# KogarashiNetwork/dusk-plonk

Hardware: AMD Instinct MI355X
Metric: PLONK prover constraints/sec (BLS12-381) at n=2^16 and 2^20, 1/2/4/8 GPUs (higher is better)
Workload: dtype u32-limb Montgomery Fr/Fp (integer)

## Files before the change

### dusk-plonk_amd/csrc/debug.hip

```cpp
#include <hip/hip_runtime.h>

#include "g1r.hpp"
#include "internal.hpp"

namespace plk {
namespace {

template <class C>
__global__ void k_field_op(int op, const Fe<C>* __restrict__ a, const Fe<C>* __restrict__ b,
                           Fe<C>* __restrict__ out, uint64_t n) {
  const uint64_t i = (uint64_t)blockIdx.x * blockDim.x + threadIdx.x;
  if (i >= n) return;
  const Fe<C> x = a[i], y = b[i];
  Fe<C> r;
  switch (op) {
    case 0: r = fe_mul(x, y); break;
    case 1: r = fe_add(x, y); break;
    case 2: r = fe_sub(x, y); break;
    case 3: r = fe_sqr(x); break;
    default: r = fe_inv(x); break;
  }
  out[i] = r;
}

template <class C>
int run(plk_ctx* ctx, int op, const uint64_t* a, const uint64_t* b, uint64_t* out, size_t n) {
  const size_t bytes = n * sizeof(Fe<C>);
  DevBuf da, db, dout;
  int st;
  if ((st = da.alloc(bytes)) || (st = db.alloc(bytes)) || (st = dout.alloc(bytes))) return st;
  hipStream_t s = ctx->stream;
  PLK_HIP_TRY(hipMemcpyAsync(da.ptr, a, bytes, hipMemcpyHostToDevice, s));
  PLK_HIP_TRY(hipMemcpyAsync(db.ptr, b ? b : a, bytes, hipMemcpyHostToDevice, s));
  hipLaunchKernelGGL(k_field_op<C>, dim3((unsigned)((n + 255) / 256)), dim3(256), 0, s, op,
                     da.as<Fe<C>>(), db.as<Fe<C>>(), dout.as<Fe<C>>(), (uint64_t)n);
  PLK_HIP_TRY(hipGetLastError());
  PLK_HIP_TRY(hipMemcpyAsync(out, dout.ptr, bytes, hipMemcpyDeviceToHost, s));
  PLK_HIP_TRY(stream_wait(s));
  return PLK_OK;
}

enum : int {
  kOpMul = 0, kOpSqr, kOpMulAdd, kOpMul2, kOpMul2Asm, kOpSqr2, kOpSqr2Asm, kOpMulAddMul2,
  kOpMulAddMul2Asm, kOpMul3, kOpAdd, kOpSub, kOpSubLazy, kOpSub2N6, kOpSmall2, kOpSmall3,
  kOpCanon, kOpIsZero, kOpIsZeroU, kOpUnpackPack, kOpSubU = 100, kOpSubN = 200
};

constexpr int rx_op_nin(int op) {
  if (op >= kOpSubU) return 2;
  switch (op) {
    case kOpSqr: case kOpSmall2: case kOpSmall3: case kOpCanon: case kOpIsZero: case kOpIsZeroU:
    case kOpUnpackPack: return 1;
    case kOpMul: case kOpSqr2: case kOpSqr2Asm: case kOpAdd: case kOpSub: case kOpSubLazy: return 2;
    case kOpSub2N6: return 3;
    default: return 4;
  }
}
constexpr int rx_op_nout(int op) {
  switch (op) {
    case kOpMul2: case kOpMul2Asm: case kOpSqr2: case kOpSqr2Asm: case kOpUnpackPack: return 2;
    case kOpMulAddMul2: case kOpMulAddMul2Asm: case kOpMul3: return 3;
    default: return 1;
  }
}

template <class C>
__device__ __forceinline__ Rx<C> ld_row(const uint32_t* __restrict__ p, uint64_t i) {
  Rx<C> r;
#pragma unroll
  for (int k = 0; k < RxShape<C>::L; ++k) r.v[k] = p[i * RxShape<C>::L + k];
  return r;
}
template <class C>
__device__ __forceinline__ void st_row(uint32_t* __restrict__ p, uint64_t i, const Rx<C>& r) {
#pragma unroll
  for (int k = 0; k < RxShape<C>::L; ++k) p[i * RxShape<C>::L + k] = r.v[k];
}
template <class C>
__device__ __forceinline__ Rx<C> rx_flag(bool f) {
  Rx<C> r = rx_zero<C>();
  r.v[0] = f ? 1u : 0u;
  return r;
}

template <class C, int OP>
__global__ void __launch_bounds__(256)
    k_rx_op(const uint32_t* __restrict__ a, const uint32_t* __restrict__ b,
            const uint32_t* __restrict__ c, const uint32_t* __restrict__ d,
            uint32_t* __restrict__ out, uint64_t n) {
  constexpr int NIN = rx_op_nin(OP), NOUT = rx_op_nout(OP);
  const uint64_t i = (uint64_t)blockIdx.x * blockDim.x + threadIdx.x;
  if (i >= n) return;
  const Rx<C> x0 = ld_row<C>(a, i);
  const Rx<C> x1 = NIN > 1 ? ld_row<C>(b, i) : rx_zero<C>();
  const Rx<C> x2 = NIN > 2 ? ld_row<C>(c, i) : rx_zero<C>();
  const Rx<C> x3 = NIN > 3 ? ld_row<C>(d, i) : rx_zero<C>();
  Rx<C> o0 = rx_zero<C>(), o1 = rx_zero<C>(), o2 = rx_zero<C>();
  if constexpr (OP == kOpMul) o0 = rx_mul(x0, x1);
  else if constexpr (OP == kOpSqr) o0 = rx_sqr(x0);
  else if constexpr (OP == kOpMulAdd) o0 = rx_mul_add(x0, x1, x2, x3);
  else if constexpr (OP == kOpMul2) rx_mul2<C, false>(x0, x1, x2, x3, o0, o1);
  else if constexpr (OP == kOpMul2Asm) rx_mul2<C, true>(x0, x1, x2, x3, o0, o1);
  else if constexpr (OP == kOpSqr2) rx_sqr2<C, false>(x0, x1, o0, o1);
  else if constexpr (OP == kOpSqr2Asm) rx_sqr2<C, true>(x0, x1, o0, o1);
  else if constexpr (OP == kOpMulAddMul2) rx_mul_add_mul2<C, false>(x0, x1, x2, x3, x0, x3, x2, x1, o0, o1, o2);
  else if constexpr (OP == kOpMulAddMul2Asm) rx_mul_add_mul2<C, true>(x0, x1, x2, x3, x0, x3, x2, x1, o0, o1, o2);
  else if constexpr (OP == kOpMul3) rx_mul3<C>(x0, x1, x2, x3, x3, x0, o0, o1, o2);
  else if constexpr (OP == kOpAdd) o0 = rx_add(x0, x1);
  else if constexpr (OP == kOpSub) o0 = rx_sub(x0, x1);
  else if constexpr (OP == kOpSubLazy) o0 = rx_sub_lazy(x0, x1);
  else if constexpr (OP == kOpSub2N6) o0 = rx_sub2_n<C, 6>(x0, x1, x2);
  else if constexpr (OP == kOpSmall2) o0 = rx_small_mul_n<C, 2>(x0);
  else if constexpr (OP == kOpSmall3) o0 = rx_small_mul_n<C, 3>(x0);
  else if constexpr (OP == kOpCanon) o0 = rx_canon(x0);
  else if constexpr (OP == kOpIsZero) o0 = rx_flag<C>(rx_is_zero(x0));
  else if constexpr (OP == kOpIsZeroU) o0 = rx_flag<C>(rx_is_zero_u(x0));
  else if constexpr (OP == kOpUnpackPack) {
    Fe<C> w;
#pragma unroll
    for (int k = 0; k < C::N; ++k) w.v[k] = x0.v[k];
    o0 = rx_unpack(w);
    w = rx_pack(o0);
#pragma unroll
    for (int k = 0; k < C::N; ++k) o1.v[k] = w.v[k];
  } else if constexpr (OP >= kOpSubN) o0 = rx_sub_n<C, OP - kOpSubN>(x0, x1);
  else o0 = rx_sub_u<C, OP - kOpSubU>(x0, x1);
  st_row<C>(out, i * NOUT, o0);
  if constexpr (NOUT > 1) st_row<C>(out, i * NOUT + 1, o1);
  if constexpr (NOUT > 2) st_row<C>(out, i * NOUT + 2, o2);
}

using RxKernel = void (*)(const uint32_t*, const uint32_t*, const uint32_t*, const uint32_t*,
                          uint32_t*, uint64_t);
#define PLK_RX_CASE(C, OP) \
  case OP: return k_rx_op<C, OP>;
#define PLK_RX_COMMON(C)                                                                       \
  PLK_RX_CASE(C, kOpMul) PLK_RX_CASE(C, kOpSqr) PLK_RX_CASE(C, kOpMulAdd) PLK_RX_CASE(C, kOpMul2) \
  PLK_RX_CASE(C, kOpMul2Asm) PLK_RX_CASE(C, kOpSqr2) PLK_RX_CASE(C, kOpMulAddMul2)             \
  PLK_RX_CASE(C, kOpMul3) PLK_RX_CASE(C, kOpAdd) PLK_RX_CASE(C, kOpSub) PLK_RX_CASE(C, kOpSubLazy) \
  PLK_RX_CASE(C, kOpSub2N6) PLK_RX_CASE(C, kOpSmall2) PLK_RX_CASE(C, kOpSmall3)                \
  PLK_RX_CASE(C, kOpCanon) PLK_RX_CASE(C, kOpIsZero) PLK_RX_CASE(C, kOpIsZeroU)                \
  PLK_RX_CASE(C, kOpUnpackPack) PLK_RX_CASE(C, kOpSubU + 3) PLK_RX_CASE(C, kOpSubU + 5)        \
  PLK_RX_CASE(C, kOpSubU + 6) PLK_RX_CASE(C, kOpSubN + 3) PLK_RX_CASE(C, kOpSubN + 5)          \
  PLK_RX_CASE(C, kOpSubN + 6)
RxKernel rx_kernel(int field, int op) {
  if (field == 0) {
    switch (op) {
      PLK_RX_COMMON(FrCfg)
      default: return nullptr;
    }
  }
  switch (op) {
    PLK_RX_COMMON(FpCfg)
    PLK_RX_CASE(FpCfg, kOpSqr2Asm) PLK_RX_CASE(FpCfg, kOpMulAddMul2Asm)
    PLK_RX_CASE(FpCfg, kOpSubU + 4) PLK_RX_CASE(FpCfg, kOpSubU + 10)
    PLK_RX_CASE(FpCfg, kOpSubN + 4) PLK_RX_CASE(FpCfg, kOpSubN + 10)
// ... 17 lines not shown
  r.X = ld_row<FpCfg>(p, 4 * i);
  r.Y = ld_row<FpCfg>(p, 4 * i + 1);
  r.ZZ = ld_row<FpCfg>(p, 4 * i + 2);
  r.ZZZ = ld_row<FpCfg>(p, 4 * i + 3);
  return r;
}

template <bool GROUPED, bool ASM, bool PAIRS>
__device__ __forceinline__ G1R madd_as_accumulate(const G1R& acc, const G1R& q, bool neg) {
  RFp y = q.Y;
  if (neg) y = rx_neg_lazy(y);
  const bool was_inf = g1r_is_inf(acc);
  G1R r = g1r_madd_lazy_sl<GROUPED, ASM, PAIRS>(acc, q.X, y);
  if (rx_is_zero(r.ZZ)) {
    RFp yr = q.Y;
    if (neg) yr = rx_neg(yr);
    r = g1r_madd_lazy_fix(was_inf, r, q.X, yr);
  }
  return r;
}

template <int OP>
__global__ void __launch_bounds__(256)
    k_g1r_op(const uint32_t* __restrict__ p, const uint32_t* __restrict__ q,
             const uint32_t* __restrict__ flags, uint32_t* __restrict__ out, uint64_t n) {
  const uint64_t t = (uint64_t)blockIdx.x * blockDim.x + threadIdx.x;
  const uint64_t i = OP == kG1AddQuad ? t >> 2 : t;
  if (i >= n) return;
  const G1R a = ld_g1row(p, i);
  G1R b = g1_op_needs_q(OP) ? ld_g1row(q, i) : a;
  const bool neg = g1_op_needs_q(OP) && flags && (flags[i] & 1u);
  G1R r;
  if constexpr (OP == kG1Madd000) r = madd_as_accumulate<false, false, false>(a, b, neg);
  else if constexpr (OP == kG1Madd100) r = madd_as_accumulate<true, false, false>(a, b, neg);
  else if constexpr (OP == kG1Madd110) r = madd_as_accumulate<true, true, false>(a, b, neg);
  else if constexpr (OP == kG1Madd111) r = madd_as_accumulate<true, true, true>(a, b, neg);
  else if constexpr (OP == kG1MaddLazy) r = g1r_madd_lazy(a, b.X, neg ? rx_neg_lazy(b.Y) : b.Y);
  else if constexpr (OP == kG1AddLazy || OP == kG1AddQuad) {
    if (neg) b.Y = rx_neg_lazy(b.Y);
    if constexpr (OP == kG1AddLazy) r = g1r_add_lazy(a, b);
    else r = g1r_add_quad(a, b, threadIdx.x & 3u);
  } else if constexpr (OP == kG1DblLazy) r = g1r_dbl_lazy(a);
  else if constexpr (OP == kG1LazyFinish) r = g1r_lazy_finish(a);
  else if constexpr (OP == kG1Add) r = g1r_add(a, neg ? g1r_neg(b) : b);
  else if constexpr (OP == kG1AddAffine) r = g1r_add_affine(a, b.X, neg ? rx_neg(b.Y) : b.Y);
  else if constexpr (OP == kG1Dbl) r = g1r_dbl(a);
  else r = g1r_dbl_affine(a.X, a.Y);
  st_row<FpCfg>(out, 4 * t, r.X);
  st_row<FpCfg>(out, 4 * t + 1, r.Y);
  st_row<FpCfg>(out, 4 * t + 2, r.ZZ);
  st_row<FpCfg>(out, 4 * t + 3, r.ZZZ);
}

using G1Kernel = void (*)(const uint32_t*, const uint32_t*, const uint32_t*, uint32_t*, uint64_t);
G1Kernel g1r_kernel(int op) {
  switch (op) {
#define PLK_G1_CASE(OP) \
  case OP: return k_g1r_op<OP>;
    PLK_G1_CASE(kG1Madd000) PLK_G1_CASE(kG1Madd100) PLK_G1_CASE(kG1Madd110)
    PLK_G1_CASE(kG1Madd111) PLK_G1_CASE(kG1MaddLazy) PLK_G1_CASE(kG1AddLazy)
    PLK_G1_CASE(kG1AddQuad) PLK_G1_CASE(kG1DblLazy) PLK_G1_CASE(kG1LazyFinish)
    PLK_G1_CASE(kG1Add) PLK_G1_CASE(kG1AddAffine) PLK_G1_CASE(kG1Dbl) PLK_G1_CASE(kG1DblAffine)
#undef PLK_G1_CASE
    default: return nullptr;
  }
}

struct RowArg {
  const uint32_t* host;
  size_t bytes;
};
template <class K, size_t NA>
int run_rows(plk_ctx* ctx, K kern, const RowArg (&in)[NA], uint32_t* out, size_t out_bytes,
             uint64_t threads, uint64_t n) {
  DevBuf din[NA], dout;
  int st;
  hipStream_t s = ctx->stream;
  for (size_t k = 0; k < NA; ++k) {
    if (!in[k].host) continue;
    if ((st = din[k].alloc(in[k].bytes))) return st;
    PLK_HIP_TRY(hipMemcpyAsync(din[k].ptr, in[k].host, in[k].bytes, hipMemcpyHostToDevice, s));
  }
  if ((st = dout.alloc(out_bytes))) return st;
  const dim3 grid((unsigned)((threads + 255) / 256)), block(256);
  const uint32_t* dp[NA];
  for (size_t k = 0; k < NA; ++k) dp[k] = static_cast<const uint32_t*>(din[k].ptr);
  uint32_t* const dres = static_cast<uint32_t*>(dout.ptr);
  if constexpr (NA == 4)
    hipLaunchKernelGGL(kern, grid, block, 0, s, dp[0], dp[1], dp[2], dp[3], dres, n);
  else
    hipLaunchKernelGGL(kern, grid, block, 0, s, dp[0], dp[1], dp[2], dres, n);
  PLK_HIP_TRY(hipGetLastError());
  PLK_HIP_TRY(hipMemcpyAsync(out, dout.ptr, out_bytes, hipMemcpyDeviceToHost, s));
  PLK_HIP_TRY(stream_wait(s));
  return PLK_OK;
}

}
}

extern "C" int plk_debug_rx_op(plk_ctx* ctx, int field, int op, const uint32_t* a,
                               const uint32_t* b, const uint32_t* c, const uint32_t* d,
                               uint32_t* out, size_t n) {
  try {
    if (!ctx || !out || (field != 0 && field != 1)) return PLK_E_ARG;
    const plk::RxKernel kern = plk::rx_kernel(field, op);
    if (!kern) return PLK_E_ARG;
    const uint32_t* rows[4] = {a, b, c, d};
    const int nin = plk::rx_op_nin(op);
    for (int k = 0; k < nin; ++k)
      if (!rows[k]) return PLK_E_ARG;
    if (n == 0) return PLK_OK;
    const size_t row = (field == 0 ? 9 : 13) * sizeof(uint32_t);
    plk::RowArg in[4];
    for (int k = 0; k < 4; ++k) in[k] = {k < nin ? rows[k] : nullptr, n * row};
    plk::DeviceGuard g(ctx->device);
    return plk::run_rows(ctx, kern, in, out, n * row * plk::rx_op_nout(op), n, n);
  } catch (...) {
    return PLK_E_DEVICE;
  }
}

extern "C" int plk_debug_g1r_op(plk_ctx* ctx, int op, const uint32_t* p, const uint32_t* q,
                                const uint32_t* flags, uint32_t* out, size_t n) {
  try {
    if (!ctx || !p || !out) return PLK_E_ARG;
    const plk::G1Kernel kern = plk::g1r_kernel(op);
    if (!kern || (plk::g1_op_needs_q(op) && !q)) return PLK_E_ARG;
    if (n == 0) return PLK_OK;
    const size_t row = plk::kG1Row * sizeof(uint32_t);
    const uint64_t threads = op == plk::kG1AddQuad ? 4 * (uint64_t)n : n;
    const plk::RowArg in[3] = {{p, n * row},
                               {plk::g1_op_needs_q(op) ? q : nullptr, n * row},
                               {flags, n * sizeof(uint32_t)}};
    plk::DeviceGuard g(ctx->device);
    return plk::run_rows(ctx, kern, in, out, threads * row, threads, n);
  } catch (...) {
    return PLK_E_DEVICE;
  }
}

extern "C" int plk_debug_field_op(plk_ctx* ctx, int field, int op, const uint64_t* a,
                                  const uint64_t* b, uint64_t* out, size_t n) {
  try {
    if (!ctx || !a || !out || op < 0 || op > 4 || (field != 0 && field != 1)) return PLK_E_ARG;
    if (n == 0) return PLK_OK;
    plk::DeviceGuard g(ctx->device);
    return field == 0 ? plk::run<plk::FrCfg>(ctx, op, a, b, out, n)
                      : plk::run<plk::FpCfg>(ctx, op, a, b, out, n);
  } catch (...) {
    return PLK_E_DEVICE;
  }
}
```

### dusk-plonk_amd/csrc/ntt.hip

```cpp
#include <cstdlib>
#include <type_traits>

#include "ffr.hpp"
#include "internal.hpp"

namespace plk {

namespace {

constexpr uint32_t kMaxLr = 9;
constexpr uint32_t kMaxLrHard = 10;
constexpr uint32_t kMaxLe = 10;

__device__ __forceinline__ Fr ld_fr(const Fr* p) {
  const uint4* q = reinterpret_cast<const uint4*>(p);
  uint4 a = q[0], b = q[1];
  Fr r;
  r.v[0] = a.x; r.v[1] = a.y; r.v[2] = a.z; r.v[3] = a.w;
  r.v[4] = b.x; r.v[5] = b.y; r.v[6] = b.z; r.v[7] = b.w;
  return r;
}

__device__ __forceinline__ void st_fr(Fr* p, const Fr& v) {
  uint4* q = reinterpret_cast<uint4*>(p);
// ... 49 lines not shown

__device__ __forceinline__ RFr sub_u(const RFr& a, const RFr& b) { return rx_sub_u<FrCfg, 3>(a, b); }

constexpr uint32_t kB = RxShape<FrCfg>::B;
constexpr uint32_t kQMax = 32;

struct FrLimbTab {
  uint32_t v[kQMax * kL];
};
constexpr FrLimbTab make_ztab() {
  FrLimbTab t{};
  for (uint32_t q = 0; q < kQMax; ++q) {
    const RxMultiple<FrCfg> m = rx_multiple<FrCfg>(q, false);
    int64_t br = 0;
    for (int i = 0; i < kL; ++i) {
      const int64_t top = (i == kL - 1) ? (int64_t)1 << kB : 0;
      int64_t d = top - (int64_t)m.v[i] + br;
      br = 0;
      if (i < kL - 1 && d < 0) {
        d += (int64_t)1 << kB;
        br = -1;
      }
      t.v[q * kL + i] = (uint32_t)d;
    }
  }
  return t;
}
__constant__ FrLimbTab kZTab = make_ztab();

template <uint32_t CP>
struct FrRaised2 {
  static constexpr RxMultiple<FrCfg> make() {
    RxMultiple<FrCfg> m = rx_multiple<FrCfg>(CP, false);
    m.v[0] += 2u << kB;
    for (int i = 1; i < kL - 1; ++i) m.v[i] += (2u << kB) - 2u;
    m.v[kL - 1] -= 2u;
    return m;
  }
  static constexpr RxMultiple<FrCfg> k = make();
};
template <uint32_t CP>
__device__ __forceinline__ RFr sub_u2(const RFr& a, const RFr& b) {
  constexpr RxMultiple<FrCfg> Q = FrRaised2<CP>::k;
  RFr r;
#pragma unroll
  for (int i = 0; i < kL; ++i) r.v[i] = a.v[i] + Q.v[i] - b.v[i];
  return r;
}

__device__ __forceinline__ RFr add_u(const RFr& a, const RFr& b) {
  RFr r;
#pragma unroll
  for (int i = 0; i < kL; ++i) r.v[i] = a.v[i] + b.v[i];
  return r;
}

__device__ __forceinline__ RFr reduce_q(const RFr& a, const uint32_t* ztab) {
  constexpr uint32_t MASK = (1u << kB) - 1;
  const uint32_t* z = ztab + (a.v[kL - 1] >> (255 - kB * (kL - 1))) * kL;
  RFr r;
  uint32_t c = 0;
#pragma unroll
  for (int i = 0; i < kL - 1; ++i) {
    const uint32_t t = a.v[i] + z[i] + c;
    r.v[i] = t & MASK;
    c = t >> kB;
  }
  r.v[kL - 1] = a.v[kL - 1] + z[kL - 1] + c - (1u << kB);
  return r;
}

__device__ __forceinline__ RFr twmul(const RFr& a, const uint32_t* twl, uint32_t TS, uint32_t idx) {
  return rx_mul(a, lds_ld(twl, TS, idx));
}
__device__ __forceinline__ void twmul2(const RFr& a0, uint32_t i0, const RFr& a1, uint32_t i1,
                                       const uint32_t* twl, uint32_t TS, RFr& o0, RFr& o1) {
  rx_mul2<FrCfg, true>(a0, lds_ld(twl, TS, i0), a1, lds_ld(twl, TS, i1), o0, o1);
}

template <bool H1>
__device__ __forceinline__ void r4_math(const uint32_t* twl, uint32_t TS, const uint32_t* ztab,
                                        uint32_t r, uint32_t h, uint32_t sh1, uint32_t sh2,
                                        const RFr& x0, const RFr& x1, const RFr& x2,
                                        const RFr& x3, RFr& o0, RFr& o1, RFr& o2, RFr& o3) {
  const RFr y0 = add_u(x0, x2), y1 = add_u(x1, x3);
  if constexpr (H1) {
    const RFr y2 = reduce_q(rx_sub_u<FrCfg, 6>(x0, x2), ztab);
    const RFr y3 = twmul(rx_sub_u<FrCfg, 6>(x1, x3), twl, TS, 1u << sh1);
    o0 = reduce_q(add_u(y0, y1), ztab);
    o2 = reduce_q(add_u(y2, y3), ztab);
    o1 = reduce_q(sub_u2<11>(y0, y1), ztab);
    o3 = reduce_q(rx_sub_u<FrCfg, 5>(y2, y3), ztab);
  } else {
    RFr y2, y3;
    twmul2(rx_sub_u<FrCfg, 6>(x0, x2), r << sh1, rx_sub_u<FrCfg, 6>(x1, x3), (r + h) << sh1, twl, TS,
           y2, y3);
    twmul2(sub_u2<11>(y0, y1), r << sh2, rx_sub_u<FrCfg, 5>(y2, y3), r << sh2, twl, TS, o1, o3);
    o0 = reduce_q(add_u(y0, y1), ztab);
    o2 = reduce_q(add_u(y2, y3), ztab);
  }
}

template <uint32_t DS, bool H1>
__device__ __forceinline__ void r4_step(uint32_t* data, const uint32_t* twl, uint32_t TS,
                                        const uint32_t* ztab, uint32_t r, uint32_t h,
                                        uint32_t sh1, uint32_t sh2, uint32_t i0, uint32_t i1,
                                        uint32_t i2, uint32_t i3, const RFr& x0, const RFr& x1,
                                        const RFr& x2, const RFr& x3) {
  RFr o0, o1, o2, o3;
  r4_math<H1>(twl, TS, ztab, r, h, sh1, sh2, x0, x1, x2, x3, o0, o1, o2, o3);
  lds_std<DS>(data, i0, o0);
  lds_std<DS>(data, i2, o2);
  lds_std<DS>(data, i1, o1);
  lds_std<DS>(data, i3, o3);
}

__device__ __forceinline__ void quad_transpose(RFr& a0, RFr& a1, RFr& a2, RFr& a3) {
  const uint32_t lane = __lane_id();
  const bool b0 = lane & 1u, b1 = lane & 2u;
#pragma unroll
  for (int l = 0; l < kL; ++l) {
    const uint32_t s01 = b0 ? a0.v[l] : a1.v[l], s23 = b0 ? a2.v[l] : a3.v[l];
    const uint32_t r01 = (uint32_t)__builtin_amdgcn_mov_dpp((int)s01, 0xB1, 0xF, 0xF, false);
    const uint32_t r23 = (uint32_t)__builtin_amdgcn_mov_dpp((int)s23, 0xB1, 0xF, 0xF, false);
    if (b0) { a0.v[l] = r01; a2.v[l] = r23; } else { a1.v[l] = r01; a3.v[l] = r23; }
    const uint32_t s02 = b1 ? a0.v[l] : a2.v[l], s13 = b1 ? a1.v[l] : a3.v[l];
    const uint32_t r02 = (uint32_t)__builtin_amdgcn_mov_dpp((int)s02, 0x4E, 0xF, 0xF, false);
    const uint32_t r13 = (uint32_t)__builtin_amdgcn_mov_dpp((int)s13, 0x4E, 0xF, 0xF, false);
    if (b1) { a0.v[l] = r02; a1.v[l] = r13; } else { a2.v[l] = r02; a3.v[l] = r13; }
  }
}

template <int PRE, int POST, int PRUNE, uint32_t DS>
__global__ void __launch_bounds__(256, PLK_NTT_MINW) k_ntt_pass(const Fr* __restrict__ in, Fr* __restrict__ out,
                                                  const Fr* __restrict__ tw,
                                                  const Fr* __restrict__ ptw,
                                                  const Fr* __restrict__ pre,
                                                  const Fr* __restrict__ post, Fr post_scalar,
                                                  uint32_t log_n, uint32_t lp, uint32_t lr,
                                                  uint32_t lt, uint64_t len_in, NttStrides str) {
  extern __shared__ __attribute__((aligned(16))) uint32_t smem32[];
  const uint32_t R = 1u << lr, T = 1u << lt, p = 1u << lp;
  const uint32_t E = R << lt, H = R >> 1;
  const uint32_t TS = PRUNE ? R : H;
  uint32_t* data = smem32;
  uint32_t* twl = smem32 + kL * DS;
  uint32_t* ztab = twl + kL * TS;

  {
    const uint32_t y = blockIdx.y;
    const uint32_t yi = str.group_in ? y % str.group_in : y, gi = str.group_in ? y / str.group_in : 0;
    in += (size_t)yi * str.in + (size_t)gi * str.in_group;
    out += (size_t)y * str.out;
    if (PRE == 1) pre += (size_t)yi * str.pre;
    if (POST == 2) post += (size_t)(str.group_post ? y % str.group_post : y) * str.post;
  }

  const uint32_t tid = threadIdx.x, bd = blockDim.x;
  const uint32_t nr_log = log_n - lr;

  for (uint32_t x = tid; x < TS; x += bd) lds_st(twl, TS, x, ld_rfr(&tw[(size_t)x << nr_log]));
  for (uint32_t x = tid; x < kQMax * kL; x += bd) ztab[x] = kZTab.v[x];

  constexpr uint32_t kLoadIt = 4;
  const uint32_t nit = (E + bd - 1) / bd;
  Fr raw[kLoadIt], aux[kLoadIt];
  auto issue = [&](uint32_t i0) {
#pragma unroll
    for (uint32_t c = 0; c < kLoadIt; ++c) {
      const uint32_t e = min(tid + c * bd, E - 1);
      const size_t g = (size_t)(i0 + (e & (T - 1))) + ((size_t)(e >> lt) << nr_log);
      const size_t gc = g < len_in ? g : 0;
      raw[c] = ld_fr(&in[gc]);
      if (PRE == 1) aux[c] = ld_fr(&pre[gc]);
    }
    if (PRE != 1 && lp != 0) {
#pragma unroll
      for (uint32_t c = 0; c < kLoadIt; ++c) {
        const uint32_t e = min(tid + c * bd, E - 1);
        aux[c] = ld_fr(&ptw[((size_t)(e >> lt) << lp) + ((i0 + (e & (T - 1))) & (p - 1))]);
      }
    }
  };
  const uint32_t i0 = blockIdx.x << lt;

  int lh = (int)lr - 1 - (PRUNE ? 3 : 0);
  const bool r2first = !PRUNE && (lr & 1) && lr >= 3 && E >= 2 * bd;
  if (PRUNE) {
    __syncthreads();
    const uint32_t R8 = R >> 3;
    for (uint32_t it = tid; it < (E >> 2); it += bd) {
      const uint32_t hs = it & 1, t = (it >> 1) & (T - 1), j = it >> (lt + 1);
      const uint32_t i = i0 + t;
      const size_t g = (size_t)i + ((size_t)j << nr_log);
      RFr x = rx_zero<FrCfg>(), x8 = rx_zero<FrCfg>();
      if (g < len_in) {
        x = ld_rfr(&in[g]);
        if (PRE == 1) x = rx_mul(x, ld_rfr(&pre[g]));
      }
      const size_t g8 = (size_t)i + ((size_t)R8 << nr_log);
      const bool has8 = j == 0 && g8 < len_in;
      if (has8) {
        x8 = ld_rfr(&in[g8]);
        if (PRE == 1) x8 = rx_mul(x8, ld_rfr(&pre[g8]));
      }
#pragma unroll
      for (uint32_t q = 0; q < 4; ++q) {
        const uint32_t blk = 4 * hs + q, b = bitrev(blk, 3);
        RFr v = (j == 0 || b == 0) ? x : rx_mul(x, lds_ld(twl, TS, j * b));
        if (has8) v = rx_add(v, b == 0 ? x8 : rx_mul(x8, lds_ld(twl, TS, R8 * b)));
        lds_std<DS>(data, ((blk * R8 + j) << lt) + t, v);
      }
    }
  }
  if (!PRUNE) {
    issue(i0);
    auto input = [&](uint32_t c) -> RFr {
      const uint32_t e = tid + c * bd;
      const uint32_t t = e & (T - 1), j = e >> lt;
      const uint32_t i = i0 + t;
      const size_t g = (size_t)i + ((size_t)j << nr_log);
      RFr v = rx_zero<FrCfg>();
      if (g < len_in) {
        v = rx_unpack(raw[c]);
        if (PRE == 1) v = rx_mul(v, rx_unpack(aux[c]));
      }
      if (PRE != 1 && lp != 0) v = rx_mul(v, rx_unpack(aux[c]));
      return v;
    };
    {
      if (r2first) __syncthreads();
#pragma unroll
      for (uint32_t c = 0; c < kLoadIt; ++c) {
        if (c >= nit) break;
        const uint32_t e = tid + c * bd;
        const RFr v = input(c);
        if (r2first && 2 * c >= nit) {
          const uint32_t el = e - (E >> 1);
          const RFr a = lds_ldd<DS>(data, el);
          lds_std<DS>(data, el, reduce_q(add_u(a, v), ztab));
          lds_std<DS>(data, e, twmul(sub_u(a, v), twl, TS, el >> lt));
        } else if (e < E) {
          lds_std<DS>(data, e, v);
        }
      }
      if (r2first) lh -= 1;
    }
  }
  __syncthreads();

  for (; lh >= 1; lh -= 2) {
    const uint32_t h = 1u << (lh - 1);
    const uint32_t sh1 = lr - 1 - lh, sh2 = lr - lh;
    const bool quad = lh == 3 && lr >= 5 && (E >> 2) % bd == 0;
    if (quad) {
      for (uint32_t g = tid; g < (E >> 2); g += bd) {
        const uint32_t r = g & 3u, t = (g >> 2) & (T - 1), B = g >> (2 + lt);
        const uint32_t j = (B << 4) + r;
        RFr x0 = lds_ldd<DS>(data, (j << lt) + t), x1 = lds_ldd<DS>(data, ((j + 4) << lt) + t);
        RFr x2 = lds_ldd<DS>(data, ((j + 8) << lt) + t), x3 = lds_ldd<DS>(data, ((j + 12) << lt) + t);
        RFr o0, o1, o2, o3;
        r4_math<false>(twl, TS, ztab, r, 4, lr - 4, lr - 3, x0, x1, x2, x3, o0, o1, o2, o3);
        quad_transpose(o0, o1, o2, o3);
        const uint32_t jq = (B << 4) + (r << 2);
        r4_step<DS, true>(data, twl, TS, ztab, 0, 1, lr - 2, lr - 1, (jq << lt) + t,
                    ((jq + 1) << lt) + t, ((jq + 2) << lt) + t, ((jq + 3) << lt) + t, o0, o1, o2,
                    o3);
      }
      lh -= 2;
      __syncthreads();
      continue;
    }
    auto steps = [&](auto h1) {
      for (uint32_t g = tid; g < (E >> 2); g += bd) {
        const uint32_t t = g & (T - 1), jg = g >> lt;
        const uint32_t r = jg & (h - 1);
        const uint32_t j = ((jg >> (lh - 1)) << (lh + 1)) + r;
        const uint32_t i0 = (j << lt) + t, i1 = ((j + h) << lt) + t;
        const uint32_t i2 = ((j + 2 * h) << lt) + t, i3 = ((j + 3 * h) << lt) + t;
        const RFr x0 = lds_ldd<DS>(data, i0), x1 = lds_ldd<DS>(data, i1);
        const RFr x2 = lds_ldd<DS>(data, i2), x3 = lds_ldd<DS>(data, i3);
        r4_step<DS, decltype(h1)::value>(data, twl, TS, ztab, r, h, sh1, sh2, i0, i1, i2, i3, x0, x1, x2, x3);
      }
    };
    if (h == 1) steps(std::true_type{});
    else steps(std::false_type{});
    __syncthreads();
  }
  if (lh == 0) {
    for (uint32_t b = tid; b < (E >> 1); b += bd) {
      const uint32_t t = b & (T - 1), jb = b >> lt;
      const uint32_t j1 = jb << 1;
      const RFr a = lds_ldd<DS>(data, (j1 << lt) + t);
      const RFr c = lds_ldd<DS>(data, ((j1 + 1) << lt) + t);
      lds_std<DS>(data, (j1 << lt) + t, reduce_q(add_u(a, c), ztab));
      lds_std<DS>(data, ((j1 + 1) << lt) + t, reduce_q(rx_sub_u<FrCfg, 6>(a, c), ztab));
    }
    __syncthreads();
  }

  for (uint32_t o = tid; o < E; o += bd) {
    uint32_t t, m;
    if (p >= T) {
      t = o & (T - 1);
      m = o >> lt;
    } else {
      const uint32_t s = o & (p - 1);
      m = (o >> lp) & (R - 1);
      t = ((o >> (lp + lr)) << lp) + s;
    }
    const uint32_t i = i0 + t;
    const uint32_t k = i & (p - 1);
    const size_t pos = ((size_t)(i - k) << lr) + k + ((size_t)m << lp);
    RFr v = lds_ldd<DS>(data, (bitrev(m, lr) << lt) + t);
    if (POST == 1) v = rx_mul(v, rx_unpack(post_scalar));
    else if (POST == 2) v = rx_mul(v, ld_rfr(&post[pos]));
    else v = reduce_q(v, ztab);
    st_fr(&out[pos], rx_pack_canonical(v));
  }
}

__global__ void k_pass_twiddles(const Fr* __restrict__ tw, Fr* __restrict__ out, uint32_t lp,
                                uint32_t lr, uint32_t shift) {
  const uint64_t e = (uint64_t)blockIdx.x * blockDim.x + threadIdx.x;
  if (e >= (1ull << (lp + lr))) return;
  const uint64_t j = e >> lp, k = e & ((1ull << lp) - 1);
  st_fr(&out[e], ld_fr(&tw[(j * k) << shift]));
}

__global__ void k_scale_table(const Fr* __restrict__ in, Fr* __restrict__ out, Fr s, uint64_t n) {
  const uint64_t e = (uint64_t)blockIdx.x * blockDim.x + threadIdx.x;
  if (e >= n) return;
  st_fr(&out[e], fe_mul(ld_fr(&in[e]), s));
}

__global__ void k_table_to_rx(const Fr* in, Fr* out, uint64_t n) {
  const uint64_t e = (uint64_t)blockIdx.x * blockDim.x + threadIdx.x;
  if (e >= n) return;
  st_fr(&out[e], fe_to_rx_domain(ld_fr(&in[e])));
}

__global__ void k_power_table(Fr* __restrict__ out, Fr base, Fr scale, uint64_t n) {
  const uint64_t e = (uint64_t)blockIdx.x * blockDim.x + threadIdx.x;
  if (e >= n) return;
  st_fr(&out[e], fe_mul(fe_pow_u64(base, e), scale));
}

__global__ void k_copy_pad(const Fr* __restrict__ in, Fr* __restrict__ out, uint64_t len_in,
                           uint64_t n) {
  const uint64_t e = (uint64_t)blockIdx.x * blockDim.x + threadIdx.x;
  if (e >= n) return;
  st_fr(&out[e], e < len_in ? ld_fr(&in[e]) : fe_zero<FrCfg>());
}

__global__ void k_vanishing(Fr* __restrict__ out, Fr gdeg, Fr wdeg, uint64_t n) {
  const uint64_t e = (uint64_t)blockIdx.x * blockDim.x + threadIdx.x;
  if (e >= n) return;
  st_fr(&out[e], fe_sub(fe_mul(gdeg, fe_pow_u64(wdeg, e)), fe_one<FrCfg>()));
}

}

void fr_root_of_unity(uint32_t log_n, Fr& omega) {
  static const uint32_t root[8] = {0x439f0d2bu, 0x3829971fu, 0x8c2280b9u, 0xb6368350u,
                                   0x22c813b4u, 0xd09b6819u, 0xdfe81f20u, 0x16a2a19eu};
  Fr w;
  for (int i = 0; i < 8; ++i) w.v[i] = root[i];
  w = fe_to_mont(w);
  for (uint32_t s = log_n; s < 32; ++s) w = fe_sqr(w);
  omega = w;
}

static void plan_domain(plk_domain* d) {
  const uint32_t L = d->log_n;
  d->plan.clear();
  if (L == 0) return;
  static const uint32_t le_min = [] {
    const char* e = getenv("PLK_NTT_LE_MIN");
    const int v = e ? atoi(e) : 10;
    return (uint32_t)(v >= 1 && v <= (int)kMaxLe ? v : 10);
  }();
  uint32_t le = L > 8 ? L - 8 : 1;
  if (le < le_min) le = L < le_min ? L : le_min;
  if (le > kMaxLe) le = kMaxLe;
  static const uint32_t lr_cap = [] {
    const char* e = getenv("PLK_NTT_MAX_LR");
    const int v = e ? atoi(e) : (int)kMaxLr;
    return (uint32_t)(v >= 1 && v <= (int)kMaxLrHard ? v : kMaxLr);
  }();
  const uint32_t max_lr = le < lr_cap ? le : lr_cap;
  const uint32_t P = (L + max_lr - 1) / max_lr;
  uint32_t lp = 0;
  for (uint32_t q = 0; q < P; ++q) {
    const uint32_t rem = L - lp, left = P - q;
    const uint32_t lr = (rem + left - 1) / left;
    uint32_t lt = le - lr;
    if (lt > L - lr) lt = L - lr;
    d->plan.push_back(NttPass{lp, lr, lt});
    lp += lr;
  }
  d->le = le;
}

int ntt_build_domain(plk_domain* d) {
  const uint64_t n = d->n;
  fr_root_of_unity(d->log_n, d->omega);
  d->omega_inv = fe_inv(d->omega);
  Fr nf = fe_zero<FrCfg>();
  nf.v[0] = (uint32_t)n;
  nf.v[1] = (uint32_t)(n >> 32);
  nf = fe_to_mont(nf);
  d->n_inv = fe_inv(nf);
  Fr g = fe_zero<FrCfg>();
  g.v[0] = 7;
  d->g = fe_to_mont(g);
  d->g_inv = fe_inv(d->g);
  plan_domain(d);

  int st;
  if ((st = d->tw_fwd.alloc(n * sizeof(Fr)))) return st;
  if ((st = d->tw_inv.alloc(n * sizeof(Fr)))) return st;
  if ((st = d->coset_pow.alloc(n * sizeof(Fr)))) return st;
  if ((st = d->icoset_scale.alloc(n * sizeof(Fr)))) return st;
  hipStream_t s = d->ctx->stream;
  const uint32_t bs = 256;
  const uint32_t nb = (uint32_t)((n + bs - 1) / bs);
  const Fr one = fe_one<FrCfg>();
  hipLaunchKernelGGL(k_power_table, dim3(nb), dim3(bs), 0, s, d->tw_fwd.as<Fr>(), d->omega, one, n);
  hipLaunchKernelGGL(k_power_table, dim3(nb), dim3(bs), 0, s, d->tw_inv.as<Fr>(), d->omega_inv, one, n);
  hipLaunchKernelGGL(k_power_table, dim3(nb), dim3(bs), 0, s, d->coset_pow.as<Fr>(), d->g, one, n);
  hipLaunchKernelGGL(k_power_table, dim3(nb), dim3(bs), 0, s, d->icoset_scale.as<Fr>(), d->g_inv,
                     d->n_inv, n);
  if ((st = d->tw_fwd_rx.alloc(n * sizeof(Fr)))) return st;
  hipLaunchKernelGGL(k_table_to_rx, dim3(nb), dim3(bs), 0, s, d->tw_fwd.as<Fr>(), d->tw_fwd_rx.as<Fr>(), n);
  hipLaunchKernelGGL(k_table_to_rx, dim3(nb), dim3(bs), 0, s, d->tw_inv.as<Fr>(), d->tw_inv.as<Fr>(), n);
  hipLaunchKernelGGL(k_table_to_rx, dim3(nb), dim3(bs), 0, s, d->coset_pow.as<Fr>(), d->coset_pow.as<Fr>(), n);
  hipLaunchKernelGGL(k_table_to_rx, dim3(nb), dim3(bs), 0, s, d->icoset_scale.as<Fr>(),
                     d->icoset_scale.as<Fr>(), n);
  PLK_HIP_TRY(hipGetLastError());
  d->pass_tw_fwd.clear();
  d->pass_tw_inv.clear();
  d->pass_tw_fwd.resize(d->plan.size());
  d->pass_tw_inv.resize(d->plan.size());
  for (size_t q = 1; q < d->plan.size(); ++q) {
    const NttPass& ps = d->plan[q];
    const uint64_t cnt = 1ull << (ps.lp + ps.lr);
    const uint32_t shift = d->log_n - ps.lr - ps.lp;
    if ((st = d->pass_tw_fwd[q].alloc(cnt * sizeof(Fr)))) return st;
    if ((st = d->pass_tw_inv[q].alloc(cnt * sizeof(Fr)))) return st;
    const uint32_t pb = (uint32_t)((cnt + bs - 1) / bs);
    hipLaunchKernelGGL(k_pass_twiddles, dim3(pb), dim3(bs), 0, s, d->tw_fwd_rx.as<Fr>(),
                       d->pass_tw_fwd[q].as<Fr>(), ps.lp, ps.lr, shift);
    hipLaunchKernelGGL(k_pass_twiddles, dim3(pb), dim3(bs), 0, s, d->tw_inv.as<Fr>(),
                       d->pass_tw_inv[q].as<Fr>(), ps.lp, ps.lr, shift);
    if (q + 1 == d->plan.size()) {
      if ((st = d->pass_tw_inv_last.alloc(cnt * sizeof(Fr)))) return st;
      hipLaunchKernelGGL(k_scale_table, dim3(pb), dim3(bs), 0, s, d->pass_tw_inv[q].as<Fr>(),
                         d->pass_tw_inv_last.as<Fr>(), d->n_inv, cnt);
    }
  }
  PLK_HIP_TRY(hipGetLastError());
  PLK_HIP_TRY(stream_wait(s));
  return PLK_OK;
}

int ntt_run(plk_domain* d, const Fr* in, Fr* out, size_t len_in, int dir, int coset, Fr* scratch,
            hipStream_t stream, uint32_t count, const Fr* pre_table) {
  NttBatch b;
  b.in_stride = b.out_stride = d->n;
  b.pre = pre_table;
  return ntt_run_batch(d, in, out, len_in, dir, coset, scratch, stream, count, b);
}

int ntt_run_batch(plk_domain* d, const Fr* in, Fr* out, size_t len_in, int dir, int coset,
                  Fr* scratch, hipStream_t stream, uint32_t count, const NttBatch& bt) {
  const uint64_t n = d->n;
  if (len_in > n || count == 0) return PLK_E_ARG;
  const Fr* pre_table = bt.pre;
  if (n == 1) {
    if (bt.pre || bt.post) return PLK_E_ARG;
    for (uint32_t v = 0; v < count; ++v) {
      Fr* o = out + v * bt.out_stride;
      const Fr* i = in + v * bt.in_stride;
      if (len_in == 0) {
        PLK_HIP_TRY(hipMemsetAsync(o, 0, sizeof(Fr), stream));
      } else if (i != o) {
        PLK_HIP_TRY(hipMemcpyAsync(o, i, sizeof(Fr), hipMemcpyDeviceToDevice, stream));
      }
    }
    return PLK_OK;
  }
  int st;
  const size_t P = d->plan.size();
  const uint64_t in_ext = bt.group ? (uint64_t)(count / bt.group - 1) * bt.in_group_stride +
                                         (uint64_t)(bt.group - 1) * bt.in_stride + len_in
                                   : (uint64_t)(count - 1) * bt.in_stride + len_in;
  const uint64_t out_ext = (uint64_t)(count - 1) * bt.out_stride + n;
  const bool out_pp = P >= 2 && bt.out_stride >= n && (len_in == 0 || in + in_ext <= out || out + out_ext <= in);
  if (!scratch) {
    if ((st = d->scratch.alloc(2 * n * sizeof(Fr) * (count > 1 ? count : 1)))) return st;
    scratch = d->scratch.as<Fr>();
  }
  Fr* s1 = scratch;
  Fr* s2 = scratch + n * count;
  const Fr* tw = dir > 0 ? d->tw_fwd_rx.as<Fr>() : d->tw_inv.as<Fr>();
  const Fr n_inv_rx = fe_to_rx_domain(d->n_inv);
  const bool no_input = len_in == 0;
  const Fr* src = no_input ? tw : in;
  for (size_t q = 0; q < P; ++q) {
    const NttPass& ps = d->plan[q];
    Fr* dst = (q + 1 == P) ? out : out_pp ? (((P - 1 - q) & 1) ? s1 : out) : ((q & 1) ? s2 : s1);
    const bool first = q == 0, last = q + 1 == P;
    const uint32_t E = 1u << (ps.lr + ps.lt);
    uint32_t bd = E / 4;
    if (bd < 64) bd = 64;
    if (bd > 256) bd = 256;
    const uint32_t blocks = (uint32_t)(n >> (ps.lr + ps.lt));
    const int pre = (first && dir > 0 && coset) ? 1 : 0;
    const bool scaled_tw = last && !first && dir < 0 && !coset;
    const int post = (last && dir < 0 && !scaled_tw) ? (coset ? 2 : 1) : 0;
    const uint64_t lin = first ? len_in : n;
    const bool prune = first && !last && ps.lr >= 4 &&
                       len_in <= ((n >> ps.lr) << (ps.lr - 3)) + (n >> ps.lr);
    const bool small = E <= kDSSmall;
    const size_t lds = ((size_t)(small ? kDSSmall : kDS) + ((1u << ps.lr) >> (prune ? 0 : 1)) + kQMax) *
                       kL * sizeof(uint32_t);
    dim3 grid(blocks, count);
    const Fr* ptw = q == 0 ? nullptr
                    : scaled_tw ? d->pass_tw_inv_last.as<Fr>()
                    : (dir > 0 ? d->pass_tw_fwd[q].as<Fr>() : d->pass_tw_inv[q].as<Fr>());
    NttStrides str;
    str.in = first ? (no_input ? 0 : bt.in_stride) : n * 1;
    str.out = last ? bt.out_stride : n * 1;
    str.pre = bt.pre ? bt.pre_stride : 0;
    str.post = bt.post ? bt.post_stride : 0;
    str.in_group = first && !no_input ? bt.in_group_stride : 0;
    str.group_in = first ? bt.group : 0;
    str.group_post = last ? bt.group : 0;
#define PLK_LAUNCH_DS(PRE, POST, PRUNE, DS)                                               \
  do {                                                                                    \
    const void* kp_ = reinterpret_cast<const void*>(&k_ntt_pass<PRE, POST, PRUNE, DS>);   \
    if (lds > 65536)                                                                      \
      PLK_HIP_TRY(hipFuncSetAttribute(kp_, hipFuncAttributeMaxDynamicSharedMemorySize, (int)lds)); \
    hipLaunchKernelGGL((k_ntt_pass<PRE, POST, PRUNE, DS>), grid, dim3(bd), lds, stream, src, dst, \
                       tw, ptw, pre_table ? pre_table : d->coset_pow.as<Fr>(),            \
                       bt.post ? bt.post : d->icoset_scale.as<Fr>(), n_inv_rx, d->log_n,  \
                       ps.lp, ps.lr, ps.lt, lin, str);                                     \
  } while (0)
#define PLK_LAUNCH(PRE, POST, PRUNE)                              \
  do {                                                            \
    if (small) PLK_LAUNCH_DS(PRE, POST, PRUNE, kDSSmall);          \
    else PLK_LAUNCH_DS(PRE, POST, PRUNE, kDS);                     \
  } while (0)
    if (prune) {
      if (pre == 1) PLK_LAUNCH(1, 0, 1);
      else PLK_LAUNCH(0, 0, 1);
    } else if (pre == 0 && post == 0) PLK_LAUNCH(0, 0, 0);
    else if (pre == 1 && post == 0) PLK_LAUNCH(1, 0, 0);
    else if (pre == 0 && post == 1) PLK_LAUNCH(0, 1, 0);
    else if (pre == 0 && post == 2) PLK_LAUNCH(0, 2, 0);
    else if (pre == 1 && post == 1) PLK_LAUNCH(1, 1, 0);
    else PLK_LAUNCH(1, 2, 0);
#undef PLK_LAUNCH_DS
#undef PLK_LAUNCH
    PLK_HIP_TRY(hipGetLastError());
    src = dst;
  }
  return PLK_OK;
}

int ntt_power_table(Fr* out, const Fr& base, const Fr& scale, uint64_t n, bool to_rx,
                    hipStream_t s) {
  if (n == 0) return PLK_OK;
  const uint32_t nb = (uint32_t)((n + 255) / 256);
  hipLaunchKernelGGL(k_power_table, dim3(nb), dim3(256), 0, s, out, base, scale, n);
  if (to_rx) hipLaunchKernelGGL(k_table_to_rx, dim3(nb), dim3(256), 0, s, out, out, n);
  PLK_HIP_TRY(hipGetLastError());
  return PLK_OK;
}

int ntt_vanishing(plk_domain* d, uint64_t deg, Fr* d_out, hipStream_t s) {
  const Fr gdeg = fe_pow_u64(d->g, deg);
  const Fr wdeg = fe_pow_u64(d->omega, deg);
  const uint32_t bs = 256;
  const uint32_t nb = (uint32_t)((d->n + bs - 1) / bs);
  hipLaunchKernelGGL(k_vanishing, dim3(nb), dim3(bs), 0, s, d_out, gdeg, wdeg, (uint64_t)d->n);
  PLK_HIP_TRY(hipGetLastError());
  return PLK_OK;
}

}
```

### dusk-plonk_amd/csrc/prover.hip

```cpp
#include <hip/hip_runtime.h>

#include <algorithm>
#include <cstring>
#include <memory>
#include <mutex>
#include <vector>

#include "ffr.hpp"
#include "internal.hpp"
#include "msm_common.hpp"
#include "prover.hpp"
#include "transcript.hpp"

using namespace plk;

namespace {

Fr fr_u64(uint64_t v) {
  Fr x = fe_zero<FrCfg>();
  x.v[0] = (uint32_t)v;
  x.v[1] = (uint32_t)(v >> 32);
  return fe_to_mont(x);
}
Fr fr_from(const plk_fr& a) {
// ... 204 lines not shown
    g.pi = *pi;
  }
  (void)append_gate(c, g);
}

void append_dummy_gates(plk_composer* c) {
  const uint32_t six = append_witness(c, fr_u64(6));
  const uint32_t one = append_witness(c, fr_u64(1));
  const uint32_t seven = append_witness(c, fr_u64(7));
  const uint32_t min_twenty = append_witness(c, fe_neg(fr_u64(20)));
  Gate g = default_gate();
  g.q[QM] = fr_u64(1);
  g.q[QL] = fr_u64(2);
  g.q[QR] = fr_u64(3);
  g.q[Q4] = fr_u64(1);
  g.q[QC] = fr_u64(4);
  g.q[QO] = fr_u64(4);
  g.w[0] = six;
  g.w[1] = seven;
  g.w[3] = one;
  g.w[2] = min_twenty;
  (void)append_gate(c, g);
  Gate h = default_gate();
  h.q[QM] = fr_u64(1);
  h.q[QL] = fr_u64(1);
  h.q[QR] = fr_u64(1);
  h.q[QC] = fr_u64(127);
  h.q[QO] = fr_u64(1);
  h.w[0] = min_twenty;
  h.w[1] = six;
  h.w[2] = seven;
  (void)append_gate(c, h);
}

Gate gate_from(const plk_constraint* s) {
  Gate g = default_gate();
  const plk_fr* qs[11] = {&s->q_m, &s->q_l, &s->q_r, &s->q_o, &s->q_4, &s->q_c, &s->q_arith,
                          &s->q_range, &s->q_logic, &s->q_fixed_group_add, &s->q_variable_group_add};
  for (int i = 0; i < 11; ++i) g.q[i] = fr_from(*qs[i]);
  g.w[0] = s->a;
  g.w[1] = s->b;
  g.w[2] = s->o;
  g.w[3] = s->d;
  g.has_pi = s->has_public != 0;
  g.pi = fr_from(s->public_input);
  return g;
}

uint32_t log2_ceil(uint64_t x) {
  uint32_t k = 0;
  while ((1ull << k) < x) ++k;
  return k;
}

#define TRY(...)                       \
  do {                                 \
    int _st = (__VA_ARGS__);           \
    if (_st != PLK_OK) return _st;     \
  } while (0)

int key_commit(plk_key* key, MsmWorkspace& ws, const std::vector<const Fr*>& ptrs,
               const std::vector<size_t>& lens, plk_g1* outs, int* statuses, hipStream_t s,
               size_t cap = SIZE_MAX) {
  const size_t max_points = std::min<size_t>(std::min<size_t>(key->srs->n, key->n_trim), cap);
  std::vector<size_t> use(lens.size());
  for (size_t i = 0; i < lens.size(); ++i) use[i] = std::min(lens[i], max_points);
  int overall = PLK_OK;
  for (size_t base = 0; base < ptrs.size(); base += kMaxSlots) {
    const size_t m = std::min<size_t>(kMaxSlots, ptrs.size() - base);
    const int r = msm_run_batch(key->srs, ws, ptrs.data() + base, use.data() + base,
                                lens.data() + base, m, outs + base,
                                statuses ? statuses + base : nullptr, s);
    if (r != PLK_OK && r != PLK_E_DEGREE) return r;
    if (r != PLK_OK) overall = r;
  }
  return overall;
}

int shard_commit(plk_prover* P, const std::vector<const Fr*>& ptrs,
                 const std::vector<size_t>& lens, plk_g1* outs, int* statuses, size_t cap) {
  plk_key* key = P->key;
  const size_t cnt = ptrs.size();
  const size_t max_points = std::min<size_t>(std::min<size_t>(key->srs->n, key->n_trim), cap);
  const bool buckets = P->shard_buckets;
  plk_srs* srs = buckets ? key->srs : P->shard;
  const uint64_t lo = buckets ? 0 : P->shard_lo, hi = buckets ? key->srs->n : lo + P->shard->n;
  const bool last = buckets || P->rank == P->world - 1;
  const uint32_t part = buckets ? (uint32_t)P->rank : 0, parts = buckets ? (uint32_t)P->world : 1;
  std::vector<const Fr*> lp(cnt);
  std::vector<size_t> luse(cnt), lchk(cnt);
  int local = PLK_OK;
  if (last && hi < max_points) local = PLK_E_ARG;
  for (size_t i = 0; i < cnt; ++i) {
    const size_t use = std::min(lens[i], max_points);
    luse[i] = use > lo ? (size_t)(std::min<uint64_t>(use, hi) - lo) : 0;
    lchk[i] = luse[i];
    lp[i] = ptrs[i] + lo;
    if (last && lens[i] > use) {
      if (use >= lo) {
        lchk[i] = lens[i] - lo;
      } else {
        lp[i] = ptrs[i] + use;
        lchk[i] = lens[i] - use;
      }
    }
  }
  std::vector<plk_g1> shares(cnt, plk_g1{});
  std::vector<int> pst(cnt, PLK_OK);
  for (size_t base = 0; local == PLK_OK && base < cnt; base += kMaxSlots) {
    const size_t m = std::min<size_t>(kMaxSlots, cnt - base);
    const int r = msm_run_batch(srs, *P->ws, lp.data() + base, luse.data() + base,
                                lchk.data() + base, m, shares.data() + base, pst.data() + base,
                                P->stream, part, parts);
    if (r != PLK_OK && r != PLK_E_DEGREE) local = r;
  }
  constexpr size_t kWords = 14;
  std::vector<uint64_t> send(cnt * kWords), recv((size_t)P->world * cnt * kWords);
  for (size_t i = 0; i < cnt; ++i) {
    uint64_t* w = &send[i * kWords];
    std::memcpy(w, &shares[i], sizeof(plk_g1));
    w[13] = (uint64_t)(local != PLK_OK ? local : pst[i]);
  }
  if (P->allgather(P->allgather_user, send.data(), send.size() * 8, recv.data()) != 0)
    return PLK_E_DEVICE;
  int overall = PLK_OK;
  std::vector<plk_g1> pts((size_t)P->world);
  for (size_t i = 0; i < cnt; ++i) {
    int st = PLK_OK;
    for (int r = 0; r < P->world; ++r) {
      const uint64_t* w = &recv[((size_t)r * cnt + i) * kWords];
      std::memcpy(&pts[r], w, sizeof(plk_g1));
      if (w[13] != PLK_OK && (st == PLK_OK || st == PLK_E_DEGREE)) st = (int)w[13];
    }
    if (st != PLK_OK && st != PLK_E_DEGREE) return st;
    if (statuses) statuses[i] = st;
    if (st != PLK_OK) {
      outs[i] = plk_g1{};
      overall = PLK_E_DEGREE;
      continue;
    }
    const int r = plk_g1_sum(pts.data(), pts.size(), &outs[i]);
    if (r != PLK_OK) return r;
  }
  return overall;
}

int prover_commit(plk_prover* P, const std::vector<const Fr*>& ptrs,
                  const std::vector<size_t>& lens, plk_g1* outs, int* statuses,
                  size_t cap = SIZE_MAX) {
  if (P->shard || P->shard_buckets) return shard_commit(P, ptrs, lens, outs, statuses, cap);
  return key_commit(P->key, *P->ws, ptrs, lens, outs, statuses, P->stream, cap);
}

Fr cube_root_of_unity() {
  static const uint32_t w[8] = {0xffffffffu, 0x00000000u, 0x0001a402u, 0xac45a401u,
                                0u, 0u, 0u, 0u};
  Fr x;
  for (int i = 0; i < 8; ++i) x.v[i] = w[i];
  return fe_to_mont(x);
}

Fr edwards_d() {
  static const uint32_t w[8] = {0xd6343eb1u, 0x01065fd6u, 0x37579d26u, 0x292d7f6du,
                                0xe6bd7fd4u, 0xf5fd9207u, 0x4bfa2b48u, 0x2a9318e7u};
  Fr x;
  for (int i = 0; i < 8; ++i) x.v[i] = w[i];
  return fe_to_mont(x);
}

Fr d2h_fr(const Fr* p, hipStream_t s) {
  thread_local PinnedBuf pin;
  if (pin.alloc(sizeof(Fr)) != PLK_OK) return fe_zero<FrCfg>();
  (void)hipMemcpyAsync(pin.ptr, p, sizeof(Fr), hipMemcpyDeviceToHost, s);
  (void)stream_wait(s);
  return *pin.as<Fr>();
}

}

namespace plk {
namespace {
__global__ void k_sigma_values(const uint32_t* __restrict__ codes, const Fr* __restrict__ el,
                               uint64_t n, Fr k1, Fr k2, Fr k3, Fr* __restrict__ out) {
  const uint64_t i = (uint64_t)blockIdx.x * blockDim.x + threadIdx.x;
  if (i >= 4 * n) return;
  const uint32_t code = codes[i];
  const uint32_t g = code >> 2, col = code & 3;
  Fr v = el[g];
  if (col == 1) v = fe_mul(v, k1);
  if (col == 2) v = fe_mul(v, k2);
  if (col == 3) v = fe_mul(v, k3);
  out[i] = v;
}
}
}

extern "C" {

namespace {
std::mutex g_pool_mu;
std::vector<std::unique_ptr<plk_composer>> g_pool;
constexpr size_t kPoolMax = 2;

std::unique_ptr<plk_composer> composer_from_pool() {
  {
    std::lock_guard<std::mutex> lk(g_pool_mu);
    if (!g_pool.empty()) {
      std::unique_ptr<plk_composer> c = std::move(g_pool.back());
      g_pool.pop_back();
      return c;
    }
  }
  return std::unique_ptr<plk_composer>(new plk_composer());
}
}

int plk_composer_create(plk_composer** out) {
  try {
    if (!out) return PLK_E_ARG;
    std::unique_ptr<plk_composer> c = composer_from_pool();
    const uint32_t zero = append_witness(c.get(), fe_zero<FrCfg>());
    const uint32_t one = append_witness(c.get(), fe_one<FrCfg>());
    assert_equal_constant(c.get(), zero, fe_zero<FrCfg>(), nullptr);
    assert_equal_constant(c.get(), one, fe_one<FrCfg>(), nullptr);
    append_dummy_gates(c.get());
    append_dummy_gates(c.get());
    *out = c.release();
    return PLK_OK;
  } catch (...) {
    return PLK_E_OOM;
  }
}

int plk_composer_destroy(plk_composer* c) {
  if (!c) return PLK_OK;
  std::unique_ptr<plk_composer> h(c);
  h->witness.clear();
  h->gates.clear();
  h->consts.clear();
  h->wire_head.clear();
  h->wire_tail.clear();
  h->wire_next.clear();
  h->struct_hash = plk_composer::kHashInit;
  std::lock_guard<std::mutex> lk(g_pool_mu);
  if (g_pool.size() < kPoolMax) g_pool.push_back(std::move(h));
  return PLK_OK;
}

int plk_composer_size(const plk_composer* c, size_t* gates, size_t* witnesses) {
  if (!c) return PLK_E_ARG;
  if (gates) *gates = c->gates.size();
  if (witnesses) *witnesses = c->witness.size();
  return PLK_OK;
}

int plk_composer_append_witness(plk_composer* c, const plk_fr* v, uint32_t* wire) {
  if (!c || !v || !wire) return PLK_E_ARG;
  *wire = append_witness(c, fr_from(*v));
  return PLK_OK;
}

int plk_composer_witness_value(const plk_composer* c, uint32_t wire, plk_fr* v) {
  if (!c || !v || wire >= c->witness.size()) return PLK_E_ARG;
  *v = fr_to(c->witness[wire]);
  return PLK_OK;
}

int plk_composer_append_public(plk_composer* c, const plk_fr* v, uint32_t* wire) {
  if (!c || !v || !wire) return PLK_E_ARG;
  const Fr val = fr_from(*v);
  *wire = append_witness(c, val);
  const Fr neg = fe_neg(val);
  assert_equal_constant(c, *wire, fe_zero<FrCfg>(), &neg);
  return PLK_OK;
}

int plk_composer_append_gate(plk_composer* c, const plk_constraint* s) {
  if (!c || !s) return PLK_E_ARG;
  return append_gate(c, gate_from(s));
}

int plk_composer_append_custom_gate(plk_composer* c, const plk_constraint* s) {
  if (!c || !s) return PLK_E_ARG;
  return append_custom_gate(c, gate_from(s));
}

int plk_composer_gate_eval(plk_composer* c, const plk_constraint* s, uint32_t* out) {
  if (!c || !s || !out) return PLK_E_ARG;
  Gate g = gate_from(s);
  g.q[QARITH] = fe_one<FrCfg>();
  g.q[QO] = fe_neg(fe_one<FrCfg>());
  for (int k = 0; k < 4; ++k)
    if (g.w[k] >= c->witness.size() && k != 2) return PLK_E_ARG;
  uint32_t o;
  if (!evaluated_output(c, g, o)) return PLK_E_ARG;
  g.w[2] = o;
  *out = o;
  return append_gate(c, g);
}

int plk_composer_assert_equal(plk_composer* c, uint32_t a, uint32_t b) {
  if (!c || a >= c->witness.size() || b >= c->witness.size()) return PLK_E_ARG;
  Gate g = default_gate();
  g.q[QL] = fe_one<FrCfg>();
  g.q[QR] = fe_neg(fe_one<FrCfg>());
  g.w[0] = a;
  g.w[1] = b;
  return append_gate(c, g);
}

int plk_composer_assert_equal_constant(plk_composer* c, uint32_t a, const plk_fr* constant,
                                       const plk_fr* public_input) {
  if (!c || !constant || a >= c->witness.size()) return PLK_E_ARG;
  const Fr pi = public_input ? fr_from(*public_input) : fe_zero<FrCfg>();
// ... 13 lines not shown
    Gate base = default_gate();
    base.q[QRANGE] = fe_one<FrCfg>();
    std::vector<Gate> cons(num_gates + 1, base);
    std::vector<uint32_t> accs;
    const Fr four = fr_u64(4);
    Fr acc = fe_zero<FrCfg>();
    for (size_t i = pad; i <= num_quads; ++i) {
      const size_t bi = (num_quads - i) << 1;
      const uint32_t quad = (bi < 256 ? bit(bi) : 0u) + 2 * (bi + 1 < 256 ? bit(bi + 1) : 0u);
      acc = fe_add(fe_mul(four, acc), fr_u64(quad));
      const uint32_t w = append_witness(c, acc);
      accs.push_back(w);
      Gate& g = cons[i / 4];
      switch (i % 4) {
        case 0: g.w[3] = w; break;
        case 1: g.w[2] = w; break;
        case 2: g.w[1] = w; break;
        default: g.w[0] = w; break;
      }
    }
    cons.back() = default_gate();
    if (!accs.empty()) cons.back().w[3] = accs.back();
    for (const Gate& g : cons)
      if (append_custom_gate(c, g) != PLK_OK) return PLK_E_ARG;
    if (!accs.empty()) return plk_composer_assert_equal(c, accs.back(), witness);
    return PLK_OK;
  } catch (...) {
    return PLK_E_OOM;
  }
}

int plk_composer_component_boolean(plk_composer* c, uint32_t a) {
  if (!c || a >= c->witness.size()) return PLK_E_ARG;
  Gate g = default_gate();
  g.q[QM] = fe_one<FrCfg>();
  g.q[QO] = fe_neg(fe_one<FrCfg>());
  g.w[0] = a;
  g.w[1] = a;
  g.w[2] = a;
  g.w[3] = 0;
  return append_gate(c, g);
}

int plk_composer_synthetic_chain(plk_composer* c, size_t gates, uint64_t seed) {
  if (!c) return PLK_E_ARG;
  try {
    Rng rng{seed};
    uint32_t x = append_witness(c, rng.fr_mont());
    c->witness.reserve(c->witness.size() + 2 * gates);
    c->wire_head.reserve(c->wire_head.size() + 2 * gates);
    c->wire_tail.reserve(c->wire_tail.size() + 2 * gates);
    c->wire_next.reserve(c->wire_next.size() + 4 * gates);
    c->gates.reserve(c->gates.size() + gates);
    GateRec g;
    g.code = (kSelOne << (2 * QM)) | (kSelOne << (2 * QL)) | (kSelMinusOne << (2 * QO)) |
             (kSelOne << (2 * QARITH));
    g.ext = (uint32_t)c->consts.size();
    g.w[3] = 0;
    for (size_t i = 0; i < gates; ++i) {
      const uint32_t y = append_witness(c, rng.fr_mont());
      const Fr& xv = c->witness[x];
      const Fr o = fe_add(fe_mul(xv, c->witness[y]), xv);
      g.w[0] = x;
      g.w[1] = y;
      g.w[2] = append_witness(c, o);
      if (push_gate(c, g) != PLK_OK) return PLK_E_ARG;
      x = g.w[2];
    }
    return PLK_OK;
  } catch (...) {
    return PLK_E_OOM;
  }
}

int plk_composer_set_witness(plk_composer* c, uint32_t wire, const plk_fr* v) {
  if (!c || !v || wire >= c->witness.size()) return PLK_E_ARG;
  c->witness[wire] = fr_from(*v);
  return PLK_OK;
}

int plk_composer_public_inputs(const plk_composer* c, plk_fr* values, uint64_t* indexes,
                               size_t cap, size_t* count) {
  if (!c || !count) return PLK_E_ARG;
  size_t k = 0;
  for (size_t i = 0; i < c->gates.size(); ++i) {
    if (!(c->gates[i].code & kPiBit)) continue;
    if (k < cap) {
      if (values) values[k] = fr_to(gate_unpack(c, i).pi);
      if (indexes) indexes[k] = i;
    }
    ++k;
  }
  *count = k;
  return PLK_OK;
}

int plk_composer_export(const plk_composer* c, plk_constraint* gates, size_t cap,
                        plk_fr* witness, size_t wcap, size_t* m, size_t* nw) {
  if (!c) return PLK_E_ARG;
  if (m) *m = c->gates.size();
  if (nw) *nw = c->witness.size();
  if (gates) {
    const size_t cnt = std::min(cap, c->gates.size());
    for (size_t i = 0; i < cnt; ++i) {
      const Gate g = gate_unpack(c, i);
      plk_constraint& o = gates[i];
      plk_fr* qs[11] = {&o.q_m,     &o.q_l,   &o.q_r,     &o.q_o,
                        &o.q_4,     &o.q_c,   &o.q_arith, &o.q_range,
                        &o.q_logic, &o.q_fixed_group_add, &o.q_variable_group_add};
      for (int q = 0; q < 11; ++q) *qs[q] = fr_to(g.q[q]);
      o.a = g.w[0];
      o.b = g.w[1];
      o.o = g.w[2];
      o.d = g.w[3];
      o.has_public = g.has_pi ? 1u : 0u;
      o._pad = 0;
      o.public_input = fr_to(g.pi);
    }
  }
  if (witness) {
    const size_t cnt = std::min(wcap, c->witness.size());
    for (size_t j = 0; j < cnt; ++j) witness[j] = fr_to(c->witness[j]);
  }
  return PLK_OK;
}

int plk_key_compile(plk_srs* srs, const plk_composer* cs, const char* label, plk_key** out) {
  try {
    if (!srs || !cs || !out) return PLK_E_ARG;
    *out = nullptr;
    plk_ctx* ctx = srs->ctx;
    DeviceGuard guard(ctx->device);
    hipStream_t s = ctx->stream;
    std::unique_ptr<plk_key> key(new plk_key());
    key->ctx = ctx;
    key->srs = srs;
    key->label = label ? label : "plonk";
    const uint64_t m = cs->gates.size();
    const uint32_t k = log2_ceil(m);
    const uint64_t n = 1ull << k;
    key->m = m;
    key->n = n;
    key->k = k;
    key->n_trim = (1ull << log2_ceil(m + 6)) + 8;
    if (k + 1 > 27) return PLK_E_ARG;
    for (uint64_t i = 0; i < m; ++i) {
      const Gate g = gate_unpack(cs, i);
      if (!fe_is_zero(g.q[QRANGE])) key->has_range = true;
      if (!fe_is_zero(g.q[QLOGIC])) key->has_logic = true;
      if (!fe_is_zero(g.q[QFIXED])) key->has_fixed = true;
      if (!fe_is_zero(g.q[QVAR])) key->has_var = true;
    }
    TRY(plk_domain_get(ctx, k, &key->dom));
    TRY(plk_domain_get(ctx, k + 1, &key->domq));
    const uint64_t n2 = 2 * n, nq = kQBlocks * n2;

    std::vector<Fr> host(11 * n, fe_zero<FrCfg>());
    for (uint64_t i = 0; i < m; ++i) {
      const Gate g = gate_unpack(cs, i);
      for (int q = 0; q < 11; ++q) host[q * n + i] = g.q[q];
    }
    TRY(key->q_coef.alloc(11 * n * sizeof(Fr)));
    PLK_HIP_TRY(hipMemcpyAsync(key->q_coef.ptr, host.data(), 11 * n * sizeof(Fr),
                               hipMemcpyHostToDevice, s));
    Fr* qc = key->q_coef.as<Fr>();
    for (int q = 0; q < 11; ++q) TRY(ntt_run(key->dom, qc + q * n, qc + q * n, n, -1, 0, nullptr, s, 1));

    std::vector<uint32_t> codes(4 * n);
    for (uint64_t i = 0; i < n; ++i)
      for (uint32_t col = 0; col < 4; ++col) codes[col * n + i] = (uint32_t)(4 * i + col);
    for (size_t wit = 0; wit < cs->wire_head.size(); ++wit)
      for (uint32_t cur = cs->wire_head[wit]; cur != plk_composer::kNoWire; cur = cs->wire_next[cur]) {
        const uint32_t nx = cs->wire_next[cur];
        const uint32_t nxt = nx == plk_composer::kNoWire ? cs->wire_head[wit] : nx;
        codes[(cur & 3) * n + (cur >> 2)] = nxt;
      }
    DevBuf dcodes;
    TRY(dcodes.alloc(4 * n * 4));
    PLK_HIP_TRY(hipMemcpyAsync(dcodes.ptr, codes.data(), 4 * n * 4, hipMemcpyHostToDevice, s));
    TRY(key->sigma_lag.alloc(4 * n * sizeof(Fr)));
    hipLaunchKernelGGL(k_sigma_values, dim3((unsigned)((4 * n + 255) / 256)), dim3(256), 0, s,
                       dcodes.as<uint32_t>(), key->dom->tw_fwd.as<Fr>(), n, fr_u64(7), fr_u64(13),
                       fr_u64(17), key->sigma_lag.as<Fr>());
    PLK_HIP_TRY(hipGetLastError());
    TRY(key->sigma_coef.alloc(4 * n * sizeof(Fr)));
    Fr* sc = key->sigma_coef.as<Fr>();
    for (int c = 0; c < 4; ++c)
      TRY(ntt_run(key->dom, key->sigma_lag.as<Fr>() + c * n, sc + c * n, n, -1, 0, nullptr, s, 1));

    const int order[11] = {QM, QL, QR, QO, QC, Q4, QARITH, QRANGE, QLOGIC, QFIXED, QVAR};
    std::vector<const Fr*> ptrs;
    std::vector<size_t> lens;
    for (int q : order) {
      ptrs.push_back(qc + q * n);
      lens.push_back(n);
    }
    for (int c = 0; c < 4; ++c) {
      ptrs.push_back(sc + c * n);
      lens.push_back(n);
    }
    int sts[15];
    const int r = key_commit(key.get(), *srs->ws, ptrs, lens, key->comms, sts, s);
    if (r != PLK_OK && r != PLK_E_DEGREE) return r;
    for (int i = 0; i < 11; ++i)
      if (sts[i] != PLK_OK) key->comms[i] = plk_g1{{0}, {0}, 1};
    for (int i = 11; i < 15; ++i)
      if (sts[i] != PLK_OK) return sts[i];

    {
      const Fr gq = key->domq->g, one = fe_one<FrCfg>();
      const Fr w3 = cube_root_of_unity();
      const uint64_t rowc = n + 8;
      TRY(key->coset_s.alloc(kQBlocks * rowc * sizeof(Fr)));
      TRY(key->coset_w.alloc(kQBlocks * rowc * sizeof(Fr)));
      TRY(key->coset_pi.alloc(kQBlocks * rowc * sizeof(Fr)));
      TRY(key->icoset_q.alloc(kQBlocks * n2 * sizeof(Fr)));
      const Fr c32 = fr_u64(32), inv3 = fe_inv(fr_u64(3));
      Fr sm = gq;
      for (int mb = 0; mb < kQBlocks; ++mb) {
        key->s_m[mb] = sm;
        TRY(ntt_power_table(key->coset_s.as<Fr>() + mb * rowc, sm, one, rowc, true, s));
        TRY(ntt_power_table(key->coset_w.as<Fr>() + mb * rowc, sm, c32, rowc, true, s));
        TRY(ntt_power_table(key->coset_pi.as<Fr>() + mb * rowc, sm, fe_inv(c32), rowc, true, s));
        TRY(ntt_power_table(key->icoset_q.as<Fr>() + mb * n2, fe_inv(sm),
                            fe_mul(key->domq->n_inv, inv3), n2, true, s));
        sm = fe_mul(sm, w3);
      }
      const Fr eta_inv = fe_inv(fe_pow_u64(w3, n2));
      const Fr eta_inv2 = fe_sqr(eta_inv);
      const Fr g1 = fe_inv(fe_pow_u64(gq, n2)), g2 = fe_sqr(g1);
      const Fr cm[6] = {g1, fe_mul(g1, eta_inv), fe_mul(g1, eta_inv2),
                        g2, fe_mul(g2, eta_inv2), fe_mul(g2, eta_inv)};
      for (int j = 0; j < 6; ++j) key->comb[j] = fe_to_rx_domain(cm[j]);
      for (int mb = 0; mb < kQBlocks; ++mb) {
        const Fr x = fe_pow_u64(key->s_m[mb], n);
        key->vh_inv[2 * mb] = fe_inv(fe_sub(x, one));
        key->vh_inv[2 * mb + 1] = fe_inv(fe_sub(fe_neg(x), one));
      }
    }
    auto coset_fwd = [&](const Fr* in, Fr* out, uint64_t len, const DevBuf& table) {
      NttBatch b;
      b.in_stride = 0;
      b.out_stride = n2;
      b.pre = table.as<Fr>();
      b.pre_stride = n + 8;
      return ntt_run_batch(key->domq, in, out, len, 1, 1, nullptr, s, kQBlocks, b);
    };
    TRY(key->selq.alloc(SEL_COUNTQ * nq * sizeof(Fr)));
    const int sel_src[SEL_COUNTQ] = {QM, QL, QR, QO, Q4, QC, QARITH, QRANGE, QLOGIC, QFIXED, QVAR};
    const bool sel_used[SEL_COUNTQ] = {true, true, true, true, true, true, true, key->has_range,
                                       key->has_logic, key->has_fixed, key->has_var};
    for (int j = 0; j < SEL_COUNTQ; ++j)
      if (sel_used[j])
        TRY(coset_fwd(qc + sel_src[j] * n, key->selq.as<Fr>() + j * nq, n, key->coset_s));
    TRY(key->sigmaq.alloc(4 * nq * sizeof(Fr)));
    for (int c = 0; c < 4; ++c)
      TRY(coset_fwd(sc + c * n, key->sigmaq.as<Fr>() + c * nq, n, key->coset_s));
    TRY(key->l1q.alloc(nq * sizeof(Fr)));
    {
      DevBuf tmp;
      TRY(tmp.alloc(n * sizeof(Fr)));
      TRY(pk_fill(tmp.as<Fr>(), key->dom->n_inv, n, s));
      TRY(coset_fwd(tmp.as<Fr>(), key->l1q.as<Fr>(), n, key->coset_s));
      PLK_HIP_TRY(stream_wait(s));
    }
    std::vector<uint32_t> idx(4 * n, 0);
    for (uint64_t i = 0; i < m; ++i)
      for (int c = 0; c < 4; ++c) {
        idx[c * n + i] = cs->gates[i].w[c];
        key->max_wire = std::max(key->max_wire, cs->gates[i].w[c]);
      }
    key->struct_hash = cs->struct_hash;
    TRY(key->wire_idx.alloc(4 * n * 4));
    PLK_HIP_TRY(hipMemcpyAsync(key->wire_idx.ptr, idx.data(), 4 * n * 4, hipMemcpyHostToDevice, s));
    PLK_HIP_TRY(stream_wait(s));
    *out = key.release();
    return PLK_OK;
  } catch (const std::bad_alloc&) {
    return PLK_E_OOM;
  } catch (...) {
    return PLK_E_DEVICE;
  }
}

int plk_key_destroy(plk_key* key) {
  if (!key) return PLK_E_ARG;
  DeviceGuard g(key->ctx->device);
  (void)stream_wait(key->ctx->stream);
  delete key;
  return PLK_OK;
}

int plk_key_info(const plk_key* key, uint64_t* n, uint64_t* m, plk_g1* commitments) {
  if (!key) return PLK_E_ARG;
  if (n) *n = key->n;
  if (m) *m = key->m;
  if (commitments) std::memcpy(commitments, key->comms, sizeof key->comms);
  return PLK_OK;
}

int plk_prover_create(plk_key* key, plk_prover** out) {
  try {
    if (!key || !out) return PLK_E_ARG;
    *out = nullptr;
    DeviceGuard guard(key->ctx->device);
    std::unique_ptr<plk_prover> p(new plk_prover());
    p->key = key;
    p->ws = msm_workspace_new();
    if (!p->ws->tail_forced) p->ws->tail_quad = lane_tail_policy(key->n);
    p->ws->shared_chip = true;
    PLK_HIP_TRY(hipStreamCreateWithFlags(&p->stream, hipStreamNonBlocking));
    p->own_stream = true;
    *out = p.release();
    return PLK_OK;
  } catch (const std::bad_alloc&) {
    return PLK_E_OOM;
  }
}

int plk_prover_destroy(plk_prover* p) {
  if (!p) return PLK_E_ARG;
  DeviceGuard g(p->key->ctx->device);
  (void)stream_wait(p->stream);
  delete p;
  return PLK_OK;
}

int plk_prover_stream(plk_prover* p, void** stream_out) {
  if (!p || !stream_out) return PLK_E_ARG;
  *stream_out = p->stream;
  return PLK_OK;
}

int plk_prover_msm_stats(plk_prover* p, int reset, double* accumulate_ms, uint64_t* launches,
                         uint64_t* point_adds, uint64_t* points) {
  if (!p) return PLK_E_ARG;
  MsmStats& st = msm_workspace_stats(*p->ws);
  if (accumulate_ms) *accumulate_ms = st.cum_accumulate_ms;
  if (launches) *launches = st.cum_launches;
  if (point_adds) *point_adds = st.cum_point_adds;
  if (points) *points = st.cum_points;
  if (reset) st.reset_cum();
  return PLK_OK;
}

int plk_prover_shard(plk_prover* p, plk_srs* slice, uint64_t slice_start, int rank, int world,
                     plk_allgather_fn allgather, void* user) {
  if (!p || world < 1 || rank < 0 || rank >= world) return PLK_E_ARG;
  const bool sharded = world > 1 || (slice && allgather);
  if (sharded && (!slice || !allgather || slice->ctx->device != p->key->ctx->device))
    return PLK_E_ARG;
  p->shard = sharded ? slice : nullptr;
  p->shard_lo = sharded ? slice_start : 0;
  p->shard_buckets = false;
  p->rank = rank;
  p->world = world;
  p->allgather = sharded ? allgather : nullptr;
  p->allgather_user = user;
  return PLK_OK;
}

int plk_prover_shard_buckets(plk_prover* p, int rank, int world, plk_allgather_fn allgather,
                             void* user) {
  if (!p || !allgather || world < 1 || rank < 0 || rank >= world) return PLK_E_ARG;
  if (!msm_parts_ok(p->key->srs, (uint32_t)world)) return PLK_E_ARG;
  p->shard = nullptr;
  p->shard_lo = 0;
  p->shard_buckets = true;
  p->rank = rank;
  p->world = world;
  p->allgather = allgather;
  p->allgather_user = user;
  return PLK_OK;
}

int plk_prove(plk_key* key, const plk_composer* cs, uint64_t seed, plk_proof* proof,
              plk_fr* public_inputs, size_t pi_cap, size_t* pi_count) {
  if (!key) return PLK_E_ARG;
  std::lock_guard<std::mutex> lk(key->def_mu);
  if (!key->def_prover) {
    try {
      std::unique_ptr<plk_prover> d(new plk_prover());
      d->key = key;
      d->ws = msm_workspace_new();
      d->stream = key->ctx->stream;
      key->def_prover = std::move(d);
    } catch (const std::bad_alloc&) {
      return PLK_E_OOM;
    }
  }
  return plk_prover_prove(key->def_prover.get(), cs, seed, proof, public_inputs, pi_cap, pi_count);
}

int plk_prover_prove(plk_prover* P, const plk_composer* cs, uint64_t seed, plk_proof* proof,
                     plk_fr* public_inputs, size_t pi_cap, size_t* pi_count) {
  try {
    if (!P || !cs || !proof) return PLK_E_ARG;
    plk_key* key = P->key;
    if (cs->gates.size() != key->m || cs->struct_hash != key->struct_hash) return PLK_E_ARG;
    if (cs->witness.size() <= key->max_wire) return PLK_E_ARG;
    DeviceGuard guard(key->ctx->device);
    hipStream_t s = P->stream;
    const uint64_t n = key->n, m = key->m, S = n + 8;
    const uint64_t n2 = 2 * n, nq = kQBlocks * n2;
    Rng rng{seed};
    const Fr one = fe_one<FrCfg>();
    const Fr K1 = fr_u64(7), K2 = fr_u64(13), K3 = fr_u64(17);

    TRY(P->witness.alloc(std::max<size_t>(cs->witness.size(), 1) * sizeof(Fr)));
    TRY(P->wires_lag.alloc(4 * n * sizeof(Fr)));
    TRY(P->wires_coef.alloc(4 * S * sizeof(Fr)));
    TRY(P->z_lag.alloc(n * sizeof(Fr)));
    TRY(P->z_coef.alloc(S * sizeof(Fr)));
    TRY(P->num.alloc(n * sizeof(Fr)));
    TRY(P->den.alloc(n * sizeof(Fr)));
    TRY(P->scan_tmp.alloc((pk_scan_tmp_elems(5 * n) + 1) * sizeof(Fr)));
    TRY(P->pi_lag.alloc(n * sizeof(Fr)));
    TRY(P->pi_coef.alloc(n * sizeof(Fr)));
    TRY(P->evq.alloc(6 * nq * sizeof(Fr)));
    TRY(P->quotq.alloc(nq * sizeof(Fr)));
    TRY(P->t_coef.alloc(nq * sizeof(Fr)));
    TRY(P->agg.alloc(5 * n * sizeof(Fr)));
    TRY(P->agg2.alloc(S * sizeof(Fr)));
    TRY(P->w_coef.alloc((5 * n + S) * sizeof(Fr)));
    TRY(P->tmp_a.alloc(5 * n * sizeof(Fr)));
    TRY(P->eval_partial.alloc((size_t)kMaxEval * pk_eval_max_blocks(nq) * sizeof(Fr)));
    if (!P->eval_out.ptr) {
      TRY(P->eval_out.alloc(kMaxEval * sizeof(Fr),
                            hipHostMallocMapped | hipHostMallocCoherent | hipHostMallocPortable));
      PLK_HIP_TRY(hipHostGetDevicePointer(&P->eval_dev, P->eval_out.ptr, 0));
    }
    TRY(P->ntt_scratch.alloc(4 * nq * sizeof(Fr)));
    Fr* nsc = P->ntt_scratch.as<Fr>();

    Transcript tr(key->label);
    {
      const char dom[] = "circuit_size";
      tr.append_message("dom-sep", reinterpret_cast<const uint8_t*>(dom), sizeof(dom) - 1);
      tr.append_u64("n", m);
      const char* labels[15] = {"q_m", "q_l", "q_r", "q_o", "q_c", "q_4", "q_arith", "q_range",
                                "q_logic", "q_fixed_group_add", "q_variable_group_add",
                                "s_sigma_1", "s_sigma_2", "s_sigma_3", "s_sigma_4"};
      for (int i = 0; i < 15; ++i) tr.append_commitment(labels[i], key->comms[i]);
    }
    std::vector<std::pair<uint64_t, Fr>> pis;
    for (uint64_t i = 0; i < m; ++i)
      if (cs->gates[i].code & kPiBit) pis.emplace_back(i, gate_unpack(cs, i).pi);
    for (auto& p : pis) tr.append_scalar("pi", p.second);
    if (pi_count) *pi_count = pis.size();
    if (public_inputs)
      for (size_t i = 0; i < pis.size() && i < pi_cap; ++i) public_inputs[i] = fr_to(pis[i].second);

    {
      const size_t bytes = cs->witness.size() * sizeof(Fr);
      TRY(P->pin_witness.alloc(bytes));
      const size_t chunk = 8u << 20;
      const char* src = reinterpret_cast<const char*>(cs->witness.data());
      char* pin = P->pin_witness.as<char>();
      char* dst = P->witness.as<char>();
      for (size_t off = 0; off < bytes; off += chunk) {
        const size_t len = std::min(chunk, bytes - off);
        std::memcpy(pin + off, src + off, len);
        PLK_HIP_TRY(hipMemcpyAsync(dst + off, pin + off, len, hipMemcpyHostToDevice, s));
      }
    }
    Fr* wl = P->wires_lag.as<Fr>();
    Fr* wc = P->wires_coef.as<Fr>();
    TRY(pk_gather_wires(P->witness.as<Fr>(), key->wire_idx.as<uint32_t>(), m, n, wl, s));
    {
      NttBatch b;
      b.in_stride = n;
      b.out_stride = S;
      TRY(ntt_run_batch(key->dom, wl, wc, n, -1, 0, nsc, s, 4, b));
    }
    BlindBatch bb{};
    bb.npoly = 4;
    for (int c = 0; c < 4; ++c) {
      bb.poly[c] = wc + c * S;
      bb.b[c].count = 2;
      bb.b[c].r[0] = rng.fr();
      bb.b[c].r[1] = rng.fr();
    }
    TRY(pk_blind_batch(bb, n, s));
    plk_g1 wcom[4];
    TRY(prover_commit(P, {wc, wc + S, wc + 2 * S, wc + 3 * S}, {n + 2, n + 2, n + 2, n + 2}, wcom,
                      nullptr));
    tr.append_commitment("a_w", wcom[0]);
    tr.append_commitment("b_w", wcom[1]);
    tr.append_commitment("c_w", wcom[2]);
    tr.append_commitment("d_w", wcom[3]);

    const Fr beta = tr.challenge_scalar("beta");
    tr.append_scalar("beta", beta);
    const Fr gamma = tr.challenge_scalar("gamma");
    Fr* num = P->num.as<Fr>();
    Fr* den = P->den.as<Fr>();
    TRY(pk_perm_numden(wl, key->sigma_lag.as<Fr>(), key->dom->tw_fwd.as<Fr>(), n, beta, gamma, K1,
                       K2, K3, num, den, s));
    Fr* st = P->scan_tmp.as<Fr>();
    TRY(pk_scan(num, num, n, true, false, true, st, s));
    TRY(pk_scan(den, den, n, true, true, false, st, s));
    const uint64_t nb = pk_scan_tmp_elems(n) - 1;
    const Fr dtot = d2h_fr(st + nb, s);
    TRY(pk_mul3(num, den, fe_inv(dtot), P->z_lag.as<Fr>(), n, s));
    Fr* zc = P->z_coef.as<Fr>();
    TRY(ntt_run(key->dom, P->z_lag.as<Fr>(), zc, n, -1, 0, nsc, s, 1));
    {
      BlindArgs b{};
      b.count = 3;
      for (int i = 0; i < 3; ++i) b.r[i] = rng.fr();
      TRY(pk_blind(zc, n, b, s));
    }
    plk_g1 zcom;
    TRY(prover_commit(P, {zc}, {n + 3}, &zcom, nullptr));
    tr.append_commitment("z", zcom);

    const Fr alpha = tr.challenge_scalar("alpha");
    const Fr range_sep = tr.challenge_scalar("range separation challenge");
    const Fr logic_sep = tr.challenge_scalar("logic separation challenge");
    const Fr fixed_sep = tr.challenge_scalar("fixed base separation challenge");
    const Fr var_sep = tr.challenge_scalar("variable base separation challenge");
    Fr* pil = P->pi_lag.as<Fr>();
    TRY(P->pin_small.alloc(std::max<size_t>(pis.size(), 1) * sizeof(Fr)));
    const bool pi_direct = !pis.empty() && pis.size() <= (size_t)kPiDirect;
    if (pi_direct) {
      PiDirect pd{};
      pd.count = (uint32_t)pis.size();
      for (size_t i = 0; i < pis.size(); ++i) {
        pd.idx[i] = pis[i].first;
        pd.c[i] = fe_mul(pis[i].second, key->dom->n_inv);
      }
      TRY(pk_pi_coef(pd, key->dom->tw_inv.as<Fr>(), n, P->pi_coef.as<Fr>(), s));
    } else if (!pis.empty()) {
      PLK_HIP_TRY(hipMemsetAsync(pil, 0, n * sizeof(Fr), s));
      for (size_t i = 0; i < pis.size(); ++i) {
        P->pin_small.as<Fr>()[i] = pis[i].second;
        PLK_HIP_TRY(hipMemcpyAsync(pil + pis[i].first, P->pin_small.as<Fr>() + i, sizeof(Fr),
                                   hipMemcpyHostToDevice, s));
      }
    }
    Fr* ev = P->evq.as<Fr>();
    auto coset_fwd = [&](const Fr* in, Fr* out, uint64_t len, const DevBuf& table) {
      NttBatch b;
      b.in_stride = 0;
      b.out_stride = n2;
      b.pre = table.as<Fr>();
      b.pre_stride = n + 8;
      return ntt_run_batch(key->domq, in, out, len, 1, 1, nsc, s, kQBlocks, b);
    };
    if (!pis.empty() && !pi_direct)
      TRY(ntt_run(key->dom, pil, P->pi_coef.as<Fr>(), n, -1, 0, nsc, s, 1));
    TRY(coset_fwd(zc, ev + 0 * nq, n + 3, key->coset_s));
    {
      NttBatch b;
      b.group = kQBlocks;
      b.in_stride = 0;
      b.in_group_stride = S;
      b.out_stride = n2;
      b.pre = key->coset_w.as<Fr>();
      b.pre_stride = n + 8;
      TRY(ntt_run_batch(key->domq, wc, ev + nq, n + 2, 1, 1, nsc, s, 4 * kQBlocks, b));
    }
    if (!pis.empty()) TRY(coset_fwd(P->pi_coef.as<Fr>(), ev + 5 * nq, n, key->coset_pi));
    const Fr alpha2 = fe_sqr(alpha);
    QuotientArgs qa{};
    qa.z = ev;
    qa.a = ev + nq;
    qa.b = ev + 2 * nq;
    qa.c = ev + 3 * nq;
    qa.d = ev + 4 * nq;
    qa.pi = pis.empty() ? nullptr : ev + 5 * nq;
    qa.l1 = key->l1q.as<Fr>();
    qa.alpha2 = alpha2;
    qa.sel = key->selq.as<Fr>();
    qa.sigma = key->sigmaq.as<Fr>();
    qa.elements = key->domq->tw_fwd.as<Fr>();
    qa.out = P->quotq.as<Fr>();
    qa.nq = nq;
    qa.log_blk = key->k + 1;
    qa.g = key->domq->g;
    qa.alpha = alpha;
    qa.beta = beta;
    qa.gamma = gamma;
    qa.k1 = K1;
    qa.k2 = K2;
    qa.k3 = K3;
    qa.range_sep = range_sep;
    qa.kappa = fe_sqr(range_sep);
    qa.kappa2 = fe_sqr(qa.kappa);
    qa.kappa3 = fe_mul(qa.kappa2, qa.kappa);
    qa.has_range = key->has_range ? 1 : 0;
    qa.logic_sep = logic_sep;
    qa.lk = fe_sqr(logic_sep);
    qa.lk2 = fe_sqr(qa.lk);
    qa.lk3 = fe_mul(qa.lk2, qa.lk);
    qa.lk4 = fe_mul(qa.lk3, qa.lk);
    qa.has_logic = key->has_logic ? 1 : 0;
    qa.fixed_sep = fixed_sep;
    qa.fk = fe_sqr(fixed_sep);
    qa.fk2 = fe_sqr(qa.fk);
    qa.fk3 = fe_mul(qa.fk2, qa.fk);
    qa.var_sep = var_sep;
    qa.vk = fe_sqr(var_sep);
    qa.vk2 = fe_sqr(qa.vk);
    qa.edwards_d = edwards_d();
    qa.has_fixed = key->has_fixed ? 1 : 0;
    qa.has_var = key->has_var ? 1 : 0;
    for (int j = 0; j < 2 * kQBlocks; ++j) qa.vh_inv[j] = key->vh_inv[j];
    {
      auto em1 = [](const Fr& x) { return fe_to_rx_domain(x); };
      auto em2 = [](const Fr& x) { return fe_to_rx_domain(fe_to_rx_domain(x)); };
      const Fr one = fe_one<FrCfg>(), two = fe_dbl(one);
      for (int mb = 0; mb < kQBlocks; ++mb) qa.rx_bg[mb] = em2(fe_mul(beta, key->s_m[mb]));
      qa.rx_beta = em2(beta);
      qa.rx_gamma = em1(gamma);
      qa.rx_one_w = em1(one);
      qa.rx_two_w = em1(two);
      qa.rx_three_w = em1(fe_add(two, one));
      qa.rx_kappa = em1(qa.kappa);
      qa.rx_kappa2 = em1(qa.kappa2);
      qa.rx_kappa3 = em1(qa.kappa3);
      qa.rx_alpha2 = em1(alpha2);
      for (int j = 0; j < 2 * kQBlocks; ++j) qa.rx_vh[j] = em2(key->vh_inv[j]);
      qa.rx_32 = fr_u64(32);
      qa.rx_inv32 = fe_inv(qa.rx_32);
    }
    TRY(pk_quotient(qa, s));
    Fr* tc = P->t_coef.as<Fr>();
    {
      NttBatch b;
      b.in_stride = b.out_stride = n2;
      b.post = key->icoset_q.as<Fr>();
      b.post_stride = n2;
      TRY(ntt_run_batch(key->domq, P->quotq.as<Fr>(), P->quotq.as<Fr>(), n2, -1, 1, nsc, s,
                        kQBlocks, b));
      TRY(pk_coset3_combine(P->quotq.as<Fr>(), n2, key->comb, tc, s));
    }
    plk_g1 tcom[4];
    TRY(prover_commit(P, {tc, tc + n, tc + 2 * n, tc + 3 * n}, {n, n, n, nq - 3 * n}, tcom,
                      nullptr, n + 8));
    const uint64_t t4_len = std::min<uint64_t>(
        n + 8, std::min<uint64_t>(key->srs->n, key->n_trim));
    tr.append_commitment("t_low", tcom[0]);
    tr.append_commitment("t_mid", tcom[1]);
    tr.append_commitment("t_high", tcom[2]);
    tr.append_commitment("t_4", tcom[3]);

    const Fr zeta = tr.challenge_scalar("z_challenge");
    const Fr zw = fe_mul(zeta, key->dom->omega);
    const Fr* qc = key->q_coef.as<Fr>();
    const Fr* sc = key->sigma_coef.as<Fr>();
    struct RTerm {
      const Fr* p;
      uint64_t len;
      int ev;
    };
    std::vector<RTerm> rt;
    EvalBatch eb{};
    const Fr* polys[16] = {tc, wc, wc + S, wc + 2 * S, wc + 3 * S, sc, sc + n, sc + 2 * n,
                           qc + QARITH * n, qc + QC * n, qc + QL * n, qc + QR * n,
                           wc, wc + S, wc + 3 * S, zc};
    const uint64_t lens[16] = {3 * n + t4_len, n + 2, n + 2, n + 2, n + 2, n, n, n, n, n, n, n,
                               n + 2, n + 2, n + 2, n + 3};
    uint32_t ne = 0;
    for (int i = 0; i < 16; ++i, ++ne) {
      eb.poly[i] = polys[i];
      eb.len[i] = lens[i];
      eb.x[i] = i < 12 ? zeta : zw;
    }
    auto rterm = [&](const Fr* p, uint64_t len, int have) {
      if (have < 0) {
        eb.poly[ne] = p;
        eb.len[ne] = len;
        eb.x[ne] = zeta;
        have = (int)ne++;
      }
      rt.push_back(RTerm{p, len, have});
    };
    rterm(qc + QM * n, n, -1);
    rterm(qc + QL * n, n, 10);
    rterm(qc + QR * n, n, 11);
    rterm(qc + QO * n, n, -1);
    rterm(qc + Q4 * n, n, -1);
    rterm(qc + QC * n, n, 9);
    if (key->has_range) rterm(qc + QRANGE * n, n, -1);
    if (key->has_logic) rterm(qc + QLOGIC * n, n, -1);
    if (key->has_fixed) rterm(qc + QFIXED * n, n, -1);
    if (key->has_var) rterm(qc + QVAR * n, n, -1);
    rterm(zc, n + 3, -1);
    rterm(sc + 3 * n, n, -1);
    TRY(pk_eval(eb, ne, 3 * n + t4_len, P->eval_partial.as<Fr>(), static_cast<Fr*>(P->eval_dev), s));
    Fr evs[kMaxEval];
    PLK_HIP_TRY(stream_wait(s));
    std::memcpy(evs, P->eval_out.ptr, ne * sizeof(Fr));
    const Fr t_eval = evs[0], a_e = evs[1], b_e = evs[2], c_e = evs[3], d_e = evs[4];
    const Fr s1_e = evs[5], s2_e = evs[6], s3_e = evs[7];
    const Fr qar_e = evs[8], qc_e = evs[9], ql_e = evs[10], qr_e = evs[11];
    const Fr an_e = evs[12], bn_e = evs[13], dn_e = evs[14], perm_e = evs[15];
    std::vector<Fr> rs;
    rs.push_back(fe_mul(qar_e, fe_mul(a_e, b_e)));
    rs.push_back(fe_mul(qar_e, a_e));
    rs.push_back(fe_mul(qar_e, b_e));
    rs.push_back(fe_mul(qar_e, c_e));
    rs.push_back(fe_mul(qar_e, d_e));
    rs.push_back(qar_e);
    if (key->has_range) {
      const Fr two = fe_dbl(one), three = fe_add(two, one);
      auto delta = [&](const Fr& f) {
        return fe_mul(fe_mul(f, fe_sub(f, one)), fe_mul(fe_sub(f, two), fe_sub(f, three)));
      };
      auto four = [](const Fr& v) { return fe_dbl(fe_dbl(v)); };
      Fr r = delta(fe_sub(c_e, four(d_e)));
      r = fe_add(r, fe_mul(delta(fe_sub(b_e, four(c_e))), qa.kappa));
      r = fe_add(r, fe_mul(delta(fe_sub(a_e, four(b_e))), qa.kappa2));
      r = fe_add(r, fe_mul(delta(fe_sub(dn_e, four(a_e))), qa.kappa3));
      rs.push_back(fe_mul(r, range_sep));
    }
    if (key->has_logic) {
      const Fr two = fe_dbl(one), three = fe_add(two, one), four = fe_dbl(two);
      auto delta = [&](const Fr& f) {
        return fe_mul(fe_mul(f, fe_sub(f, one)), fe_mul(fe_sub(f, two), fe_sub(f, three)));
      };
      const Fr qa_ = fe_sub(an_e, fe_mul(four, a_e));
      const Fr qb_ = fe_sub(bn_e, fe_mul(four, b_e));
      const Fr qd_ = fe_sub(dn_e, fe_mul(four, d_e));
      Fr r = delta(qa_);
      r = fe_add(r, fe_mul(delta(qb_), qa.lk));
      r = fe_add(r, fe_mul(delta(qd_), qa.lk2));
      r = fe_add(r, fe_mul(fe_sub(c_e, fe_mul(qa_, qb_)), qa.lk3));
      r = fe_add(r, fe_mul(logic_xor_and(qa_, qb_, c_e, qd_, qc_e), qa.lk4));
      rs.push_back(fe_mul(r, logic_sep));
    }
    if (key->has_fixed) {
      const Fr w = widget_fixed_base(a_e, an_e, b_e, bn_e, c_e, d_e, dn_e, ql_e, qr_e, qc_e,
                                     qa.fk, qa.fk2, qa.fk3, qa.edwards_d);
      rs.push_back(fe_mul(w, fixed_sep));
    }
    if (key->has_var) {
      const Fr w = widget_var_base(a_e, an_e, b_e, bn_e, c_e, d_e, dn_e, qa.vk, qa.vk2,
                                   qa.edwards_d);
      rs.push_back(fe_mul(w, var_sep));
    }
    const Fr bz = fe_mul(beta, zeta);
    Fr idc = fe_mul(fe_add(fe_add(a_e, bz), gamma), fe_add(fe_add(b_e, fe_mul(K1, bz)), gamma));
    idc = fe_mul(idc, fe_add(fe_add(c_e, fe_mul(K2, bz)), gamma));
    idc = fe_mul(idc, fe_add(fe_add(d_e, fe_mul(K3, bz)), gamma));
    idc = fe_mul(idc, alpha);
    const Fr zh = fe_sub(fe_pow_u64(zeta, n), one);
    const Fr l1 = fe_mul(zh, fe_inv(fe_mul(fr_u64(n), fe_sub(zeta, one))));
    rs.push_back(fe_add(idc, fe_mul(l1, alpha2)));
    Fr cpc = fe_add(fe_add(a_e, fe_mul(beta, s1_e)), gamma);
    cpc = fe_mul(cpc, fe_add(fe_add(b_e, fe_mul(beta, s2_e)), gamma));
    cpc = fe_mul(cpc, fe_add(fe_add(c_e, fe_mul(beta, s3_e)), gamma));
    cpc = fe_mul(fe_mul(cpc, fe_mul(beta, perm_e)), alpha);
    rs.push_back(fe_neg(cpc));
    if (rs.size() != rt.size()) return PLK_E_DEVICE;
    Fr r_e = fe_zero<FrCfg>();
    for (size_t t = 0; t < rt.size(); ++t) r_e = fe_add(r_e, fe_mul(rs[t], evs[rt[t].ev]));

    const char* elabels[17] = {"a_eval", "b_eval", "c_eval", "d_eval", "a_next_eval",
                               "b_next_eval", "d_next_eval", "s_sigma_1_eval", "s_sigma_2_eval",
                               "s_sigma_3_eval", "q_arith_eval", "q_c_eval", "q_l_eval",
                               "q_r_eval", "perm_eval", "t_eval", "r_eval"};
    const Fr evals17[17] = {a_e, b_e, c_e, d_e, an_e, bn_e, dn_e, s1_e, s2_e, s3_e,
                            qar_e, qc_e, ql_e, qr_e, perm_e, t_eval, r_e};
    for (int i = 0; i < 17; ++i) tr.append_scalar(elabels[i], evals17[i]);

    const Fr v1 = tr.challenge_scalar("v_challenge");
    const Fr v2 = tr.challenge_scalar("v_challenge");
    const Fr zn = fe_pow_u64(zeta, n), z2n = fe_sqr(zn), z3n = fe_mul(z2n, zn);
    LinComb la{};
    auto lt = [&](const Fr* p, uint64_t len, const Fr& sc_) {
      la.p[la.terms] = p;
      la.len[la.terms] = len;
      la.s[la.terms] = sc_;
      ++la.terms;
    };
    if (4 + rt.size() + 7 > (size_t)kMaxTerms) return PLK_E_DEVICE;
    const uint64_t agg_len = std::max<uint64_t>(n + 3, t4_len);
    lt(tc, n, one);
    lt(tc + n, n, zn);
    lt(tc + 2 * n, n, z2n);
    lt(tc + 3 * n, t4_len, z3n);
    Fr vp = v1;
    for (size_t t = 0; t < rt.size(); ++t) lt(rt[t].p, rt[t].len, fe_mul(vp, rs[t]));
    for (int c = 0; c < 4; ++c) {
      vp = fe_mul(vp, v1);
      lt(wc + c * S, n + 2, vp);
    }
// ... 73 lines not shown
```

### dusk-plonk_amd/csrc/prover.hpp

```cpp
#pragma once
#include <map>
#include <string>
#include <vector>

#include "internal.hpp"

namespace plk {

struct BlindArgs {
  Fr r[4];
  uint32_t count;
};
constexpr int kPiDirect = 16;
struct PiDirect {
  uint64_t idx[kPiDirect];
  Fr c[kPiDirect];
  uint32_t count;
};
struct BlindBatch {
  Fr* poly[4];
  BlindArgs b[4];
  uint32_t npoly;
};

enum { SEL_QM = 0, SEL_QL, SEL_QR, SEL_QO, SEL_Q4, SEL_QC, SEL_QARITH, SEL_QRANGE, SEL_QLOGIC,
       SEL_QFIXED, SEL_QVAR, SEL_COUNTQ };

constexpr int kQBlocks = 3;

struct QuotientArgs {
  const Fr *a, *b, *c, *d, *z, *pi, *l1, *sel, *sigma, *elements;
  Fr* out;
  uint64_t nq;
  uint32_t log_blk;
  Fr g, alpha, alpha2, beta, gamma, k1, k2, k3;
  Fr range_sep, kappa, kappa2, kappa3;
  Fr logic_sep, lk, lk2, lk3, lk4;
  Fr fixed_sep, fk, fk2, fk3;
  Fr var_sep, vk, vk2;
  Fr edwards_d;
  int has_range, has_logic, has_fixed, has_var;
  Fr vh_inv[2 * kQBlocks];
  Fr rx_bg[kQBlocks], rx_beta, rx_gamma;
  Fr rx_one_w, rx_two_w, rx_three_w;
  Fr rx_kappa, rx_kappa2, rx_kappa3;
  Fr rx_alpha2;
  Fr rx_vh[2 * kQBlocks];
  Fr rx_inv32, rx_32;
};

constexpr int kMaxEval = 28;
struct EvalBatch {
  const Fr* poly[kMaxEval];
  uint64_t len[kMaxEval];
  Fr x[kMaxEval];
};

constexpr int kMaxTerms = 24;
struct LinComb {
  const Fr* p[kMaxTerms];
  uint64_t len[kMaxTerms];
  Fr s[kMaxTerms];
  uint32_t terms;
};

PLK_HD Fr logic_xor_and(const Fr& a, const Fr& b, const Fr& w, const Fr& c,
                                            const Fr& qc) {
  auto k = [](uint32_t v) {
    Fr x = fe_zero<FrCfg>();
    x.v[0] = v;
    return fe_to_mont(x);
  };
  const Fr ab = fe_add(a, b);
  Fr f = fe_sub(fe_mul(k(4), w), fe_mul(k(18), ab));
  f = fe_add(f, k(81));
  f = fe_mul(w, f);
  f = fe_add(f, fe_mul(k(18), fe_add(fe_sqr(a), fe_sqr(b))));
  f = fe_sub(f, fe_mul(k(81), ab));
  f = fe_add(f, k(83));
  f = fe_mul(w, f);
  const Fr e = fe_sub(fe_mul(k(3), fe_add(ab, c)), fe_dbl(f));
  const Fr bb = fe_mul(qc, fe_sub(fe_mul(k(9), c), fe_mul(k(3), ab)));
  return fe_add(bb, e);
}

PLK_HD Fr widget_fixed_base(const Fr& ax, const Fr& ax_n, const Fr& ay, const Fr& ay_n,
                            const Fr& xy_alpha, const Fr& acc, const Fr& acc_n,
                            const Fr& x_beta, const Fr& y_beta, const Fr& xy_beta, const Fr& k,
                            const Fr& k2, const Fr& k3, const Fr& d) {
  const Fr one = fe_one<FrCfg>();
  const Fr bit = fe_sub(acc_n, fe_dbl(acc));
  const Fr bit_consistency = fe_mul(fe_mul(bit, fe_sub(bit, one)), fe_add(bit, one));
  const Fr y_alpha = fe_add(fe_mul(fe_sqr(bit), fe_sub(y_beta, one)), one);
  const Fr x_alpha = fe_mul(x_beta, bit);
  const Fr xy_consistency = fe_mul(fe_sub(fe_mul(bit, xy_beta), xy_alpha), k);
  const Fr prod = fe_mul(fe_mul(fe_mul(xy_alpha, ax), ay), d);
  const Fr x_lhs = fe_add(ax_n, fe_mul(ax_n, prod));
  const Fr x_rhs = fe_add(fe_mul(ax, y_alpha), fe_mul(ay, x_alpha));
  const Fr y_lhs = fe_sub(ay_n, fe_mul(ay_n, prod));
  const Fr y_rhs = fe_add(fe_mul(ay, y_alpha), fe_mul(ax, x_alpha));
  Fr id = fe_add(bit_consistency, xy_consistency);
  id = fe_add(id, fe_mul(fe_sub(x_lhs, x_rhs), k2));
  id = fe_add(id, fe_mul(fe_sub(y_lhs, y_rhs), k3));
  return id;
}

PLK_HD Fr widget_var_base(const Fr& x1, const Fr& x3, const Fr& y1, const Fr& y3, const Fr& x2,
                          const Fr& y2, const Fr& x1y2, const Fr& k, const Fr& k2, const Fr& d) {
  const Fr xy_consistency = fe_sub(fe_mul(x1, y2), x1y2);
  const Fr y1x2 = fe_mul(y1, x2);
  const Fr y1y2 = fe_mul(y1, y2);
  const Fr x1x2 = fe_mul(x1, x2);
  const Fr dprod = fe_mul(fe_mul(d, x1y2), y1x2);
  const Fr x3c = fe_sub(fe_add(x1y2, y1x2), fe_add(x3, fe_mul(x3, dprod)));
  const Fr y3c = fe_sub(fe_add(y1y2, x1x2), fe_sub(y3, fe_mul(y3, dprod)));
  return fe_add(fe_add(xy_consistency, fe_mul(x3c, k)), fe_mul(y3c, k2));
}

int pk_gather_wires(const Fr* witness, const uint32_t* idx, uint64_t m, uint64_t n, Fr* out,
                    hipStream_t s);
int pk_blind(Fr* poly, uint64_t n, const BlindArgs& b, hipStream_t s);
int pk_blind_batch(const BlindBatch& bb, uint64_t n, hipStream_t s);
int pk_pi_coef(const PiDirect& pd, const Fr* tw_inv, uint64_t n, Fr* out, hipStream_t s);
int pk_fill(Fr* out, const Fr& v, uint64_t n, hipStream_t s);
int pk_perm_numden(const Fr* wires, const Fr* sigmas, const Fr* elements, uint64_t n,
                   const Fr& beta, const Fr& gamma, const Fr& k1, const Fr& k2, const Fr& k3,
                   Fr* num, Fr* den, hipStream_t s);
int pk_mul3(const Fr* a, const Fr* b, const Fr& c, Fr* out, uint64_t n, hipStream_t s);
uint64_t pk_scan_tmp_elems(uint64_t n);
int pk_scan(const Fr* in, Fr* out, uint64_t n, bool mul, bool suffix, bool exclusive, Fr* tmp,
            hipStream_t s);
int pk_quotient(const QuotientArgs& q, hipStream_t s);
int pk_coset3_combine(const Fr* in, uint64_t n2, const Fr* comb, Fr* out, hipStream_t s);
int pk_scale_copy(const Fr* in, const Fr& c, Fr* out, uint64_t n, hipStream_t s);
uint32_t pk_eval_max_blocks(uint64_t max_len);
int pk_eval(const EvalBatch& e, uint32_t count, uint64_t max_len, Fr* partial, Fr* d_out,
            hipStream_t s);
int pk_lincomb(const LinComb& lc, Fr* out, uint64_t len_out, hipStream_t s);
int pk_scale_powers(const Fr* c, uint64_t len, const Fr& x, uint64_t shift, Fr* y, hipStream_t s);
int pk_ruffini(const Fr* c, uint64_t len, const Fr& z, Fr* q, Fr* tmp, Fr* scan_tmp,
               hipStream_t s);

struct Gate {
  Fr q[11];
  uint32_t w[4];
  bool has_pi;
  Fr pi;
};

enum : uint32_t { kSelZero = 0, kSelOne = 1, kSelMinusOne = 2, kSelPooled = 3 };
constexpr uint32_t kPiBit = 1u << 22;
struct GateRec {
  uint32_t w[4];
  uint32_t code;
  uint32_t ext;
};
inline uint32_t sel_code(uint32_t code, int q) { return (code >> (2 * q)) & 3u; }

}

struct plk_composer {
  std::vector<plk::Fr> witness;
  std::vector<plk::GateRec> gates;
  std::vector<plk::Fr> consts;
  static constexpr uint32_t kNoWire = 0xffffffffu;
  std::vector<uint32_t> wire_head, wire_tail, wire_next;
  static constexpr uint64_t kHashInit = 0x6a09e667f3bcc908ull;
  uint64_t struct_hash = kHashInit;
};

struct plk_key {
  plk_ctx* ctx = nullptr;
  plk_srs* srs = nullptr;
  std::string label;
  uint64_t m = 0, n = 0, n_trim = 0;
  uint32_t k = 0;
  plk_domain* dom = nullptr;
  plk_domain* domq = nullptr;
  bool has_range = false, has_logic = false, has_fixed = false, has_var = false;
  plk::DevBuf q_coef;
  plk::DevBuf selq;
  plk::DevBuf sigma_coef;
  plk::DevBuf sigma_lag;
  plk::DevBuf sigmaq;
  plk::DevBuf l1q;
  plk::DevBuf coset_s, coset_w, coset_pi;
  plk::DevBuf icoset_q;
  plk::Fr s_m[plk::kQBlocks];
  plk::Fr comb[6];
  plk::DevBuf wire_idx;
  plk::Fr vh_inv[2 * plk::kQBlocks];
  plk_g1 comms[15];
  uint64_t struct_hash = 0;
  uint32_t max_wire = 0;
  std::mutex def_mu;
  std::unique_ptr<plk_prover> def_prover;
  ~plk_key();
};

struct plk_prover {
  plk_key* key = nullptr;
  hipStream_t stream = nullptr;
  bool own_stream = false;
  plk::MsmWorkspace* ws = nullptr;
  plk_srs* shard = nullptr;
  uint64_t shard_lo = 0;
  bool shard_buckets = false;
  int rank = 0, world = 1;
  plk_allgather_fn allgather = nullptr;
  void* allgather_user = nullptr;
  plk::PinnedBuf pin_witness, pin_small;
  plk::PinnedBuf eval_out;
  void* eval_dev = nullptr;
  plk::DevBuf witness, wires_lag, wires_coef, z_lag, z_coef, num, den, tmp_a, scan_tmp, pi_lag,
      pi_coef, evq, quotq, t_coef, agg, agg2, w_coef, eval_partial, ntt_scratch;
  ~plk_prover();
};
```

### dusk-plonk_amd/csrc/prover_kernels.hip

```cpp
#include <hip/hip_runtime.h>

#include "ffr.hpp"
#include "internal.hpp"
#include "prover.hpp"

namespace plk {

namespace {

__device__ __forceinline__ Fr ldf(const Fr* p) {
  const uint4* q = reinterpret_cast<const uint4*>(p);
  uint4 a = q[0], b = q[1];
  Fr r;
  r.v[0] = a.x; r.v[1] = a.y; r.v[2] = a.z; r.v[3] = a.w;
  r.v[4] = b.x; r.v[5] = b.y; r.v[6] = b.z; r.v[7] = b.w;
  return r;
}

__device__ __forceinline__ void stf(Fr* p, const Fr& v) {
  uint4* q = reinterpret_cast<uint4*>(p);
  q[0] = make_uint4(v.v[0], v.v[1], v.v[2], v.v[3]);
  q[1] = make_uint4(v.v[4], v.v[5], v.v[6], v.v[7]);
}

using RFr = Rx<FrCfg>;
__device__ __forceinline__ RFr ldr(const Fr* p) { return rx_unpack(ldf(p)); }

__device__ __forceinline__ RFr add3_u(const RFr& a, const RFr& b, const RFr& c) {
  RFr r;
#pragma unroll
  for (int l = 0; l < RxShape<FrCfg>::L; ++l) r.v[l] = a.v[l] + b.v[l] + c.v[l];
  return r;
}

__device__ __forceinline__ RFr rx_norm(const RFr& a) {
  constexpr uint32_t B = RxShape<FrCfg>::B, MASK = (1u << B) - 1;
  RFr r;
  uint32_t c = 0;
#pragma unroll
  for (int l = 0; l < RxShape<FrCfg>::L; ++l) {
    const uint32_t t = a.v[l] + c;
    r.v[l] = l == RxShape<FrCfg>::L - 1 ? t : (t & MASK);
    c = t >> B;
  }
  return r;
}

inline uint32_t blocks_for(uint64_t n, uint32_t bs) { return (uint32_t)((n + bs - 1) / bs); }

__global__ void k_gather_wires(const Fr* __restrict__ witness, const uint32_t* __restrict__ idx,
                               uint64_t m, uint64_t n, Fr* __restrict__ out) {
  const uint64_t i = (uint64_t)blockIdx.x * blockDim.x + threadIdx.x;
  const uint32_t col = blockIdx.y;
  if (i >= n) return;
  stf(&out[col * n + i], i < m ? ldf(&witness[idx[col * n + i]]) : fe_zero<FrCfg>());
}

__global__ void k_blind(Fr* __restrict__ poly, uint64_t n, BlindArgs b) {
  const uint32_t i = threadIdx.x;
  if (i >= b.count) return;
  stf(&poly[i], fe_sub(ldf(&poly[i]), b.r[i]));
  stf(&poly[n + i], b.r[i]);
}

__global__ void k_pi_coef(PiDirect pd, const Fr* __restrict__ tw_inv, uint64_t n,
                          Fr* __restrict__ out) {
  const uint64_t j = (uint64_t)blockIdx.x * blockDim.x + threadIdx.x;
  if (j >= n) return;
  RFr acc = rx_zero<FrCfg>();
  for (uint32_t k = 0; k < pd.count; ++k)
    acc = rx_add(acc, rx_mul(rx_unpack(pd.c[k]), ldr(&tw_inv[(pd.idx[k] * j) & (n - 1)])));
  stf(&out[j], rx_pack_canonical(acc));
}

__global__ void k_blind_batch(BlindBatch bb, uint64_t n) {
  const uint32_t p = threadIdx.x >> 2, i = threadIdx.x & 3;
  if (p >= bb.npoly || i >= bb.b[p].count) return;
  Fr* poly = bb.poly[p];
  stf(&poly[i], fe_sub(ldf(&poly[i]), bb.b[p].r[i]));
  stf(&poly[n + i], bb.b[p].r[i]);
}

__global__ void k_fill(Fr* __restrict__ out, Fr v, uint64_t n) {
  const uint64_t i = (uint64_t)blockIdx.x * blockDim.x + threadIdx.x;
  if (i < n) stf(&out[i], v);
}

__global__ void k_perm_numden(const Fr* __restrict__ wires, const Fr* __restrict__ sigmas,
                              const Fr* __restrict__ elements, uint64_t n, Fr beta_rx, Fr gamma,
                              Fr k1_rx, Fr k2_rx, Fr k3_rx, Fr fix, Fr* __restrict__ num,
                              Fr* __restrict__ den) {
  const uint64_t i = (uint64_t)blockIdx.x * blockDim.x + threadIdx.x;
  if (i >= n) return;
  const RFr be = rx_unpack(beta_rx), g = rx_unpack(gamma);
  const RFr bx = rx_mul(be, ldr(&elements[i]));
  auto tn = [&](int c, const RFr& bxk) { return add3_u(ldr(&wires[c * n + i]), g, bxk); };
  auto td = [&](int c) { return add3_u(ldr(&wires[c * n + i]), g, rx_mul(be, ldr(&sigmas[c * n + i]))); };
  RFr nu = rx_norm(tn(0, bx)), de = rx_norm(td(0));
  nu = rx_mul(nu, tn(1, rx_mul(rx_unpack(k1_rx), bx)));
  de = rx_mul(de, td(1));
  nu = rx_mul(nu, tn(2, rx_mul(rx_unpack(k2_rx), bx)));
  de = rx_mul(de, td(2));
  nu = rx_mul(nu, tn(3, rx_mul(rx_unpack(k3_rx), bx)));
  de = rx_mul(de, td(3));
  const RFr f = rx_unpack(fix);
  stf(&num[i], rx_pack_canonical(rx_mul(nu, f)));
  stf(&den[i], rx_pack_canonical(rx_mul(de, f)));
}

__global__ void k_mul3(const Fr* __restrict__ a, const Fr* __restrict__ b, Fr c,
                       Fr* __restrict__ out, uint64_t n) {
  const uint64_t i = (uint64_t)blockIdx.x * blockDim.x + threadIdx.x;
  if (i < n) stf(&out[i], fe_mul(fe_mul(ldf(&a[i]), ldf(&b[i])), c));
}

constexpr uint32_t kScanThreads = 256, kScanPer = 8, kScanBlock = kScanThreads * kScanPer;

template <bool MUL>
__device__ __forceinline__ Fr op(const Fr& a, const Fr& b) {
  return MUL ? fe_mul(a, b) : fe_add(a, b);
}
template <bool MUL>
__device__ __forceinline__ Fr ident() {
  return MUL ? fe_one<FrCfg>() : fe_zero<FrCfg>();
}

template <bool SUFFIX>
__device__ __forceinline__ uint64_t phys(uint64_t j, uint64_t n) {
  return SUFFIX ? n - 1 - j : j;
}

template <bool MUL, bool SUFFIX>
__global__ void __launch_bounds__(kScanThreads) k_scan_reduce(const Fr* __restrict__ in, uint64_t n,
                                                              Fr* __restrict__ tot) {
  __shared__ Fr sh[kScanThreads];
  const uint64_t base = (uint64_t)blockIdx.x * kScanBlock + threadIdx.x * kScanPer;
  Fr acc = ident<MUL>();
  for (uint32_t k = 0; k < kScanPer; ++k)
    if (base + k < n) acc = op<MUL>(acc, ldf(&in[phys<SUFFIX>(base + k, n)]));
  sh[threadIdx.x] = acc;
  __syncthreads();
  for (uint32_t h = kScanThreads / 2; h >= 1; h >>= 1) {
    if (threadIdx.x < h) sh[threadIdx.x] = op<MUL>(sh[threadIdx.x], sh[threadIdx.x + h]);
    __syncthreads();
  }
  if (threadIdx.x == 0) stf(&tot[blockIdx.x], sh[0]);
}

template <bool MUL>
__global__ void __launch_bounds__(kScanThreads) k_scan_tops(Fr* __restrict__ tot, uint32_t nb) {
  __shared__ Fr sh[kScanThreads];
  const uint32_t per = (nb + kScanThreads - 1) / kScanThreads;
  const uint32_t b0 = threadIdx.x * per;
  Fr acc = ident<MUL>();
  for (uint32_t b = b0; b < b0 + per && b < nb; ++b) acc = op<MUL>(acc, ldf(&tot[b]));
  sh[threadIdx.x] = acc;
  __syncthreads();
  for (uint32_t off = 1; off < kScanThreads; off <<= 1) {
    Fr v = threadIdx.x >= off ? sh[threadIdx.x - off] : ident<MUL>();
    __syncthreads();
    sh[threadIdx.x] = op<MUL>(sh[threadIdx.x], v);
    __syncthreads();
  }
  Fr run = threadIdx.x ? sh[threadIdx.x - 1] : ident<MUL>();
  for (uint32_t b = b0; b < b0 + per && b < nb; ++b) {
    const Fr v = ldf(&tot[b]);
    stf(&tot[b], run);
    run = op<MUL>(run, v);
  }
  if (threadIdx.x == kScanThreads - 1) stf(&tot[nb], sh[kScanThreads - 1]);
}

constexpr uint32_t kScanSingleThreads = 1024, kScanSingleMax = 32 * kScanSingleThreads;
constexpr uint32_t kScanSingleWaves = kScanSingleThreads / 64;
__device__ __forceinline__ Fr shfl_up_fr(const Fr& v, uint32_t h) {
  Fr o;
#pragma unroll
  for (int k = 0; k < 8; ++k) o.v[k] = (uint32_t)__shfl_up((int)v.v[k], h, 64);
  return o;
}
template <bool MUL>
__device__ __forceinline__ Fr wave_scan_incl(Fr v, uint32_t lane) {
#pragma unroll
  for (uint32_t h = 1; h < 64; h <<= 1) {
    const Fr o = shfl_up_fr(v, h);
    if (lane >= h) v = op<MUL>(o, v);
  }
  return v;
}
template <bool MUL, bool SUFFIX, bool EXCL>
__global__ void __launch_bounds__(kScanSingleThreads) k_scan_single(const Fr* __restrict__ in,
                                                                    uint64_t n, Fr* __restrict__ out,
                                                                    Fr* __restrict__ tot, uint32_t nb) {
  __shared__ Fr sh[kScanSingleWaves];
  const uint32_t tid = threadIdx.x, lane = tid & 63, wave = tid >> 6;
  const uint32_t per = (uint32_t)((n + kScanSingleThreads - 1) / kScanSingleThreads);
  const uint64_t base = (uint64_t)tid * per;
  Fr acc = ident<MUL>();
  for (uint32_t k = 0; k < per && base + k < n; ++k) acc = op<MUL>(acc, ldf(&in[phys<SUFFIX>(base + k, n)]));
  const Fr incl = wave_scan_incl<MUL>(acc, lane);
  if (lane == 63) sh[wave] = incl;
  __syncthreads();
  if (wave == 0) {
    const Fr w = lane < kScanSingleWaves ? sh[lane] : ident<MUL>();
    const Fr wi = wave_scan_incl<MUL>(w, lane);
    const Fr we = shfl_up_fr(wi, 1);
    if (lane < kScanSingleWaves) sh[lane] = lane ? we : ident<MUL>();
    if (lane == kScanSingleWaves - 1) stf(&tot[nb], wi);
  }
  __syncthreads();
  const Fr excl_in_wave = shfl_up_fr(incl, 1);
  Fr run = lane ? (wave ? op<MUL>(sh[wave], excl_in_wave) : excl_in_wave)
                : (wave ? sh[wave] : ident<MUL>());
  for (uint32_t k = 0; k < per && base + k < n; ++k) {
    const uint64_t p = phys<SUFFIX>(base + k, n);
    const Fr v = ldf(&in[p]);
    if (EXCL) {
      stf(&out[p], run);
      run = op<MUL>(run, v);
    } else {
      run = op<MUL>(run, v);
      stf(&out[p], run);
    }
  }
}

template <bool MUL, bool SUFFIX, bool EXCL>
__global__ void __launch_bounds__(kScanThreads) k_scan_apply(const Fr* __restrict__ in, uint64_t n,
                                                             const Fr* __restrict__ tot,
                                                             Fr* __restrict__ out) {
  __shared__ Fr sh[kScanThreads];
  const uint64_t base = (uint64_t)blockIdx.x * kScanBlock + threadIdx.x * kScanPer;
  Fr acc = ident<MUL>();
  for (uint32_t k = 0; k < kScanPer; ++k)
    if (base + k < n) acc = op<MUL>(acc, ldf(&in[phys<SUFFIX>(base + k, n)]));
  sh[threadIdx.x] = acc;
  __syncthreads();
  for (uint32_t off = 1; off < kScanThreads; off <<= 1) {
    Fr v = threadIdx.x >= off ? sh[threadIdx.x - off] : ident<MUL>();
    __syncthreads();
    sh[threadIdx.x] = op<MUL>(sh[threadIdx.x], v);
    __syncthreads();
  }
  Fr run = op<MUL>(ldf(&tot[blockIdx.x]), threadIdx.x ? sh[threadIdx.x - 1] : ident<MUL>());
  for (uint32_t k = 0; k < kScanPer; ++k) {
    if (base + k >= n) break;
    const uint64_t p = phys<SUFFIX>(base + k, n);
    const Fr v = ldf(&in[p]);
    if (EXCL) {
      stf(&out[p], run);
      run = op<MUL>(run, v);
    } else {
      run = op<MUL>(run, v);
      stf(&out[p], run);
    }
  }
}

template <bool FINAL>
__global__ void __launch_bounds__(256) __attribute__((amdgpu_waves_per_eu(3, 3))) k_quotient(QuotientArgs q) {
  const uint64_t i = (uint64_t)blockIdx.x * blockDim.x + threadIdx.x;
  const uint64_t N = q.nq;
  if (i >= N) return;
  const uint64_t blk = i >> q.log_blk, u = i & ((1ull << q.log_blk) - 1);
  const uint64_t nx = (blk << q.log_blk) + ((u + 2) & ((1ull << q.log_blk) - 1));
  const RFr a = ldr(&q.a[i]), b = ldr(&q.b[i]), c = ldr(&q.c[i]), d = ldr(&q.d[i]);
  const RFr z = ldr(&q.z[i]), z_next = ldr(&q.z[nx]);
  RFr t = rx_mul(ldr(&q.sel[SEL_QM * N + i]), rx_mul(a, b));
  const RFr lr = rx_mul_add(ldr(&q.sel[SEL_QL * N + i]), a, ldr(&q.sel[SEL_QR * N + i]), b);
  const RFr o4 = rx_mul_add(ldr(&q.sel[SEL_QO * N + i]), c, ldr(&q.sel[SEL_Q4 * N + i]), d);
  const RFr qc = ldr(&q.sel[SEL_QC * N + i]);
#pragma unroll
  for (int l = 0; l < RxShape<FrCfg>::L; ++l) t.v[l] += lr.v[l] + o4.v[l] + qc.v[l];
  t = rx_mul(ldr(&q.sel[SEL_QARITH * N + i]), t);
  if (q.pi) t = rx_add(t, ldr(&q.pi[i]));
  if (q.has_range) {
    const RFr qr = ldr(&q.sel[SEL_QRANGE * N + i]);
    if (!rx_is_zero(qr)) {
      const RFr d_next = ldr(&q.d[nx]);
      const RFr one = rx_unpack(q.rx_one_w), two = rx_unpack(q.rx_two_w),
                three = rx_unpack(q.rx_three_w);
      auto delta = [&](const RFr& f) {
        return rx_mul(rx_mul(f, rx_sub(f, one)), rx_mul(rx_sub(f, two), rx_sub(f, three)));
      };
      auto four = [](const RFr& x) { return rx_dbl(rx_dbl(x)); };
      RFr r = delta(rx_sub(c, four(d)));
      r = rx_add(r, rx_mul(delta(rx_sub(b, four(c))), rx_unpack(q.rx_kappa)));
      r = rx_add(r, rx_mul(delta(rx_sub(a, four(b))), rx_unpack(q.rx_kappa2)));
      r = rx_add(r, rx_mul(delta(rx_sub(d_next, four(a))), rx_unpack(q.rx_kappa3)));
      t = rx_add(t, rx_mul(rx_mul(r, qr), rx_unpack(q.range_sep)));
    }
  }
  const RFr bX = rx_mul(rx_unpack(q.rx_bg[blk]), ldr(&q.elements[u]));
  const RFr bX2 = rx_dbl(bX), bX4 = rx_dbl(bX2), bX8 = rx_dbl(bX4), bX16 = rx_dbl(bX8);
  const RFr bX7 = rx_sub(bX8, bX), bX13 = rx_add(rx_add(bX8, bX4), bX), bX17 = rx_add(bX16, bX);
  const RFr gm = rx_unpack(q.rx_gamma);
  RFr id = rx_mul(rx_norm(add3_u(a, bX, gm)), add3_u(b, bX7, gm));
  id = rx_mul(id, add3_u(c, bX13, gm));
  id = rx_mul(id, add3_u(d, bX17, gm));
  id = rx_mul(id, z);
  const RFr be = rx_unpack(q.rx_beta);
  RFr cp = rx_norm(add3_u(a, rx_mul(be, ldr(&q.sigma[0 * N + i])), gm));
  cp = rx_mul(cp, add3_u(b, rx_mul(be, ldr(&q.sigma[1 * N + i])), gm));
  cp = rx_mul(cp, add3_u(c, rx_mul(be, ldr(&q.sigma[2 * N + i])), gm));
  cp = rx_mul(cp, add3_u(d, rx_mul(be, ldr(&q.sigma[3 * N + i])), gm));
  cp = rx_mul(cp, z_next);
  const RFr zm1l1 = rx_mul(rx_sub_u<FrCfg, 3>(z, rx_unpack(fe_one<FrCfg>())), ldr(&q.l1[i]));
  const RFr perm = rx_mul_add(rx_sub_u<FrCfg, 3>(id, cp), rx_unpack(q.alpha), zm1l1,
                              rx_unpack(q.rx_alpha2));
  if (FINAL) {
    RFr num = t;
#pragma unroll
    for (int l = 0; l < RxShape<FrCfg>::L; ++l) num.v[l] += perm.v[l];
    stf(&q.out[i], rx_pack_canonical(rx_mul(num, rx_unpack(q.rx_vh[2 * blk + (u & 1)]))));
  } else {
    stf(&q.out[i], rx_pack_canonical(rx_add(t, perm)));
  }
}

__global__ void __launch_bounds__(256) k_quotient_ext(QuotientArgs q) {
  const uint64_t i = (uint64_t)blockIdx.x * blockDim.x + threadIdx.x;
  const uint64_t N = q.nq;
  if (i >= N) return;
  const uint64_t blk = i >> q.log_blk, u = i & ((1ull << q.log_blk) - 1);
  const uint64_t nx = (blk << q.log_blk) + ((u + 2) & ((1ull << q.log_blk) - 1));
  auto ldw = [&](const Fr* p) { return fe_mul(ldf(p), q.rx_inv32); };
  const Fr a = ldw(&q.a[i]), b = ldw(&q.b[i]), c = ldw(&q.c[i]), d = ldw(&q.d[i]);
  Fr t = fe_mul(ldf(&q.out[i]), q.rx_32);
  if (q.has_logic) {
    const Fr ql = ldf(&q.sel[SEL_QLOGIC * N + i]);
    if (!fe_is_zero(ql)) {
      const Fr one = fe_one<FrCfg>();
      const Fr two = fe_dbl(one), three = fe_add(two, one), four = fe_dbl(two);
      auto delta = [&](const Fr& f) {
        return fe_mul(fe_mul(f, fe_sub(f, one)), fe_mul(fe_sub(f, two), fe_sub(f, three)));
      };
      const Fr qa = fe_sub(ldw(&q.a[nx]), fe_mul(four, a));
      const Fr qb = fe_sub(ldw(&q.b[nx]), fe_mul(four, b));
      const Fr qd = fe_sub(ldw(&q.d[nx]), fe_mul(four, d));
      const Fr qc = ldf(&q.sel[SEL_QC * N + i]);
      Fr r = delta(qa);
      r = fe_add(r, fe_mul(delta(qb), q.lk));
      r = fe_add(r, fe_mul(delta(qd), q.lk2));
      r = fe_add(r, fe_mul(fe_sub(c, fe_mul(qa, qb)), q.lk3));
      r = fe_add(r, fe_mul(logic_xor_and(qa, qb, c, qd, qc), q.lk4));
      t = fe_add(t, fe_mul(fe_mul(r, ql), q.logic_sep));
    }
  }
  if (q.has_fixed) {
    const Fr qf = ldf(&q.sel[SEL_QFIXED * N + i]);
    if (!fe_is_zero(qf)) {
      const Fr w = widget_fixed_base(a, ldw(&q.a[nx]), b, ldw(&q.b[nx]), c, d, ldw(&q.d[nx]),
                                     ldf(&q.sel[SEL_QL * N + i]), ldf(&q.sel[SEL_QR * N + i]),
                                     ldf(&q.sel[SEL_QC * N + i]), q.fk, q.fk2, q.fk3, q.edwards_d);
      t = fe_add(t, fe_mul(fe_mul(w, qf), q.fixed_sep));
    }
  }
  if (q.has_var) {
    const Fr qv = ldf(&q.sel[SEL_QVAR * N + i]);
    if (!fe_is_zero(qv)) {
      const Fr w = widget_var_base(a, ldw(&q.a[nx]), b, ldw(&q.b[nx]), c, d, ldw(&q.d[nx]),
                                   q.vk, q.vk2, q.edwards_d);
      t = fe_add(t, fe_mul(fe_mul(w, qv), q.var_sep));
    }
  }
  stf(&q.out[i], fe_mul(t, q.vh_inv[2 * blk + (u & 1)]));
}

__global__ void __launch_bounds__(256) k_coset3_combine(const Fr* __restrict__ in, uint64_t n2,
                                                        Fr c1a, Fr c1b, Fr c1c, Fr c2a, Fr c2b,
                                                        Fr c2c, Fr* __restrict__ out) {
  const uint64_t k = (uint64_t)blockIdx.x * blockDim.x + threadIdx.x;
  if (k >= n2) return;
  const RFr b0 = ldr(&in[k]), b1 = ldr(&in[n2 + k]), b2 = ldr(&in[2 * n2 + k]);
  stf(&out[k], rx_pack_canonical(rx_add(rx_add(b0, b1), b2)));
  const RFr e1 = rx_add(rx_mul_add(b0, rx_unpack(c1a), b1, rx_unpack(c1b)), rx_mul(b2, rx_unpack(c1c)));
  stf(&out[n2 + k], rx_pack_canonical(e1));
  const RFr e2 = rx_add(rx_mul_add(b0, rx_unpack(c2a), b1, rx_unpack(c2b)), rx_mul(b2, rx_unpack(c2c)));
  stf(&out[2 * n2 + k], rx_pack_canonical(e2));
}

__global__ void k_scale_copy(const Fr* __restrict__ in, Fr c, Fr* __restrict__ out, uint64_t n) {
  const uint64_t j = (uint64_t)blockIdx.x * blockDim.x + threadIdx.x;
  if (j < n) stf(&out[j], fe_mul(ldf(&in[j]), c));
}

constexpr uint32_t kEvalThreads = 256, kEvalPer = 16, kEvalBlock = kEvalThreads * kEvalPer;

__device__ __forceinline__ Fr pow_blocks(Fr x4096, uint64_t b) {
  Fr r = fe_one<FrCfg>();
  for (; b; b >>= 1) {
    if (b & 1) r = fe_mul(r, x4096);
    x4096 = fe_sqr(x4096);
  }
  return r;
}

__device__ __forceinline__ RFr pow_blocks_rx(RFr x4096, uint64_t b) {
  RFr r = rx_one<FrCfg>();
  for (; b; b >>= 1) {
    if (b & 1) r = rx_mul(r, x4096);
    x4096 = rx_sqr(x4096);
  }
  return r;
}

__global__ void __launch_bounds__(kEvalThreads) k_eval_partial(EvalBatch e, Fr* __restrict__ partial,
                                                               uint32_t max_blocks) {
  __shared__ Fr sh[kEvalThreads];
  __shared__ Fr xp[9];
  __shared__ Fr xblock;
  const uint32_t k = blockIdx.y, tid = threadIdx.x;
  const Fr* p = e.poly[k];
  const uint64_t len = e.len[k];
  const uint64_t block0 = (uint64_t)blockIdx.x * kEvalBlock;
  if (block0 >= len) {
    if (tid == 0) stf(&partial[(size_t)k * max_blocks + blockIdx.x], fe_zero<FrCfg>());
    return;
  }
  if (tid == 0) {
    RFr t = rx_unpack(e.x[k]);
    for (int l = 0; l < 9; ++l) {
      xp[l] = rx_pack(t);
      t = rx_sqr(t);
    }
    for (int l = 9; l < 12; ++l) t = rx_sqr(t);
    xblock = rx_pack(pow_blocks_rx(t, blockIdx.x));
  }
  __syncthreads();
  const RFr x256 = rx_unpack(xp[8]);
  RFr acc = rx_zero<FrCfg>();
#pragma unroll
  for (int i = (int)kEvalPer - 1; i >= 0; --i) {
    const uint64_t j = block0 + tid + (uint64_t)i * kEvalThreads;
    acc = rx_mul(acc, x256);
    if (j < len) acc = rx_add(acc, ldr(&p[j]));
  }
  sh[tid] = rx_pack(acc);
  __syncthreads();
  for (int l = 7; l >= 0; --l) {
    const uint32_t h = 1u << l;
    if (tid < h)
      sh[tid] = rx_pack(rx_add(rx_unpack(sh[tid]), rx_mul(rx_unpack(sh[tid + h]), rx_unpack(xp[l]))));
    __syncthreads();
  }
  if (tid == 0)
    stf(&partial[(size_t)k * max_blocks + blockIdx.x],
        rx_pack_canonical(rx_mul(rx_unpack(sh[0]), rx_unpack(xblock))));
}

__global__ void __launch_bounds__(kEvalThreads) k_eval_final(const Fr* __restrict__ partial,
                                                             uint32_t nblocks, uint32_t max_blocks,
                                                             Fr* __restrict__ out) {
  __shared__ Fr sh[kEvalThreads];
  const uint32_t k = blockIdx.x;
  Fr acc = fe_zero<FrCfg>();
  for (uint32_t b = threadIdx.x; b < nblocks; b += kEvalThreads)
    acc = fe_add(acc, ldf(&partial[(size_t)k * max_blocks + b]));
  sh[threadIdx.x] = acc;
  __syncthreads();
  for (uint32_t h = kEvalThreads / 2; h >= 1; h >>= 1) {
    if (threadIdx.x < h) sh[threadIdx.x] = fe_add(sh[threadIdx.x], sh[threadIdx.x + h]);
    __syncthreads();
  }
  if (threadIdx.x == 0) stf(&out[k], sh[0]);
}

constexpr uint32_t kRuffiniThreads = 1024, kRuffiniSingleMax = 16 * kRuffiniThreads;
static_assert(kRuffiniThreads == 32 * 32, "start powers: t = 32 hi + lo");
struct RuffiniPow {
  Fr up[10];
  Fr dn[10];
};
__global__ void __launch_bounds__(kRuffiniThreads) k_ruffini_single(const Fr* __restrict__ c, uint64_t len,
                                                                    uint32_t E, Fr z, Fr zi,
                                                                    RuffiniPow pw2, Fr* __restrict__ q) {
  __shared__ Fr P[4][32];
  __shared__ Fr W[kRuffiniThreads / 64];
  const uint32_t tid = threadIdx.x;
  if (tid < 128) {
    const uint32_t tb = tid >> 5, i = tid & 31;
    RFr v = rx_one<FrCfg>();
#pragma unroll
    for (int b = 0; b < 5; ++b) {
      Fr f;
#pragma unroll
      for (int k = 0; k < 8; ++k)
        f.v[k] = tb < 2 ? (tb == 0 ? pw2.up[b].v[k] : pw2.up[b + 5].v[k])
                        : (tb == 2 ? pw2.dn[b].v[k] : pw2.dn[b + 5].v[k]);
      const RFr m = rx_mul(v, rx_unpack(f));
      if ((i >> b) & 1) v = m;
    }
    P[tb][i] = rx_pack(v);
  }
  __syncthreads();
  const uint64_t j0 = (uint64_t)tid * E;
  const uint64_t j1 = j0 + E < len ? j0 + E : (j0 < len ? len : j0);
  const RFr zr = rx_unpack(z), zir = rx_unpack(zi);
  RFr pw = rx_mul(rx_unpack(P[0][tid & 31]), rx_unpack(P[1][tid >> 5]));
  RFr pwi = rx_mul(rx_mul(zir, rx_unpack(P[2][tid & 31])), rx_unpack(P[3][tid >> 5]));
  Fr loc = fe_zero<FrCfg>(), ylast = fe_zero<FrCfg>();
  for (uint64_t j = j0; j < j1; ++j) {
    const Fr y = rx_pack_canonical(rx_mul(ldr(&c[j]), pw));
    loc = fe_add(loc, y);
    if (j + 1 < len) stf(&q[j], y);
    else ylast = y;
    pw = rx_mul(pw, zr);
    pwi = rx_mul(pwi, zir);
  }
  Fr v = loc;
  const uint32_t lane = tid & 63, wave = tid >> 6;
#pragma unroll
  for (uint32_t h = 1; h < 64; h <<= 1) {
    Fr o;
#pragma unroll
    for (int k = 0; k < 8; ++k) o.v[k] = (uint32_t)__shfl_down((int)v.v[k], h, 64);
    if (lane + h < 64) v = fe_add(v, o);
  }
  if (lane == 0) W[wave] = v;
  __syncthreads();
  Fr run = fe_sub(v, loc);
  for (uint32_t w = wave + 1; w < kRuffiniThreads / 64; ++w) run = fe_add(run, W[w]);
  for (uint64_t k = j1; k-- > j0;) {
    pwi = rx_mul(pwi, zr);
    const bool in_q = k + 1 < len;
    const Fr yk = in_q ? ldf(&q[k]) : ylast;
    if (in_q) stf(&q[k], rx_pack_canonical(rx_mul(rx_unpack(run), pwi)));
    run = fe_add(run, yk);
  }
}

__global__ void k_lincomb(LinComb lc, Fr* __restrict__ out, uint64_t len_out) {
  const uint64_t j = (uint64_t)blockIdx.x * blockDim.x + threadIdx.x;
  if (j >= len_out) return;
  RFr acc = rx_zero<FrCfg>();
  for (uint32_t t = 0; t < lc.terms; ++t)
    if (j < lc.len[t]) acc = rx_add(acc, rx_mul(rx_unpack(lc.s[t]), ldr(&lc.p[t][j])));
  stf(&out[j], rx_pack_canonical(acc));
}

__global__ void __launch_bounds__(256) k_scale_powers(const Fr* __restrict__ c, uint64_t len, Fr x,
                                                      Fr x16, Fr x4096, Fr xshift,
                                                      Fr* __restrict__ y) {
  __shared__ Fr T[256];
  const uint32_t tid = threadIdx.x;
  const uint64_t jb = (uint64_t)blockIdx.x * 256 * 16;
  RFr v = rx_unpack(x16);
  if (tid == 0) v = rx_mul(pow_blocks_rx(rx_unpack(x4096), blockIdx.x), rx_unpack(xshift));
  T[tid] = rx_pack(v);
  __syncthreads();
  for (uint32_t h = 1; h < 256; h <<= 1) {
    const RFr o = tid >= h ? rx_unpack(T[tid - h]) : rx_one<FrCfg>();
    __syncthreads();
    if (tid >= h) T[tid] = rx_pack(rx_mul(rx_unpack(T[tid]), o));
    __syncthreads();
  }
  const uint64_t j0 = jb + (uint64_t)tid * 16;
  if (j0 >= len) return;
  RFr pw = rx_unpack(T[tid]);
  const RFr xr = rx_unpack(x);
  const uint64_t j1 = j0 + 16 < len ? j0 + 16 : len;
  for (uint64_t j = j0; j < j1; ++j) {
    stf(&y[j], rx_pack_canonical(rx_mul(ldr(&c[j]), pw)));
    pw = rx_mul(pw, xr);
  }
}

}

int pk_gather_wires(const Fr* witness, const uint32_t* idx, uint64_t m, uint64_t n, Fr* out,
                    hipStream_t s) {
  hipLaunchKernelGGL(k_gather_wires, dim3(blocks_for(n, 256), 4), dim3(256), 0, s, witness, idx, m,
                     n, out);
  PLK_HIP_TRY(hipGetLastError());
  return PLK_OK;
}

int pk_blind(Fr* poly, uint64_t n, const BlindArgs& b, hipStream_t s) {
  hipLaunchKernelGGL(k_blind, dim3(1), dim3(64), 0, s, poly, n, b);
  PLK_HIP_TRY(hipGetLastError());
  return PLK_OK;
}

int pk_pi_coef(const PiDirect& pd, const Fr* tw_inv, uint64_t n, Fr* out, hipStream_t s) {
  if (pd.count > (uint32_t)kPiDirect || (n & (n - 1))) return PLK_E_ARG;
  hipLaunchKernelGGL(k_pi_coef, dim3(blocks_for(n, 256)), dim3(256), 0, s, pd, tw_inv, n, out);
  PLK_HIP_TRY(hipGetLastError());
  return PLK_OK;
}

int pk_blind_batch(const BlindBatch& bb, uint64_t n, hipStream_t s) {
  hipLaunchKernelGGL(k_blind_batch, dim3(1), dim3(64), 0, s, bb, n);
  PLK_HIP_TRY(hipGetLastError());
  return PLK_OK;
}

int pk_fill(Fr* out, const Fr& v, uint64_t n, hipStream_t s) {
  hipLaunchKernelGGL(k_fill, dim3(blocks_for(n, 256)), dim3(256), 0, s, out, v, n);
  PLK_HIP_TRY(hipGetLastError());
  return PLK_OK;
}

int pk_perm_numden(const Fr* wires, const Fr* sigmas, const Fr* elements, uint64_t n,
                   const Fr& beta, const Fr& gamma, const Fr& k1, const Fr& k2, const Fr& k3,
                   Fr* num, Fr* den, hipStream_t s) {
  Fr fix = fe_zero<FrCfg>();
  fix.v[0] = 1;
  for (int b = 0; b < 4 * RxShape<FrCfg>::B * RxShape<FrCfg>::L - 3 * 256; ++b) fix = fe_dbl(fix);
  hipLaunchKernelGGL(k_perm_numden, dim3(blocks_for(n, 256)), dim3(256), 0, s, wires, sigmas,
                     elements, n, fe_to_rx_domain(beta), gamma, fe_to_rx_domain(k1),
                     fe_to_rx_domain(k2), fe_to_rx_domain(k3), fix, num, den);
  PLK_HIP_TRY(hipGetLastError());
  return PLK_OK;
}

int pk_mul3(const Fr* a, const Fr* b, const Fr& c, Fr* out, uint64_t n, hipStream_t s) {
  hipLaunchKernelGGL(k_mul3, dim3(blocks_for(n, 256)), dim3(256), 0, s, a, b, c, out, n);
  PLK_HIP_TRY(hipGetLastError());
  return PLK_OK;
}

uint64_t pk_scan_tmp_elems(uint64_t n) { return (n + kScanBlock - 1) / kScanBlock + 1; }

int pk_scan(const Fr* in, Fr* out, uint64_t n, bool mul, bool suffix, bool exclusive, Fr* tmp,
            hipStream_t s) {
  if (n == 0) return PLK_OK;
  const uint32_t nb = (uint32_t)((n + kScanBlock - 1) / kScanBlock);
  const bool single = n <= kScanSingleMax;
#define SCAN3(M, S, E)                                                                           \
  do {                                                                                           \
    if (single) {                                                                                \
      hipLaunchKernelGGL((k_scan_single<M, S, E>), dim3(1), dim3(kScanSingleThreads), 0, s, in, n, \
                         out, tmp, nb);                                                          \
      break;                                                                                     \
    }                                                                                            \
    hipLaunchKernelGGL((k_scan_reduce<M, S>), dim3(nb), dim3(kScanThreads), 0, s, in, n, tmp);   \
    hipLaunchKernelGGL((k_scan_tops<M>), dim3(1), dim3(kScanThreads), 0, s, tmp, nb);            \
    hipLaunchKernelGGL((k_scan_apply<M, S, E>), dim3(nb), dim3(kScanThreads), 0, s, in, n, tmp,   \
                       out);                                                                     \
  } while (0)
  if (mul) {
    if (suffix) {
      if (exclusive) SCAN3(true, true, true); else SCAN3(true, true, false);
    } else {
      if (exclusive) SCAN3(true, false, true); else SCAN3(true, false, false);
    }
  } else {
    if (suffix) {
      if (exclusive) SCAN3(false, true, true); else SCAN3(false, true, false);
    } else {
      if (exclusive) SCAN3(false, false, true); else SCAN3(false, false, false);
    }
  }
#undef SCAN3
  PLK_HIP_TRY(hipGetLastError());
  return PLK_OK;
}

int pk_coset3_combine(const Fr* in, uint64_t n2, const Fr* comb, Fr* out, hipStream_t s) {
  hipLaunchKernelGGL(k_coset3_combine, dim3(blocks_for(n2, 256)), dim3(256), 0, s, in, n2, comb[0],
                     comb[1], comb[2], comb[3], comb[4], comb[5], out);
  PLK_HIP_TRY(hipGetLastError());
  return PLK_OK;
}

int pk_quotient(const QuotientArgs& q, hipStream_t s) {
  const dim3 grid(blocks_for(q.nq, 256));
  if (q.has_logic || q.has_fixed || q.has_var) {
    hipLaunchKernelGGL((k_quotient<false>), grid, dim3(256), 0, s, q);
    hipLaunchKernelGGL(k_quotient_ext, grid, dim3(256), 0, s, q);
  } else {
    hipLaunchKernelGGL((k_quotient<true>), grid, dim3(256), 0, s, q);
  }
  PLK_HIP_TRY(hipGetLastError());
  return PLK_OK;
}

uint32_t pk_eval_max_blocks(uint64_t max_len) {
  return (uint32_t)((max_len + kEvalBlock - 1) / kEvalBlock);
}

int pk_scale_copy(const Fr* in, const Fr& c, Fr* out, uint64_t n, hipStream_t s) {
  if (n == 0) return PLK_OK;
  hipLaunchKernelGGL(k_scale_copy, dim3(blocks_for(n, 256)), dim3(256), 0, s, in, c, out, n);
  PLK_HIP_TRY(hipGetLastError());
  return PLK_OK;
}

int pk_eval(const EvalBatch& e, uint32_t count, uint64_t max_len, Fr* partial, Fr* d_out,
            hipStream_t s) {
  const uint32_t mb = pk_eval_max_blocks(max_len ? max_len : 1);
  EvalBatch er = e;
  for (uint32_t k = 0; k < count; ++k) er.x[k] = fe_to_rx_domain(e.x[k]);
  hipLaunchKernelGGL(k_eval_partial, dim3(mb, count), dim3(kEvalThreads), 0, s, er, partial, mb);
  hipLaunchKernelGGL(k_eval_final, dim3(count), dim3(kEvalThreads), 0, s, partial, mb, mb, d_out);
  PLK_HIP_TRY(hipGetLastError());
  return PLK_OK;
}

int pk_lincomb(const LinComb& lc, Fr* out, uint64_t len_out, hipStream_t s) {
  if (len_out == 0) return PLK_OK;
  LinComb lr = lc;
  for (uint32_t t = 0; t < lc.terms; ++t) lr.s[t] = fe_to_rx_domain(lc.s[t]);
  hipLaunchKernelGGL(k_lincomb, dim3(blocks_for(len_out, 256)), dim3(256), 0, s, lr, out, len_out);
  PLK_HIP_TRY(hipGetLastError());
  return PLK_OK;
}

int pk_scale_powers(const Fr* c, uint64_t len, const Fr& x, uint64_t shift, Fr* y, hipStream_t s) {
  if (len == 0) return PLK_OK;
  Fr x16 = x;
  for (int i = 0; i < 4; ++i) x16 = fe_sqr(x16);
  Fr x4096 = x16;
  for (int i = 0; i < 8; ++i) x4096 = fe_sqr(x4096);
  const Fr xshift = fe_pow_u64(x, shift);
  hipLaunchKernelGGL(k_scale_powers, dim3(blocks_for((len + 15) / 16, 256)), dim3(256), 0, s, c, len,
                     fe_to_rx_domain(x), fe_to_rx_domain(x16), fe_to_rx_domain(x4096),
                     fe_to_rx_domain(xshift), y);
  PLK_HIP_TRY(hipGetLastError());
  return PLK_OK;
}

int pk_ruffini(const Fr* c, uint64_t len, const Fr& z, Fr* q, Fr* tmp, Fr* scan_tmp,
               hipStream_t s) {
  if (len <= 1) return PLK_OK;
  int st;
  if (len <= kRuffiniSingleMax) {
    const uint32_t E = (uint32_t)((len + kRuffiniThreads - 1) / kRuffiniThreads);
    const Fr zinv = fe_inv(z);
    RuffiniPow pw2;
    Fr up = fe_pow_u64(z, E), dn = fe_pow_u64(zinv, E);
    for (int b = 0; b < 10; ++b) {
      pw2.up[b] = fe_to_rx_domain(up);
      pw2.dn[b] = fe_to_rx_domain(dn);
      up = fe_sqr(up);
      dn = fe_sqr(dn);
    }
    hipLaunchKernelGGL(k_ruffini_single, dim3(1), dim3(kRuffiniThreads), 0, s, c, len, E,
                       fe_to_rx_domain(z), fe_to_rx_domain(zinv), pw2, q);
    PLK_HIP_TRY(hipGetLastError());
    return PLK_OK;
  }
  if ((st = pk_scale_powers(c, len, z, 0, tmp, s))) return st;
  if ((st = pk_scan(tmp, tmp, len, false, true, true, scan_tmp, s))) return st;
  const Fr zinv = fe_inv(z);
  return pk_scale_powers(tmp, len - 1, zinv, 1, q, s);
}

}
```

### dusk-plonk_amd/plonk.py

```python
from __future__ import annotations

import ctypes as C
import os
from pathlib import Path

import numpy as np

_PKG = Path(__file__).resolve().parent
_LIB_PATH = Path(os.environ["PLK_LIB"]) if os.environ.get("PLK_LIB") else _PKG / "libplk.so"

PLK_OK, PLK_E_DEGREE, PLK_E_ARG, PLK_E_DEVICE, PLK_E_OOM, PLK_E_NODEV = range(6)

ABI_SYMBOLS = (
    "plk_abi_version", "plk_status_str", "plk_build_info", "plk_device_count", "plk_ctx_create",
    "plk_ctx_destroy", "plk_ctx_stream", "plk_ctx_synchronize", "plk_domain_get",
    "plk_domain_info", "plk_domain_elements", "plk_domain_vanishing_over_coset", "plk_ntt",
    "plk_ntt_dev", "plk_ntt_batch_dev", "plk_srs_setup", "plk_srs_load", "plk_srs_destroy",
    "plk_srs_len", "plk_srs_points", "plk_msm", "plk_commit", "plk_commit_dev",
    "plk_srs_last_msm_stats", "plk_debug_field_op", "plk_debug_rx_op", "plk_debug_g1r_op",
    "plk_commit_batch_dev",
    "plk_commit_batch_dev_part",
    "plk_srs_setup_range", "plk_g1_sum", "plk_msm_sharded", "plk_srs_msm_stats_reset",
    "plk_srs_cum_msm_stats", "plk_ntt_stream", "plk_aggregate_witness",
    "plk_aggregate_witness_dev",
    "plk_composer_create", "plk_composer_destroy", "plk_composer_size",
    "plk_composer_append_witness", "plk_composer_witness_value", "plk_composer_set_witness",
    "plk_composer_append_public", "plk_composer_append_gate", "plk_composer_append_custom_gate",
    "plk_composer_gate_eval", "plk_composer_assert_equal", "plk_composer_assert_equal_constant",
    "plk_composer_component_boolean", "plk_composer_component_range",
    "plk_composer_synthetic_chain",
    "plk_composer_public_inputs", "plk_composer_export", "plk_key_compile", "plk_key_destroy",
    "plk_key_info",
    "plk_prove", "plk_prover_create", "plk_prover_destroy", "plk_prover_stream",
    "plk_prover_prove", "plk_prover_msm_stats", "plk_prover_shard", "plk_prover_shard_buckets",
    "plk_proof_encode", "plk_proof_decode",
)


class PlonkError(RuntimeError):
    def __init__(self, status: int, what: str = ""):
        self.status = status
        msg = _lib().plk_status_str(status).decode() if _LIB is not None else str(status)
        super().__init__(f"{what}: {msg} (status {status})" if what else msg)


_LIB = None


def _lib():
    global _LIB
    if _LIB is None:
        if not _LIB_PATH.exists():
            raise ImportError(f"{_LIB_PATH} not built — run __graft_entry__.build() first")
        try:
            import torch
        except Exception:
            pass
        lib = C.CDLL(str(_LIB_PATH))
        vp, u32, u64, sz, i32 = C.c_void_p, C.c_uint32, C.c_uint64, C.c_size_t, C.c_int
        pp = C.POINTER(C.c_void_p)
        sig = {
            "plk_abi_version": (i32, []),
            "plk_status_str": (C.c_char_p, [i32]),
            "plk_build_info": (C.c_char_p, []),
            "plk_device_count": (i32, [C.POINTER(i32)]),
            "plk_ctx_create": (i32, [i32, pp]),
            "plk_ctx_destroy": (i32, [vp]),
            "plk_ctx_stream": (i32, [vp, pp]),
            "plk_ctx_synchronize": (i32, [vp]),
            "plk_domain_get": (i32, [vp, u32, pp]),
            "plk_domain_info": (i32, [vp, C.POINTER(u64), vp, vp, vp, vp, vp]),
            "plk_domain_elements": (i32, [vp, vp]),
            "plk_domain_vanishing_over_coset": (i32, [vp, u64, vp]),
            "plk_ntt": (i32, [vp, vp, sz, i32, i32]),
            "plk_ntt_dev": (i32, [vp, vp, vp, sz, i32, i32, vp, vp]),
            "plk_ntt_stream": (i32, [vp, vp, sz, i32, i32, vp]),
            "plk_aggregate_witness": (i32, [vp, vp, vp, sz, vp, vp, vp, C.POINTER(sz)]),
            "plk_aggregate_witness_dev": (i32, [vp, vp, vp, sz, vp, vp, vp, C.POINTER(sz), vp]),
            "plk_ntt_batch_dev": (i32, [vp, vp, sz, i32, i32, vp]),
            "plk_srs_setup": (i32, [vp, vp, sz, vp, pp]),
            "plk_srs_load": (i32, [vp, vp, sz, pp]),
            "plk_srs_destroy": (i32, [vp]),
            "plk_srs_len": (i32, [vp, C.POINTER(sz)]),
            "plk_srs_points": (i32, [vp, sz, sz, vp]),
            "plk_msm": (i32, [vp, vp, sz, vp]),
            "plk_commit": (i32, [vp, vp, sz, vp]),
            "plk_commit_dev": (i32, [vp, vp, sz, vp, vp]),
            "plk_srs_last_msm_stats": (i32, [vp, C.POINTER(C.c_float), C.POINTER(u64),
                                             C.POINTER(u32)]),
            "plk_debug_field_op": (i32, [vp, i32, i32, vp, vp, vp, sz]),
            "plk_debug_rx_op": (i32, [vp, i32, i32, vp, vp, vp, vp, vp, sz]),
            "plk_debug_g1r_op": (i32, [vp, i32, vp, vp, vp, vp, sz]),
            "plk_commit_batch_dev": (i32, [vp, vp, vp, sz, vp, vp, vp]),
            "plk_commit_batch_dev_part": (i32, [vp, vp, vp, sz, u32, u32, vp, vp, vp]),
            "plk_srs_setup_range": (i32, [vp, vp, u64, sz, vp, pp]),
            "plk_g1_sum": (i32, [vp, sz, vp]),
            "plk_msm_sharded": (i32, [vp, i32, vp, sz, vp]),
            "plk_srs_msm_stats_reset": (i32, [vp]),
            "plk_srs_cum_msm_stats": (i32, [vp, C.POINTER(C.c_double), C.POINTER(u64),
                                            C.POINTER(u64), C.POINTER(u64)]),
        }
        for name, (res, args) in sig.items():
            f = getattr(lib, name)
            f.restype, f.argtypes = res, args
        _LIB = lib
    return _LIB


def build_info() -> dict:
    raw = _lib().plk_build_info().decode()
    d = dict(kv.split("=", 1) for kv in raw.split())
    d["lib"] = str(_LIB_PATH)
    return d


def check_build(root: Path | None = None) -> dict:
    import importlib.util
    spec = importlib.util.spec_from_file_location("_plk_build_ext", _PKG / "build_ext.py")
    be = importlib.util.module_from_spec(spec)
    spec.loader.exec_module(be)
    info = build_info()
    tree_src = be.source_id(root or be.ROOT)
    info["tree_src"] = tree_src
    if os.environ.get("PLK_LIB") and os.environ.get("PLK_LIB_ANY_SRC") == "1":
        info["src_check"] = "skipped (PLK_LIB variant with PLK_LIB_ANY_SRC=1: an A/B against another tree)"
        return info
    if info.get("src") != tree_src:
        raise ImportError(f"{_LIB_PATH} was built from other sources (library src={info.get('src')}, "
                          f"tree src={tree_src}): rebuild with __graft_entry__.build()")
    if not os.environ.get("PLK_LIB") and info.get("flags") != be.flags_id():
        raise ImportError(f"{_LIB_PATH} was built with other flags (library flags={info.get('flags')}, "
                          f"default flags={be.flags_id()}): rebuild with __graft_entry__.build()")
    return info


def _check(status: int, what: str):
    if status != PLK_OK:
        raise PlonkError(status, what)


def _ptr(a: np.ndarray):
    return a.ctypes.data_as(C.c_void_p)


def device_count() -> int:
    n = C.c_int(0)
    _check(_lib().plk_device_count(C.byref(n)), "plk_device_count")
    return n.value


class Context:

    _default: dict[int, "Context"] = {}

    def __init__(self, device: int = 0):
        h = C.c_void_p()
        _check(_lib().plk_ctx_create(device, C.byref(h)), "plk_ctx_create")
        self.handle = h
        self.device = device
        self._domains: dict[int, C.c_void_p] = {}

    @classmethod
    def default(cls, device: int | None = None) -> "Context":
        if device is None:
            device = int(os.environ.get("LOCAL_RANK", "0")) if "LOCAL_RANK" in os.environ else 0
            try:
                import torch
                if torch.cuda.is_available():
                    device = torch.cuda.current_device()
            except Exception:
                pass
        if device not in cls._default:
            cls._default[device] = Context(device)
        return cls._default[device]

    def stream(self) -> int:
        s = C.c_void_p()
        _check(_lib().plk_ctx_stream(self.handle, C.byref(s)), "plk_ctx_stream")
        return s.value or 0

    def synchronize(self):
        _check(_lib().plk_ctx_synchronize(self.handle), "plk_ctx_synchronize")

    def field_op(self, field: str, op: str, a: np.ndarray, b: np.ndarray | None = None):
        w = 4 if field == "fr" else 6
        a = np.ascontiguousarray(np.asarray(a, dtype=np.uint64).reshape(-1, w))
        bb = None if b is None else np.ascontiguousarray(np.asarray(b, dtype=np.uint64).reshape(-1, w))
        out = np.zeros_like(a)
        code = {"mul": 0, "add": 1, "sub": 2, "sqr": 3, "inv": 4}[op]
        _check(_lib().plk_debug_field_op(self.handle, 0 if field == "fr" else 1, code, _ptr(a),
                                         None if bb is None else _ptr(bb), _ptr(out), a.shape[0]),
               "plk_debug_field_op")
        return out

    RX_OPS = {"mul": (0, 2, 1), "sqr": (1, 1, 1), "mul_add": (2, 4, 1), "mul2": (3, 4, 2),
              "mul2_asm": (4, 4, 2), "sqr2": (5, 2, 2), "sqr2_asm": (6, 2, 2),
              "mul_add_mul2": (7, 4, 3), "mul_add_mul2_asm": (8, 4, 3), "mul3": (9, 4, 3),
              "add": (10, 2, 1), "sub": (11, 2, 1), "sub_lazy": (12, 2, 1), "sub2_n6": (13, 3, 1),
              "small_mul2": (14, 1, 1), "small_mul3": (15, 1, 1), "canon": (16, 1, 1),
              "is_zero": (17, 1, 1), "is_zero_u": (18, 1, 1), "unpack_pack": (19, 1, 2),
              "sub_u": (100, 2, 1), "sub_n": (200, 2, 1)}
    G1R_OPS = {"madd_000": 0, "madd_100": 1, "madd_110": 2, "madd_111": 3, "madd_lazy": 4,
               "add_lazy": 5, "add_quad": 6, "dbl_lazy": 7, "lazy_finish": 8, "add": 9,
               "add_affine": 10, "dbl": 11, "dbl_affine": 12}

    def rx_op(self, field: str, op: str, *rows, cp: int = 0) -> np.ndarray:
        L = 9 if field == "fr" else 13
        code, nin, nout = self.RX_OPS[op]
        if len(rows) != nin:
            raise ValueError(f"rx_op {op} takes {nin} operand arrays")
        ops = [np.ascontiguousarray(np.asarray(r, dtype=np.uint32).reshape(-1, L)) for r in rows]
        n = ops[0].shape[0]
        if any(o.shape[0] != n for o in ops):
            raise ValueError("rx_op operands differ in length")
        out = np.zeros((n, nout, L), dtype=np.uint32)
        ptrs = [_ptr(o) for o in ops] + [None] * (4 - nin)
        _check(_lib().plk_debug_rx_op(self.handle, 0 if field == "fr" else 1, code + cp, *ptrs,
                                      _ptr(out), n), "plk_debug_rx_op")
        return out

    def g1r_op(self, op: str, p, q=None, flags=None) -> np.ndarray:
        p = np.ascontiguousarray(np.asarray(p, dtype=np.uint32).reshape(-1, 4, 13))
        n = p.shape[0]
        if q is not None:
            q = np.ascontiguousarray(np.asarray(q, dtype=np.uint32).reshape(-1, 4, 13))
        if flags is not None:
            flags = np.ascontiguousarray(np.asarray(flags, dtype=np.uint32).reshape(-1))
        if any(x is not None and x.shape[0] != n for x in (q, flags)):
            raise ValueError("g1r_op operands differ in length")
        out = np.zeros((n, 4, 4, 13) if op == "add_quad" else (n, 4, 13), dtype=np.uint32)
        _check(_lib().plk_debug_g1r_op(self.handle, self.G1R_OPS[op], _ptr(p),
                                       None if q is None else _ptr(q),
                                       None if flags is None else _ptr(flags), _ptr(out), n),
               "plk_debug_g1r_op")
        return out

    def domain(self, k: int) -> C.c_void_p:
        if k not in self._domains:
            d = C.c_void_p()
            _check(_lib().plk_domain_get(self.handle, k, C.byref(d)), "plk_domain_get")
            self._domains[k] = d
        return self._domains[k]


def _as_fr_array(values) -> np.ndarray:
# ... 269 lines not shown
```

### include/plk.h

```cpp
#ifndef PLK_H
#define PLK_H

#include <stddef.h>
#include <stdint.h>

#ifdef __cplusplus
extern "C" {
#endif

#define PLK_ABI_VERSION 2

typedef struct { uint64_t l[4]; } plk_fr;
typedef struct { uint64_t x[6]; uint64_t y[6]; uint64_t infinity; } plk_g1;

typedef enum {
  PLK_OK = 0,
  PLK_E_DEGREE = 1,
  PLK_E_ARG = 2,
  PLK_E_DEVICE = 3,
  PLK_E_OOM = 4,
  PLK_E_NODEV = 5,
  PLK_E_UNSUPPORTED = 6
} plk_status;

typedef struct plk_ctx plk_ctx;
typedef struct plk_domain plk_domain;
typedef struct plk_srs plk_srs;
typedef struct plk_composer plk_composer;
typedef struct plk_key plk_key;

int plk_abi_version(void);
const char* plk_status_str(int status);
const char* plk_build_info(void);
int plk_device_count(int* out);
int plk_ctx_create(int device, plk_ctx** out);
int plk_ctx_destroy(plk_ctx* ctx);
int plk_ctx_stream(plk_ctx* ctx, void** stream_out);
int plk_ctx_synchronize(plk_ctx* ctx);

int plk_domain_get(plk_ctx* ctx, uint32_t log_n, plk_domain** out);
int plk_domain_info(const plk_domain* d, uint64_t* size, plk_fr* generator,
                    plk_fr* generator_inv, plk_fr* size_inv, plk_fr* coset, plk_fr* coset_inv);
int plk_domain_elements(const plk_domain* d, plk_fr* out);
int plk_domain_vanishing_over_coset(const plk_domain* d, uint64_t poly_degree, plk_fr* out);

int plk_ntt(plk_domain* d, plk_fr* inout, size_t len_in, int dir, int coset);
int plk_ntt_stream(plk_domain* d, plk_fr* inout, size_t len_in, int dir, int coset, void* stream);
int plk_ntt_dev(plk_domain* d, const plk_fr* d_in, plk_fr* d_out, size_t len_in, int dir,
                int coset, plk_fr* d_scratch, void* stream);
int plk_ntt_batch_dev(plk_domain* d, plk_fr* d_inout, size_t count, int dir, int coset,
                      void* stream);

int plk_srs_setup(plk_ctx* ctx, const plk_fr* tau, size_t n_points, plk_g1* out_points,
                  plk_srs** out);
int plk_srs_setup_range(plk_ctx* ctx, const plk_fr* tau, uint64_t start, size_t n_points,
                        plk_g1* out_points, plk_srs** out);
int plk_srs_load(plk_ctx* ctx, const plk_g1* points, size_t n_points, plk_srs** out);
int plk_srs_destroy(plk_srs* srs);
int plk_srs_len(const plk_srs* srs, size_t* n_points);
int plk_srs_points(const plk_srs* srs, size_t start, size_t count, plk_g1* out);

int plk_msm(plk_srs* srs, const plk_fr* scalars, size_t len, plk_g1* out);
int plk_commit(plk_srs* srs, const plk_fr* coeffs, size_t len, plk_g1* out);
int plk_commit_dev(plk_srs* srs, const plk_fr* d_coeffs, size_t len, plk_g1* out,
                   void* stream);

int plk_commit_batch_dev(plk_srs* srs, const plk_fr* const* d_coeffs, const size_t* lens,
                         size_t count, plk_g1* outs, int* statuses, void* stream);

int plk_commit_batch_dev_part(plk_srs* srs, const plk_fr* const* d_coeffs, const size_t* lens,
                              size_t count, uint32_t part, uint32_t parts, plk_g1* outs,
                              int* statuses, void* stream);

int plk_aggregate_witness_dev(plk_ctx* ctx, const plk_fr* const* d_polys, const size_t* lens,
                              size_t count, const plk_fr* point, const plk_fr* v,
                              plk_fr* d_out, size_t* out_len, void* stream);
int plk_aggregate_witness(plk_ctx* ctx, const plk_fr* const* polys, const size_t* lens,
                          size_t count, const plk_fr* point, const plk_fr* v, plk_fr* out,
                          size_t* out_len);

int plk_g1_sum(const plk_g1* points, size_t n, plk_g1* out);

int plk_msm_sharded(plk_srs* const* per_gpu, int n_gpu, const plk_fr* scalars, size_t len,
                    plk_g1* out);

int plk_srs_last_msm_stats(const plk_srs* srs, float* accumulate_ms, uint64_t* point_adds,
                           uint32_t* window_bits);
int plk_srs_msm_stats_reset(plk_srs* srs);
int plk_srs_cum_msm_stats(const plk_srs* srs, double* accumulate_ms, uint64_t* launches,
                          uint64_t* point_adds, uint64_t* points);

typedef struct {
  plk_fr q_m, q_l, q_r, q_o, q_4, q_c, q_arith, q_range, q_logic, q_fixed_group_add,
      q_variable_group_add;
  uint32_t a, b, o, d;
  uint32_t has_public, _pad;
  plk_fr public_input;
} plk_constraint;

typedef struct {
  plk_g1 a_comm, b_comm, c_comm, d_comm, z_comm, t_low_comm, t_mid_comm, t_high_comm, t_4_comm,
      w_z_chall_comm, w_z_chall_w_comm;
  plk_fr a_eval, b_eval, c_eval, d_eval, a_next_eval, b_next_eval, d_next_eval, q_arith_eval,
      q_c_eval, q_l_eval, q_r_eval, s_sigma_1_eval, s_sigma_2_eval, s_sigma_3_eval, r_poly_eval,
      perm_eval;
} plk_proof;

int plk_composer_create(plk_composer** out);
int plk_composer_destroy(plk_composer* c);
int plk_composer_size(const plk_composer* c, size_t* gates, size_t* witnesses);
int plk_composer_append_witness(plk_composer* c, const plk_fr* value, uint32_t* wire);
int plk_composer_witness_value(const plk_composer* c, uint32_t wire, plk_fr* value);
int plk_composer_set_witness(plk_composer* c, uint32_t wire, const plk_fr* value);
int plk_composer_append_public(plk_composer* c, const plk_fr* value, uint32_t* wire);
int plk_composer_append_gate(plk_composer* c, const plk_constraint* s);
int plk_composer_append_custom_gate(plk_composer* c, const plk_constraint* s);
int plk_composer_gate_eval(plk_composer* c, const plk_constraint* s, uint32_t* out_wire);
int plk_composer_assert_equal(plk_composer* c, uint32_t a, uint32_t b);
int plk_composer_assert_equal_constant(plk_composer* c, uint32_t a, const plk_fr* constant,
                                       const plk_fr* public_input );
int plk_composer_component_boolean(plk_composer* c, uint32_t a);
int plk_composer_component_range(plk_composer* c, uint32_t a, size_t num_bits);
int plk_composer_synthetic_chain(plk_composer* c, size_t gates, uint64_t seed);
int plk_composer_public_inputs(const plk_composer* c, plk_fr* values, uint64_t* indexes,
                               size_t cap, size_t* count);
int plk_composer_export(const plk_composer* c, plk_constraint* gates, size_t cap,
                        plk_fr* witness, size_t wcap, size_t* m, size_t* nw);

int plk_key_compile(plk_srs* srs, const plk_composer* circuit, const char* label, plk_key** out);
int plk_key_destroy(plk_key* key);
int plk_key_info(const plk_key* key, uint64_t* n, uint64_t* m, plk_g1* commitments);
int plk_prove(plk_key* key, const plk_composer* circuit, uint64_t seed, plk_proof* proof,
              plk_fr* public_inputs, size_t pi_cap, size_t* pi_count);

typedef struct plk_prover plk_prover;
int plk_prover_create(plk_key* key, plk_prover** out);
int plk_prover_destroy(plk_prover* p);
int plk_prover_stream(plk_prover* p, void** stream_out);
int plk_prover_prove(plk_prover* p, const plk_composer* circuit, uint64_t seed, plk_proof* proof,
                     plk_fr* public_inputs, size_t pi_cap, size_t* pi_count);
int plk_prover_msm_stats(plk_prover* p, int reset, double* accumulate_ms, uint64_t* launches,
                         uint64_t* point_adds, uint64_t* points);

typedef int (*plk_allgather_fn)(void* user, const void* send, size_t bytes, void* recv);
int plk_prover_shard(plk_prover* p, plk_srs* slice, uint64_t slice_start, int rank, int world,
                     plk_allgather_fn allgather, void* user);
int plk_prover_shard_buckets(plk_prover* p, int rank, int world, plk_allgather_fn allgather,
                             void* user);

#define PLK_PROOF_SCALE_BYTES (11 * 97 + 16 * 32)
int plk_proof_encode(const plk_proof* proof, uint8_t* out, size_t cap, size_t* len);
int plk_proof_decode(const uint8_t* in, size_t len, plk_proof* proof);

int plk_debug_field_op(plk_ctx* ctx, int field, int op, const uint64_t* a, const uint64_t* b,
                       uint64_t* out, size_t n);
int plk_debug_rx_op(plk_ctx* ctx, int field, int op, const uint32_t* a, const uint32_t* b,
                    const uint32_t* c, const uint32_t* d, uint32_t* out, size_t n);
int plk_debug_g1r_op(plk_ctx* ctx, int op, const uint32_t* p, const uint32_t* q,
                     const uint32_t* flags, uint32_t* out, size_t n);

#ifdef __cplusplus
}
#endif
#endif
```

Baseline: 32.29 million.

## Evaluate quotient on five size-n cosets instead of three double-size cosets

Changes the quotient evaluation domain from 3 cosets of size 2n to 5 (or 6 for tiny n) cosets of size n, with a general Vandermonde-inverse combine matrix for recovering coefficients. The forward coset NTT gains a fold mode that adds the wrap-around coefficients beyond n, so polynomials longer than n can be transformed on the size-n domain. Sparse public inputs are evaluated directly from shifted L1 values rather than through an extra coset NTT. Total evaluation points drop from 6n to 5n and NTTs shrink to size n, reducing quotient-stage work. The cost is more NTT launches, a larger combine kernel, and a debug entry point for checking block evaluations.

```diff
diff --git a/dusk-plonk_amd/csrc/debug.hip b/dusk-plonk_amd/csrc/debug.hip
--- a/dusk-plonk_amd/csrc/debug.hip
+++ b/dusk-plonk_amd/csrc/debug.hip
@@ -2,6 +2,7 @@
 
 #include "g1r.hpp"
 #include "internal.hpp"
+#include "prover.hpp"
 
 namespace plk {
 namespace {
@@ -325,3 +326,35 @@
     return PLK_E_DEVICE;
   }
 }
+
+extern "C" int plk_debug_block_eval(plk_key* key, const uint64_t* coef, size_t len, uint64_t* out,
+                                    size_t out_cap, int* blocks_out) {
+  using plk::last_hip_error;
+  try {
+    if (!key) return PLK_E_ARG;
+    if (blocks_out) *blocks_out = key->qb;
+    if (!out) return PLK_OK;
+    const uint64_t n = key->n, total = (uint64_t)key->qb * n;
+    if (!coef || len == 0 || len > n + 8 || out_cap < total) return PLK_E_ARG;
+    plk::DeviceGuard g(key->ctx->device);
+    hipStream_t s = key->ctx->stream;
+    plk::DevBuf din, dout;
+    int st;
+    if ((st = din.alloc(len * sizeof(plk::Fr))) || (st = dout.alloc(total * sizeof(plk::Fr))))
+      return st;
+    PLK_HIP_TRY(hipMemcpyAsync(din.ptr, coef, len * sizeof(plk::Fr), hipMemcpyHostToDevice, s));
+    plk::NttBatch b;
+    b.in_stride = 0;
+    b.out_stride = n;
+    b.pre = key->coset_s.as<plk::Fr>();
+    b.pre_stride = n + 8;
+    if ((st = plk::ntt_run_batch(key->dom, din.as<plk::Fr>(), dout.as<plk::Fr>(), len, 1, 1,
+                                 nullptr, s, (uint32_t)key->qb, b)))
+      return st;
+    PLK_HIP_TRY(hipMemcpyAsync(out, dout.ptr, total * sizeof(plk::Fr), hipMemcpyDeviceToHost, s));
+    PLK_HIP_TRY(plk::stream_wait(s));
+    return PLK_OK;
+  } catch (...) {
+    return PLK_E_DEVICE;
+  }
+}
diff --git a/dusk-plonk_amd/csrc/ntt.hip b/dusk-plonk_amd/csrc/ntt.hip
--- a/dusk-plonk_amd/csrc/ntt.hip
+++ b/dusk-plonk_amd/csrc/ntt.hip
@@ -225,7 +225,7 @@
     const uint32_t yi = str.group_in ? y % str.group_in : y, gi = str.group_in ? y / str.group_in : 0;
     in += (size_t)yi * str.in + (size_t)gi * str.in_group;
     out += (size_t)y * str.out;
-    if (PRE == 1) pre += (size_t)yi * str.pre;
+    if (PRE >= 1) pre += (size_t)yi * str.pre;
     if (POST == 2) post += (size_t)(str.group_post ? y % str.group_post : y) * str.post;
   }
 
@@ -245,9 +245,9 @@
       const size_t g = (size_t)(i0 + (e & (T - 1))) + ((size_t)(e >> lt) << nr_log);
       const size_t gc = g < len_in ? g : 0;
       raw[c] = ld_fr(&in[gc]);
-      if (PRE == 1) aux[c] = ld_fr(&pre[gc]);
-    }
-    if (PRE != 1 && lp != 0) {
+      if (PRE >= 1) aux[c] = ld_fr(&pre[gc]);
+    }
+    if (PRE == 0 && lp != 0) {
 #pragma unroll
       for (uint32_t c = 0; c < kLoadIt; ++c) {
         const uint32_t e = min(tid + c * bd, E - 1);
@@ -296,9 +296,13 @@
       RFr v = rx_zero<FrCfg>();
       if (g < len_in) {
         v = rx_unpack(raw[c]);
-        if (PRE == 1) v = rx_mul(v, rx_unpack(aux[c]));
-      }
-      if (PRE != 1 && lp != 0) v = rx_mul(v, rx_unpack(aux[c]));
+        if (PRE >= 1) v = rx_mul(v, rx_unpack(aux[c]));
+        if (PRE == 2) {
+          const size_t g2 = g + ((size_t)1 << log_n);
+          if (g2 < len_in) v = rx_add(v, rx_mul(ld_rfr(&in[g2]), ld_rfr(&pre[g2])));
+        }
+      }
+      if (PRE == 0 && lp != 0) v = rx_mul(v, rx_unpack(aux[c]));
       return v;
     };
     {
@@ -548,7 +552,9 @@
 int ntt_run_batch(plk_domain* d, const Fr* in, Fr* out, size_t len_in, int dir, int coset,
                   Fr* scratch, hipStream_t stream, uint32_t count, const NttBatch& bt) {
   const uint64_t n = d->n;
-  if (len_in > n || count == 0) return PLK_E_ARG;
+  if (count == 0) return PLK_E_ARG;
+  const bool fold = len_in > n;
+  if (fold && !(bt.pre && dir > 0 && coset && len_in <= n + 8 && n > 1)) return PLK_E_ARG;
   const Fr* pre_table = bt.pre;
   if (n == 1) {
     if (bt.pre || bt.post) return PLK_E_ARG;
@@ -589,7 +595,7 @@
     if (bd < 64) bd = 64;
     if (bd > 256) bd = 256;
     const uint32_t blocks = (uint32_t)(n >> (ps.lr + ps.lt));
-    const int pre = (first && dir > 0 && coset) ? 1 : 0;
+    const int pre = (first && dir > 0 && coset) ? (fold ? 2 : 1) : 0;
     const bool scaled_tw = last && !first && dir < 0 && !coset;
     const int post = (last && dir < 0 && !scaled_tw) ? (coset ? 2 : 1) : 0;
     const uint64_t lin = first ? len_in : n;
@@ -630,6 +636,7 @@
       else PLK_LAUNCH(0, 0, 1);
     } else if (pre == 0 && post == 0) PLK_LAUNCH(0, 0, 0);
     else if (pre == 1 && post == 0) PLK_LAUNCH(1, 0, 0);
+    else if (pre == 2) PLK_LAUNCH(2, 0, 0);
     else if (pre == 0 && post == 1) PLK_LAUNCH(0, 1, 0);
     else if (pre == 0 && post == 2) PLK_LAUNCH(0, 2, 0);
     else if (pre == 1 && post == 1) PLK_LAUNCH(1, 1, 0);
diff --git a/dusk-plonk_amd/csrc/prover.hip b/dusk-plonk_amd/csrc/prover.hip
--- a/dusk-plonk_amd/csrc/prover.hip
+++ b/dusk-plonk_amd/csrc/prover.hip
@@ -380,14 +380,6 @@
   return key_commit(P->key, *P->ws, ptrs, lens, outs, statuses, P->stream, cap);
 }
 
-Fr cube_root_of_unity() {
-  static const uint32_t w[8] = {0xffffffffu, 0x00000000u, 0x0001a402u, 0xac45a401u,
-                                0u, 0u, 0u, 0u};
-  Fr x;
-  for (int i = 0; i < 8; ++i) x.v[i] = w[i];
-  return fe_to_mont(x);
-}
-
 Fr edwards_d() {
   static const uint32_t w[8] = {0xd6343eb1u, 0x01065fd6u, 0x37579d26u, 0x292d7f6du,
                                 0xe6bd7fd4u, 0xf5fd9207u, 0x4bfa2b48u, 0x2a9318e7u};
@@ -707,8 +699,8 @@
       if (!fe_is_zero(g.q[QVAR])) key->has_var = true;
     }
     TRY(plk_domain_get(ctx, k, &key->dom));
-    TRY(plk_domain_get(ctx, k + 1, &key->domq));
-    const uint64_t n2 = 2 * n, nq = kQBlocks * n2;
+    const int QB = key->qb = q_blocks(n);
+    const uint64_t nq = (uint64_t)QB * n;
 
     std::vector<Fr> host(11 * n, fe_zero<FrCfg>());
     for (uint64_t i = 0; i < m; ++i) {
@@ -763,43 +755,55 @@
       if (sts[i] != PLK_OK) return sts[i];
 
     {
-      const Fr gq = key->domq->g, one = fe_one<FrCfg>();
-      const Fr w3 = cube_root_of_unity();
+      const Fr gq = key->dom->g, one = fe_one<FrCfg>();
+      Fr w8n;
+      fr_root_of_unity(k + 3, w8n);
       const uint64_t rowc = n + 8;
-      TRY(key->coset_s.alloc(kQBlocks * rowc * sizeof(Fr)));
-      TRY(key->coset_w.alloc(kQBlocks * rowc * sizeof(Fr)));
-      TRY(key->coset_pi.alloc(kQBlocks * rowc * sizeof(Fr)));
-      TRY(key->icoset_q.alloc(kQBlocks * n2 * sizeof(Fr)));
-      const Fr c32 = fr_u64(32), inv3 = fe_inv(fr_u64(3));
+      TRY(key->coset_s.alloc(QB * rowc * sizeof(Fr)));
+      TRY(key->coset_w.alloc(QB * rowc * sizeof(Fr)));
+      TRY(key->coset_pi.alloc(QB * rowc * sizeof(Fr)));
+      TRY(key->icoset_q.alloc(QB * n * sizeof(Fr)));
+      const Fr c32 = fr_u64(32);
       Fr sm = gq;
-      for (int mb = 0; mb < kQBlocks; ++mb) {
+      for (int mb = 0; mb < QB; ++mb) {
         key->s_m[mb] = sm;
         TRY(ntt_power_table(key->coset_s.as<Fr>() + mb * rowc, sm, one, rowc, true, s));
         TRY(ntt_power_table(key->coset_w.as<Fr>() + mb * rowc, sm, c32, rowc, true, s));
         TRY(ntt_power_table(key->coset_pi.as<Fr>() + mb * rowc, sm, fe_inv(c32), rowc, true, s));
-        TRY(ntt_power_table(key->icoset_q.as<Fr>() + mb * n2, fe_inv(sm),
-                            fe_mul(key->domq->n_inv, inv3), n2, true, s));
-        sm = fe_mul(sm, w3);
-      }
-      const Fr eta_inv = fe_inv(fe_pow_u64(w3, n2));
-      const Fr eta_inv2 = fe_sqr(eta_inv);
-      const Fr g1 = fe_inv(fe_pow_u64(gq, n2)), g2 = fe_sqr(g1);
-      const Fr cm[6] = {g1, fe_mul(g1, eta_inv), fe_mul(g1, eta_inv2),
-                        g2, fe_mul(g2, eta_inv2), fe_mul(g2, eta_inv)};
-      for (int j = 0; j < 6; ++j) key->comb[j] = fe_to_rx_domain(cm[j]);
-      for (int mb = 0; mb < kQBlocks; ++mb) {
-        const Fr x = fe_pow_u64(key->s_m[mb], n);
-        key->vh_inv[2 * mb] = fe_inv(fe_sub(x, one));
-        key->vh_inv[2 * mb + 1] = fe_inv(fe_sub(fe_neg(x), one));
+        TRY(ntt_power_table(key->icoset_q.as<Fr>() + mb * n, fe_inv(sm), key->dom->n_inv, n, true,
+                            s));
+        sm = fe_mul(sm, w8n);
+      }
+      Fr cm[kQBlocksMax];
+      for (int mb = 0; mb < QB; ++mb) {
+        cm[mb] = fe_pow_u64(key->s_m[mb], n);
+        key->vh_inv[mb] = fe_inv(fe_sub(cm[mb], one));
+      }
+      for (int mb = 0; mb < QB; ++mb) {
+        Fr poly[kQBlocksMax + 1];
+        int deg = 0;
+        poly[0] = one;
+        Fr den = one;
+        for (int j = 0; j < QB; ++j) {
+          if (j == mb) continue;
+          poly[deg + 1] = fe_zero<FrCfg>();
+          for (int l = deg + 1; l >= 1; --l)
+            poly[l] = fe_sub(poly[l - 1], fe_mul(poly[l], cm[j]));
+          poly[0] = fe_neg(fe_mul(poly[0], cm[j]));
+          ++deg;
+          den = fe_mul(den, fe_sub(cm[mb], cm[j]));
+        }
+        const Fr dinv = fe_inv(den);
+        for (int l = 0; l < QB; ++l) key->comb.m[l * QB + mb] = fe_to_rx_domain(fe_mul(poly[l], dinv));
       }
     }
     auto coset_fwd = [&](const Fr* in, Fr* out, uint64_t len, const DevBuf& table) {
       NttBatch b;
       b.in_stride = 0;
-      b.out_stride = n2;
+      b.out_stride = n;
       b.pre = table.as<Fr>();
       b.pre_stride = n + 8;
-      return ntt_run_batch(key->domq, in, out, len, 1, 1, nullptr, s, kQBlocks, b);
+      return ntt_run_batch(key->dom, in, out, len, 1, 1, nullptr, s, QB, b);
     };
     TRY(key->selq.alloc(SEL_COUNTQ * nq * sizeof(Fr)));
     const int sel_src[SEL_COUNTQ] = {QM, QL, QR, QO, Q4, QC, QARITH, QRANGE, QLOGIC, QFIXED, QVAR};
@@ -957,7 +961,8 @@
     DeviceGuard guard(key->ctx->device);
     hipStream_t s = P->stream;
     const uint64_t n = key->n, m = key->m, S = n + 8;
-    const uint64_t n2 = 2 * n, nq = kQBlocks * n2;
+    const int QB = key->qb;
+    const uint64_t nq = (uint64_t)QB * n;
     Rng rng{seed};
     const Fr one = fe_one<FrCfg>();
     const Fr K1 = fr_u64(7), K2 = fr_u64(13), K3 = fr_u64(17);
@@ -1077,7 +1082,8 @@
     const Fr var_sep = tr.challenge_scalar("variable base separation challenge");
     Fr* pil = P->pi_lag.as<Fr>();
     TRY(P->pin_small.alloc(std::max<size_t>(pis.size(), 1) * sizeof(Fr)));
-    const bool pi_direct = !pis.empty() && pis.size() <= (size_t)kPiDirect;
+    const bool pi_sparse = !pis.empty() && pis.size() <= (size_t)kPiSparse;
+    const bool pi_direct = !pis.empty() && !pi_sparse && pis.size() <= (size_t)kPiDirect;
     if (pi_direct) {
       PiDirect pd{};
       pd.count = (uint32_t)pis.size();
@@ -1086,7 +1092,7 @@
         pd.c[i] = fe_mul(pis[i].second, key->dom->n_inv);
       }
       TRY(pk_pi_coef(pd, key->dom->tw_inv.as<Fr>(), n, P->pi_coef.as<Fr>(), s));
-    } else if (!pis.empty()) {
+    } else if (!pis.empty() && !pi_sparse) {
       PLK_HIP_TRY(hipMemsetAsync(pil, 0, n * sizeof(Fr), s));
       for (size_t i = 0; i < pis.size(); ++i) {
         P->pin_small.as<Fr>()[i] = pis[i].second;
@@ -1098,25 +1104,35 @@
     auto coset_fwd = [&](const Fr* in, Fr* out, uint64_t len, const DevBuf& table) {
       NttBatch b;
       b.in_stride = 0;
-      b.out_stride = n2;
+      b.out_stride = n;
       b.pre = table.as<Fr>();
       b.pre_stride = n + 8;
-      return ntt_run_batch(key->domq, in, out, len, 1, 1, nsc, s, kQBlocks, b);
+      return ntt_run_batch(key->dom, in, out, len, 1, 1, nsc, s, QB, b);
     };
-    if (!pis.empty() && !pi_direct)
+    if (!pis.empty() && !pi_direct && !pi_sparse)
       TRY(ntt_run(key->dom, pil, P->pi_coef.as<Fr>(), n, -1, 0, nsc, s, 1));
     TRY(coset_fwd(zc, ev + 0 * nq, n + 3, key->coset_s));
     {
       NttBatch b;
-      b.group = kQBlocks;
+      b.group = QB;
       b.in_stride = 0;
       b.in_group_stride = S;
-      b.out_stride = n2;
+      b.out_stride = n;
       b.pre = key->coset_w.as<Fr>();
       b.pre_stride = n + 8;
-      TRY(ntt_run_batch(key->domq, wc, ev + nq, n + 2, 1, 1, nsc, s, 4 * kQBlocks, b));
-    }
-    if (!pis.empty()) TRY(coset_fwd(P->pi_coef.as<Fr>(), ev + 5 * nq, n, key->coset_pi));
+      TRY(ntt_run_batch(key->dom, wc, ev + nq, n + 2, 1, 1, nsc, s, 4 * QB, b));
+    }
+    if (pi_sparse) {
+      PiSparse ps{};
+      ps.count = (uint32_t)pis.size();
+      for (size_t i = 0; i < pis.size(); ++i) {
+        ps.idx[i] = (uint32_t)pis[i].first;
+        ps.v[i] = pis[i].second;
+      }
+      TRY(pk_pi_sparse(ps, key->l1q.as<Fr>(), key->k, nq, ev + 5 * nq, s));
+    } else if (!pis.empty()) {
+      TRY(coset_fwd(P->pi_coef.as<Fr>(), ev + 5 * nq, n, key->coset_pi));
+    }
     const Fr alpha2 = fe_sqr(alpha);
     QuotientArgs qa{};
     qa.z = ev;
@@ -1129,11 +1145,11 @@
     qa.alpha2 = alpha2;
     qa.sel = key->selq.as<Fr>();
     qa.sigma = key->sigmaq.as<Fr>();
-    qa.elements = key->domq->tw_fwd.as<Fr>();
+    qa.elements = key->dom->tw_fwd.as<Fr>();
     qa.out = P->quotq.as<Fr>();
     qa.nq = nq;
-    qa.log_blk = key->k + 1;
-    qa.g = key->domq->g;
+    qa.log_blk = key->k;
+    qa.g = key->dom->g;
     qa.alpha = alpha;
     qa.beta = beta;
     qa.gamma = gamma;
@@ -1161,12 +1177,12 @@
     qa.edwards_d = edwards_d();
     qa.has_fixed = key->has_fixed ? 1 : 0;
     qa.has_var = key->has_var ? 1 : 0;
-    for (int j = 0; j < 2 * kQBlocks; ++j) qa.vh_inv[j] = key->vh_inv[j];
+    for (int j = 0; j < QB; ++j) qa.vh_inv[j] = key->vh_inv[j];
     {
       auto em1 = [](const Fr& x) { return fe_to_rx_domain(x); };
       auto em2 = [](const Fr& x) { return fe_to_rx_domain(fe_to_rx_domain(x)); };
       const Fr one = fe_one<FrCfg>(), two = fe_dbl(one);
-      for (int mb = 0; mb < kQBlocks; ++mb) qa.rx_bg[mb] = em2(fe_mul(beta, key->s_m[mb]));
+      for (int mb = 0; mb < QB; ++mb) qa.rx_bg[mb] = em2(fe_mul(beta, key->s_m[mb]));
       qa.rx_beta = em2(beta);
       qa.rx_gamma = em1(gamma);
       qa.rx_one_w = em1(one);
@@ -1176,7 +1192,7 @@
       qa.rx_kappa2 = em1(qa.kappa2);
       qa.rx_kappa3 = em1(qa.kappa3);
       qa.rx_alpha2 = em1(alpha2);
-      for (int j = 0; j < 2 * kQBlocks; ++j) qa.rx_vh[j] = em2(key->vh_inv[j]);
+      for (int j = 0; j < QB; ++j) qa.rx_vh[j] = em2(key->vh_inv[j]);
       qa.rx_32 = fr_u64(32);
       qa.rx_inv32 = fe_inv(qa.rx_32);
     }
@@ -1184,12 +1200,11 @@
     Fr* tc = P->t_coef.as<Fr>();
     {
       NttBatch b;
-      b.in_stride = b.out_stride = n2;
+      b.in_stride = b.out_stride = n;
       b.post = key->icoset_q.as<Fr>();
-      b.post_stride = n2;
-      TRY(ntt_run_batch(key->domq, P->quotq.as<Fr>(), P->quotq.as<Fr>(), n2, -1, 1, nsc, s,
-                        kQBlocks, b));
-      TRY(pk_coset3_combine(P->quotq.as<Fr>(), n2, key->comb, tc, s));
+      b.post_stride = n;
+      TRY(ntt_run_batch(key->dom, P->quotq.as<Fr>(), P->quotq.as<Fr>(), n, -1, 1, nsc, s, QB, b));
+      TRY(pk_coset_combine(P->quotq.as<Fr>(), n, QB, key->comb, tc, s));
     }
     plk_g1 tcom[4];
     TRY(prover_commit(P, {tc, tc + n, tc + 2 * n, tc + 3 * n}, {n, n, n, nq - 3 * n}, tcom,
diff --git a/dusk-plonk_amd/csrc/prover.hpp b/dusk-plonk_amd/csrc/prover.hpp
--- a/dusk-plonk_amd/csrc/prover.hpp
+++ b/dusk-plonk_amd/csrc/prover.hpp
@@ -26,7 +26,14 @@
 enum { SEL_QM = 0, SEL_QL, SEL_QR, SEL_QO, SEL_Q4, SEL_QC, SEL_QARITH, SEL_QRANGE, SEL_QLOGIC,
        SEL_QFIXED, SEL_QVAR, SEL_COUNTQ };
 
-constexpr int kQBlocks = 3;
+constexpr int kQBlocks = 5, kQBlocksSmall = 6, kQBlocksMax = 6;
+inline int q_blocks(uint64_t n) { return n >= 16 ? kQBlocks : kQBlocksSmall; }
+constexpr int kPiSparse = 4;
+struct PiSparse {
+  uint32_t count;
+  uint32_t idx[kPiSparse];
+  Fr v[kPiSparse];
+};
 
 struct QuotientArgs {
   const Fr *a, *b, *c, *d, *z, *pi, *l1, *sel, *sigma, *elements;
@@ -40,12 +47,12 @@
   Fr var_sep, vk, vk2;
   Fr edwards_d;
   int has_range, has_logic, has_fixed, has_var;
-  Fr vh_inv[2 * kQBlocks];
-  Fr rx_bg[kQBlocks], rx_beta, rx_gamma;
+  Fr vh_inv[kQBlocksMax];
+  Fr rx_bg[kQBlocksMax], rx_beta, rx_gamma;
   Fr rx_one_w, rx_two_w, rx_three_w;
   Fr rx_kappa, rx_kappa2, rx_kappa3;
   Fr rx_alpha2;
-  Fr rx_vh[2 * kQBlocks];
+  Fr rx_vh[kQBlocksMax];
   Fr rx_inv32, rx_32;
 };
 
@@ -122,6 +129,8 @@
 int pk_blind(Fr* poly, uint64_t n, const BlindArgs& b, hipStream_t s);
 int pk_blind_batch(const BlindBatch& bb, uint64_t n, hipStream_t s);
 int pk_pi_coef(const PiDirect& pd, const Fr* tw_inv, uint64_t n, Fr* out, hipStream_t s);
+int pk_pi_sparse(const PiSparse& ps, const Fr* l1, uint32_t log_n, uint64_t nq, Fr* out,
+                 hipStream_t s);
 int pk_fill(Fr* out, const Fr& v, uint64_t n, hipStream_t s);
 int pk_perm_numden(const Fr* wires, const Fr* sigmas, const Fr* elements, uint64_t n,
                    const Fr& beta, const Fr& gamma, const Fr& k1, const Fr& k2, const Fr& k3,
@@ -131,7 +140,11 @@
 int pk_scan(const Fr* in, Fr* out, uint64_t n, bool mul, bool suffix, bool exclusive, Fr* tmp,
             hipStream_t s);
 int pk_quotient(const QuotientArgs& q, hipStream_t s);
-int pk_coset3_combine(const Fr* in, uint64_t n2, const Fr* comb, Fr* out, hipStream_t s);
+struct CombineMat {
+  Fr m[kQBlocksMax * kQBlocksMax];
+};
+int pk_coset_combine(const Fr* in, uint64_t n, int blocks, const CombineMat& mat, Fr* out,
+                     hipStream_t s);
 int pk_scale_copy(const Fr* in, const Fr& c, Fr* out, uint64_t n, hipStream_t s);
 uint32_t pk_eval_max_blocks(uint64_t max_len);
 int pk_eval(const EvalBatch& e, uint32_t count, uint64_t max_len, Fr* partial, Fr* d_out,
@@ -176,7 +189,7 @@
   uint64_t m = 0, n = 0, n_trim = 0;
   uint32_t k = 0;
   plk_domain* dom = nullptr;
-  plk_domain* domq = nullptr;
+  int qb = 0;
   bool has_range = false, has_logic = false, has_fixed = false, has_var = false;
   plk::DevBuf q_coef;
   plk::DevBuf selq;
@@ -186,10 +199,10 @@
   plk::DevBuf l1q;
   plk::DevBuf coset_s, coset_w, coset_pi;
   plk::DevBuf icoset_q;
-  plk::Fr s_m[plk::kQBlocks];
-  plk::Fr comb[6];
+  plk::Fr s_m[plk::kQBlocksMax];
+  plk::CombineMat comb;
   plk::DevBuf wire_idx;
-  plk::Fr vh_inv[2 * plk::kQBlocks];
+  plk::Fr vh_inv[plk::kQBlocksMax];
   plk_g1 comms[15];
   uint64_t struct_hash = 0;
   uint32_t max_wire = 0;
diff --git a/dusk-plonk_amd/csrc/prover_kernels.hip b/dusk-plonk_amd/csrc/prover_kernels.hip
--- a/dusk-plonk_amd/csrc/prover_kernels.hip
+++ b/dusk-plonk_amd/csrc/prover_kernels.hip
@@ -71,6 +71,18 @@
   for (uint32_t k = 0; k < pd.count; ++k)
     acc = rx_add(acc, rx_mul(rx_unpack(pd.c[k]), ldr(&tw_inv[(pd.idx[k] * j) & (n - 1)])));
   stf(&out[j], rx_pack_canonical(acc));
+}
+
+__global__ void __launch_bounds__(256) k_pi_sparse(PiSparse ps, const Fr* __restrict__ l1,
+                                                   uint32_t log_n, uint64_t nq,
+                                                   Fr* __restrict__ out) {
+  const uint64_t i = (uint64_t)blockIdx.x * blockDim.x + threadIdx.x;
+  if (i >= nq) return;
+  const uint64_t mask = (1ull << log_n) - 1, base = i & ~mask, u = i & mask;
+  RFr acc = rx_mul(ldr(&l1[base + ((u - ps.idx[0]) & mask)]), rx_unpack(ps.v[0]));
+  for (uint32_t k = 1; k < ps.count; ++k)
+    acc = rx_add(acc, rx_mul(ldr(&l1[base + ((u - ps.idx[k]) & mask)]), rx_unpack(ps.v[k])));
+  stf(&out[i], rx_pack_canonical(acc));
 }
 
 __global__ void k_blind_batch(BlindBatch bb, uint64_t n) {
@@ -263,7 +275,7 @@
   const uint64_t N = q.nq;
   if (i >= N) return;
   const uint64_t blk = i >> q.log_blk, u = i & ((1ull << q.log_blk) - 1);
-  const uint64_t nx = (blk << q.log_blk) + ((u + 2) & ((1ull << q.log_blk) - 1));
+  const uint64_t nx = (blk << q.log_blk) + ((u + 1) & ((1ull << q.log_blk) - 1));
   const RFr a = ldr(&q.a[i]), b = ldr(&q.b[i]), c = ldr(&q.c[i]), d = ldr(&q.d[i]);
   const RFr z = ldr(&q.z[i]), z_next = ldr(&q.z[nx]);
   RFr t = rx_mul(ldr(&q.sel[SEL_QM * N + i]), rx_mul(a, b));
@@ -312,7 +324,7 @@
     RFr num = t;
 #pragma unroll
     for (int l = 0; l < RxShape<FrCfg>::L; ++l) num.v[l] += perm.v[l];
-    stf(&q.out[i], rx_pack_canonical(rx_mul(num, rx_unpack(q.rx_vh[2 * blk + (u & 1)]))));
+    stf(&q.out[i], rx_pack_canonical(rx_mul(num, rx_unpack(q.rx_vh[blk]))));
   } else {
     stf(&q.out[i], rx_pack_canonical(rx_add(t, perm)));
   }
@@ -323,7 +335,7 @@
   const uint64_t N = q.nq;
   if (i >= N) return;
   const uint64_t blk = i >> q.log_blk, u = i & ((1ull << q.log_blk) - 1);
-  const uint64_t nx = (blk << q.log_blk) + ((u + 2) & ((1ull << q.log_blk) - 1));
+  const uint64_t nx = (blk << q.log_blk) + ((u + 1) & ((1ull << q.log_blk) - 1));
   auto ldw = [&](const Fr* p) { return fe_mul(ldf(p), q.rx_inv32); };
   const Fr a = ldw(&q.a[i]), b = ldw(&q.b[i]), c = ldw(&q.c[i]), d = ldw(&q.d[i]);
   Fr t = fe_mul(ldf(&q.out[i]), q.rx_32);
@@ -364,20 +376,27 @@
       t = fe_add(t, fe_mul(fe_mul(w, qv), q.var_sep));
     }
   }
-  stf(&q.out[i], fe_mul(t, q.vh_inv[2 * blk + (u & 1)]));
-}
-
-__global__ void __launch_bounds__(256) k_coset3_combine(const Fr* __restrict__ in, uint64_t n2,
-                                                        Fr c1a, Fr c1b, Fr c1c, Fr c2a, Fr c2b,
-                                                        Fr c2c, Fr* __restrict__ out) {
+  stf(&q.out[i], fe_mul(t, q.vh_inv[blk]));
+}
+
+template <int B>
+__global__ void __launch_bounds__(256) k_coset_combine(const Fr* __restrict__ in, uint64_t n,
+                                                       CombineMat mat, Fr* __restrict__ out) {
   const uint64_t k = (uint64_t)blockIdx.x * blockDim.x + threadIdx.x;
-  if (k >= n2) return;
-  const RFr b0 = ldr(&in[k]), b1 = ldr(&in[n2 + k]), b2 = ldr(&in[2 * n2 + k]);
-  stf(&out[k], rx_pack_canonical(rx_add(rx_add(b0, b1), b2)));
-  const RFr e1 = rx_add(rx_mul_add(b0, rx_unpack(c1a), b1, rx_unpack(c1b)), rx_mul(b2, rx_unpack(c1c)));
-  stf(&out[n2 + k], rx_pack_canonical(e1));
-  const RFr e2 = rx_add(rx_mul_add(b0, rx_unpack(c2a), b1, rx_unpack(c2b)), rx_mul(b2, rx_unpack(c2c)));
-  stf(&out[2 * n2 + k], rx_pack_canonical(e2));
+  if (k >= n) return;
+  RFr r[B];
+#pragma unroll
+  for (int m = 0; m < B; ++m) r[m] = ldr(&in[m * n + k]);
+#pragma unroll
+  for (int l = 0; l < B; ++l) {
+    const Fr* row = &mat.m[l * B];
+    RFr e = rx_mul_add(r[0], rx_unpack(row[0]), r[1], rx_unpack(row[1]));
+#pragma unroll
+    for (int m = 2; m + 1 < B; m += 2)
+      e = rx_add(e, rx_mul_add(r[m], rx_unpack(row[m]), r[m + 1], rx_unpack(row[m + 1])));
+    if (B & 1) e = rx_add(e, rx_mul(r[B - 1], rx_unpack(row[B - 1])));
+    stf(&out[l * n + k], rx_pack_canonical(e));
+  }
 }
 
 __global__ void k_scale_copy(const Fr* __restrict__ in, Fr c, Fr* __restrict__ out, uint64_t n) {
@@ -585,6 +604,15 @@
 int pk_pi_coef(const PiDirect& pd, const Fr* tw_inv, uint64_t n, Fr* out, hipStream_t s) {
   if (pd.count > (uint32_t)kPiDirect || (n & (n - 1))) return PLK_E_ARG;
   hipLaunchKernelGGL(k_pi_coef, dim3(blocks_for(n, 256)), dim3(256), 0, s, pd, tw_inv, n, out);
+  PLK_HIP_TRY(hipGetLastError());
+  return PLK_OK;
+}
+
+int pk_pi_sparse(const PiSparse& ps, const Fr* l1, uint32_t log_n, uint64_t nq, Fr* out,
+                 hipStream_t s) {
+  if (ps.count == 0 || ps.count > (uint32_t)kPiSparse) return PLK_E_ARG;
+  hipLaunchKernelGGL(k_pi_sparse, dim3(blocks_for(nq, 256)), dim3(256), 0, s, ps, l1, log_n, nq,
+                     out);
   PLK_HIP_TRY(hipGetLastError());
   return PLK_OK;
 }
@@ -657,9 +685,15 @@
   return PLK_OK;
 }
 
-int pk_coset3_combine(const Fr* in, uint64_t n2, const Fr* comb, Fr* out, hipStream_t s) {
-  hipLaunchKernelGGL(k_coset3_combine, dim3(blocks_for(n2, 256)), dim3(256), 0, s, in, n2, comb[0],
-                     comb[1], comb[2], comb[3], comb[4], comb[5], out);
+int pk_coset_combine(const Fr* in, uint64_t n, int blocks, const CombineMat& mat, Fr* out,
+                     hipStream_t s) {
+  const dim3 grid(blocks_for(n, 256));
+  if (blocks == kQBlocks)
+    hipLaunchKernelGGL((k_coset_combine<kQBlocks>), grid, dim3(256), 0, s, in, n, mat, out);
+  else if (blocks == kQBlocksSmall)
+    hipLaunchKernelGGL((k_coset_combine<kQBlocksSmall>), grid, dim3(256), 0, s, in, n, mat, out);
+  else
+    return PLK_E_ARG;
   PLK_HIP_TRY(hipGetLastError());
   return PLK_OK;
 }
diff --git a/dusk-plonk_amd/plonk.py b/dusk-plonk_amd/plonk.py
--- a/dusk-plonk_amd/plonk.py
+++ b/dusk-plonk_amd/plonk.py
@@ -18,7 +18,7 @@
     "plk_ntt_dev", "plk_ntt_batch_dev", "plk_srs_setup", "plk_srs_load", "plk_srs_destroy",
     "plk_srs_len", "plk_srs_points", "plk_msm", "plk_commit", "plk_commit_dev",
     "plk_srs_last_msm_stats", "plk_debug_field_op", "plk_debug_rx_op", "plk_debug_g1r_op",
-    "plk_commit_batch_dev",
+    "plk_debug_block_eval", "plk_commit_batch_dev",
     "plk_commit_batch_dev_part",
     "plk_srs_setup_range", "plk_g1_sum", "plk_msm_sharded", "plk_srs_msm_stats_reset",
     "plk_srs_cum_msm_stats", "plk_ntt_stream", "plk_aggregate_witness",
@@ -91,6 +91,7 @@
             "plk_debug_field_op": (i32, [vp, i32, i32, vp, vp, vp, sz]),
             "plk_debug_rx_op": (i32, [vp, i32, i32, vp, vp, vp, vp, vp, sz]),
             "plk_debug_g1r_op": (i32, [vp, i32, vp, vp, vp, vp, sz]),
+            "plk_debug_block_eval": (i32, [vp, vp, sz, vp, sz, C.POINTER(i32)]),
             "plk_commit_batch_dev": (i32, [vp, vp, vp, sz, vp, vp, vp]),
             "plk_commit_batch_dev_part": (i32, [vp, vp, vp, sz, u32, u32, vp, vp, vp]),
             "plk_srs_setup_range": (i32, [vp, vp, u64, sz, vp, pp]),
diff --git a/include/plk.h b/include/plk.h
--- a/include/plk.h
+++ b/include/plk.h
@@ -158,6 +158,8 @@
                     const uint32_t* c, const uint32_t* d, uint32_t* out, size_t n);
 int plk_debug_g1r_op(plk_ctx* ctx, int op, const uint32_t* p, const uint32_t* q,
                      const uint32_t* flags, uint32_t* out, size_t n);
+int plk_debug_block_eval(plk_key* key, const uint64_t* coef, size_t len, uint64_t* out,
+                         size_t out_cap, int* blocks_out);
 
 #ifdef __cplusplus
 }
```

New measurement: 33.88 million, median of 6. +4.9%, better.
